# davxy/ark-vrf

Hardware: AMD Instinct MI355X
Metric: thin_vrf_batch_verifications_per_sec (higher is better)
Workload: dtype u32x8 (256-bit prime-field Montgomery, integer)

## Files before the change

### ark_vrf_amd/csrc/batch_terms_dev.h

```cpp
#pragma once
#include "proto_dev.h"

namespace avrf {

AVRF_DI fp fp_from_u128(const uint32_t *w) {
  fp a = fp_zero(); uint4 v = *reinterpret_cast<const uint4 *>(w);
  a.v[0] = v.x; a.v[1] = v.y; a.v[2] = v.z; a.v[3] = v.w; return a;
}
template <class S> AVRF_DI void emit_term(uint32_t *scalars, te_pre *pre, uint32_t t, const fp &scalar_plain, const uint8_t *xy) {
  using Fq = typename S::Fq;
  fp_store(scalars + 8 * (size_t)t, scalar_plain);
  fp x = fp_to_mont<Fq>(fp_load_le(xy)), y = fp_to_mont<Fq>(fp_load_le(xy + 32));
  store_pre(pre + t, te_make_pre<S>(x, y));
}

template <class F, int NT, bool ROLLED = false>
AVRF_DI fp block_sum(const fp &v, fp *red) {
  red[threadIdx.x] = v;
  __syncthreads();
#pragma unroll ROLLED ? 1 : NT
  for (int s2 = NT / 2; s2 >= 1; s2 >>= 1) {
    if ((int)threadIdx.x < s2) red[threadIdx.x] = fp_add<F>(red[threadIdx.x], red[threadIdx.x + s2]);
    __syncthreads();
  }
  return red[0];
}

template <class S, class Out>
AVRF_DI fp thin_item(const BatchDev &b, const Seed64 &seed, uint64_t j0, const uint32_t *__restrict__ c_in, const uint32_t *__restrict__ z_in,
                     uint32_t j, const Out &out) {
  using Fr = typename S::Fr;
  uint32_t io0 = b.io_off[j], m = b.io_off[j + 1] - io0;
  uint64_t gj = j0 + j;
  uint32_t ww[4];
  if (b.weights) { const uint4 v = *reinterpret_cast<const uint4 *>(b.weights + 16 * (size_t)j); ww[0] = v.x; ww[1] = v.y; ww[2] = v.z; ww[3] = v.w; }
  else { uint64_t blk[8]; sha512_xof_block(seed.w, gj >> 2, blk); digest_le128(blk, (int)(gj & 3), ww); }
  fp w_plain = fp_zero(); w_plain.v[0] = ww[0]; w_plain.v[1] = ww[1]; w_plain.v[2] = ww[2]; w_plain.v[3] = ww[3];
  fp w = fp_to_mont<Fr>(w_plain);
  fp c = fp_to_mont<Fr>(fp_from_u128(c_in + 4 * (size_t)j));
  const uint8_t *pr = b.proofs + 96 * (size_t)j;
  fp s = fp_to_mont<Fr>(fp_load_le(pr + 64));
  fp wc = fp_mul<Fr>(w, c);
  fp ws = fp_mul<Fr>(w, s);
  out.r(j, io0, w_plain, pr);
  out.key(j, io0, wc);
  for (uint32_t i = 0; i < m; i++) {
    fp z = fp_to_mont<Fr>(fp_from_u128(z_in + 4 * (size_t)(io0 + i)));
    const uint8_t *p = b.ios_xy + 128 * (size_t)(io0 + i);
    out.output(j, io0, i, fp_from_mont<Fr>(fp_mul<Fr>(wc, z)), p + 64);
    out.input(j, io0, i, fp_neg<Fr>(fp_mul<Fr>(ws, z)), p);
  }
  return ws;
}

template <class S, class Out>
AVRF_DI fp ped_item(const BatchDev &b, const Seed64 &seed, uint64_t j0, const uint32_t *__restrict__ c_in, const uint8_t *__restrict__ merged_xy,
                    uint32_t j, const Out &out, fp &usb) {
  using Fr = typename S::Fr;
  fp t_plain, u_plain;
  if (b.weights) { t_plain = fp_from_u128(reinterpret_cast<const uint32_t *>(b.weights + 32 * (size_t)j)); u_plain = fp_from_u128(reinterpret_cast<const uint32_t *>(b.weights + 32 * (size_t)j + 16)); }
  else {
    ShaReader rd; for (int i = 0; i < 8; i++) rd.seed[i] = seed.w[i]; rd.have = 0;
    t_plain = xof128(rd, (uint32_t)(2 * (j0 + j))); u_plain = xof128(rd, (uint32_t)(2 * (j0 + j) + 1));
  }
  fp tt = fp_to_mont<Fr>(t_plain), uu = fp_to_mont<Fr>(u_plain);
  fp c = fp_to_mont<Fr>(fp_from_u128(c_in + 4 * (size_t)j));
  const uint8_t *pr = b.proofs + 256 * (size_t)j, *mo = merged_xy + 128 * (size_t)j;
  fp s = fp_to_mont<Fr>(fp_load_le(pr + 192)), sb = fp_to_mont<Fr>(fp_load_le(pr + 224));
  out.term(j, 0, fp_from_mont<Fr>(fp_mul<Fr>(tt, c)), mo + 64);
  out.term(j, 1, t_plain, pr + 128);
  out.term(j, 2, fp_from_mont<Fr>(fp_neg<Fr>(fp_mul<Fr>(tt, s))), mo);
  out.term(j, 3, fp_from_mont<Fr>(fp_mul<Fr>(uu, c)), pr);
  out.term(j, 4, u_plain, pr + 64);
  const fp us = fp_mul<Fr>(uu, s); usb = fp_mul<Fr>(uu, sb);
  return us;
}

template <class S, bool ROLLED = false>
AVRF_DI void base_term(const uint32_t *__restrict__ gpart, uint32_t nparts, uint32_t *__restrict__ scalars, te_pre *__restrict__ pre,
                       uint32_t t_last, int which_base, fp *red) {
  using Fr = typename S::Fr; using Fq = typename S::Fq;
  fp acc = fp_zero();
  for (uint32_t i = threadIdx.x; i < nparts; i += 256) acc = fp_add<Fr>(acc, fp_load(gpart + 8 * (size_t)i));
  const fp sum = block_sum<Fr, 256, ROLLED>(acc, red);
  if (threadIdx.x == 0) {
    fp_store(scalars + 8 * (size_t)t_last, fp_from_mont<Fr>(fp_neg<Fr>(sum)));
    te_pre g;
    if (which_base == 0) { g.x = fp_const<Fq>(S::G_X); g.y = fp_const<Fq>(S::G_Y); g.k = fp_const<Fq>(S::G_K); }
    else { g.x = fp_const<Fq>(S::B_X); g.y = fp_const<Fq>(S::B_Y); g.k = fp_const<Fq>(S::B_K); }
    store_pre(pre + t_last, g);
  }
}

}
```

### ark_vrf_amd/csrc/consts_gen.h

```cpp
#pragma once
#include <stdint.h>

namespace avrf {

struct FqBandersnatch {
  static constexpr int N = 8;
  static constexpr uint32_t P[8] = {0x00000001u, 0xffffffffu, 0xfffe5bfeu, 0x53bda402u, 0x09a1d805u, 0x3339d808u, 0x299d7d48u, 0x73eda753u};
  static constexpr uint32_t ONE[8] = {0xfffffffeu, 0x00000001u, 0x00034802u, 0x5884b7fau, 0xecbc4ff5u, 0x998c4fefu, 0xacc5056fu, 0x1824b159u};
  static constexpr uint32_t R2[8] = {0xf3f29c6du, 0xc999e990u, 0x87925c23u, 0x2b6cedcbu, 0x7254398fu, 0x05d31496u, 0x9f59ff11u, 0x0748d9d9u};
  static constexpr uint32_t HALF[8] = {0x80000000u, 0x7fffffffu, 0x7fff2dffu, 0xa9ded201u, 0x04d0ec02u, 0x199cec04u, 0x94cebea4u, 0x39f6d3a9u};
  static constexpr uint32_t NINV = 0xffffffffu;
  static constexpr int BITS = 255;
  static constexpr bool FULL = false;
  static constexpr int TWO_ADICITY = 32;
  static constexpr uint32_t T_MINUS1_HALF[8] = {0x7fffffffu, 0x7fff2dffu, 0xa9ded201u, 0x04d0ec02u, 0x199cec04u, 0x94cebea4u, 0x39f6d3a9u, 0x00000000u};
  static constexpr uint32_t ROOT[8] = {0x0c17f47cu, 0x9cab6d5cu, 0xfd4b71e5u, 0x1ce1e93du, 0x471dd505u, 0x0d6db230u, 0x743a3b6au, 0x3f0ee990u};
  static constexpr uint32_t PM2[8] = {0xffffffffu, 0xfffffffeu, 0xfffe5bfeu, 0x53bda402u, 0x09a1d805u, 0x3339d808u, 0x299d7d48u, 0x73eda753u};
  static constexpr int SQRT_W = 8;
  static constexpr int SQRT_HW = 8;
  static constexpr int SQRT_STEPS = 4;
  static constexpr int SQRT_HBITS = 12;
  static constexpr uint32_t SQRT_HMUL = 0xa330d7b1u;
  static constexpr uint8_t SQRT_HIDX[4096] = {0, 0, 0, 139, 0, 0, 0, 0, 0, 0, 0, 167, 0, 0, 0, 0, 0, 0, 0, 0, 0, 133, 0, 0, 189, 0, 0, 0, 4, 0, 0, 0, 0, 0, 0, 0, 0, 0, 0, 226, 0, 0, 0, 0, 0, 248, 0, 0, 0, 0, 0, 0, 0, 0, 0, 0, 0, 0, 0, 0, 18, 0, 0, 0,
    0, 0, 0, 150, 0, 0, 0, 0, 0, 0, 0, 0, 0, 0, 0, 0, 0, 0, 0, 0, 0, 0, 0, 0, 0, 0, 0, 0, 0, 0, 0, 0, 0, 0, 0, 0, 0, 0, 0, 247, 0, 0, 0, 0, 0, 0, 0, 0, 0, 0, 0, 0, 0, 0, 0, 0, 0, 0, 0, 0, 0, 0, 0, 0,
    0, 0, 0, 0, 0, 0, 185, 0, 0, 0, 0, 0, 0, 0, 0, 0, 0, 148, 0, 0, 0, 0, 0, 0, 0, 0, 0, 0, 0, 0, 0, 0, 0, 0, 0, 0, 0, 0, 0, 0, 0, 0, 0, 0, 0, 0, 0, 0, 0, 17, 0, 0, 0, 0, 0, 0, 0, 0, 0, 0, 0, 0, 0, 0,
    0, 0, 0, 143, 0, 0, 0, 0, 0, 0, 0, 0, 0, 0, 0, 0, 0, 0, 0, 209, 0, 0, 0, 0, 0, 0, 0, 0, 0, 0, 0, 0, 0, 0, 0, 0, 0, 0, 0, 0, 0, 80, 0, 0, 0, 0, 0, 0, 0, 0, 0, 0, 0, 0, 23, 0, 0, 0, 0, 0, 0, 0, 0, 0,
    0, 0, 0, 0, 0, 0, 193, 0, 0, 0, 0, 0, 0, 0, 0, 0, 0, 0, 217, 0, 0, 0, 0, 0, 0, 0, 0, 0, 0, 210, 0, 0, 27, 0, 0, 0, 0, 0, 0, 0, 0, 0, 0, 0, 0, 0, 0, 0, 0, 0, 0, 0, 0, 0, 0, 230, 0, 77, 0, 161, 0, 0, 0, 0,
    0, 0, 0, 0, 0, 0, 0, 0, 0, 0, 0, 0, 121, 0, 0, 0, 0, 0, 0, 0, 0, 0, 173, 0, 0, 0, 0, 0, 0, 0, 0, 0, 0, 0, 0, 0, 0, 0, 188, 0, 0, 0, 0, 0, 0, 0, 0, 0, 0, 0, 0, 0, 0, 0, 0, 0, 0, 0, 0, 0, 0, 0, 0, 0,
    0, 0, 0, 0, 0, 0, 0, 0, 229, 0, 0, 0, 0, 0, 0, 0, 0, 0, 0, 99, 0, 0, 0, 0, 0, 0, 0, 0, 0, 0, 0, 0, 0, 0, 0, 0, 0, 0, 25, 0, 0, 0, 0, 0, 0, 0, 0, 0, 0, 0, 0, 0, 0, 0, 0, 0, 0, 0, 0, 0, 0, 0, 0, 0,
    0, 0, 218, 0, 0, 0, 0, 0, 0, 0, 0, 0, 0, 0, 0, 0, 0, 0, 0, 0, 0, 0, 0, 0, 0, 0, 0, 0, 0, 0, 0, 0, 0, 0, 0, 0, 156, 0, 0, 0, 0, 0, 0, 0, 0, 0, 0, 0, 0, 0, 0, 0, 0, 0, 0, 0, 0, 0, 0, 0, 0, 0, 0, 0,
    0, 0, 0, 0, 0, 0, 0, 0, 0, 0, 0, 0, 0, 0, 0, 0, 0, 0, 0, 0, 0, 0, 0, 0, 0, 0, 0, 0, 0, 0, 26, 0, 0, 0, 0, 0, 0, 0, 0, 0, 0, 236, 0, 0, 0, 0, 0, 0, 0, 55, 0, 0, 0, 0, 157, 0, 0, 0, 0, 0, 0, 0, 0, 0,
    0, 0, 0, 0, 0, 0, 0, 0, 0, 0, 0, 0, 0, 0, 0, 0, 0, 0, 0, 0, 109, 123, 0, 0, 0, 0, 0, 0, 0, 0, 0, 0, 0, 0, 0, 0, 0, 0, 0, 0, 0, 0, 0, 0, 0, 0, 0, 0, 0, 0, 0, 0, 0, 0, 0, 0, 0, 0, 0, 0, 0, 0, 0, 0,
    0, 0, 0, 225, 0, 0, 0, 0, 0, 0, 0, 0, 0, 0, 134, 0, 0, 159, 0, 0, 0, 0, 242, 0, 0, 0, 0, 244, 0, 0, 0, 0, 0, 0, 0, 0, 0, 0, 0, 0, 0, 0, 0, 0, 0, 0, 0, 0, 0, 0, 0, 0, 0, 0, 0, 0, 0, 0, 0, 76, 0, 0, 0, 152,
    0, 0, 0, 0, 0, 0, 0, 0, 0, 0, 0, 0, 0, 164, 0, 0, 0, 0, 0, 223, 0, 0, 21, 0, 0, 0, 0, 0, 0, 0, 40, 0, 0, 0, 0, 0, 0, 0, 0, 0, 0, 0, 0, 0, 0, 0, 0, 0, 0, 0, 0, 0, 0, 0, 0, 0, 0, 0, 0, 0, 0, 0, 0, 0,
    0, 0, 0, 0, 0, 0, 0, 0, 0, 0, 0, 0, 0, 141, 0, 0, 0, 0, 0, 0, 0, 0, 0, 0, 0, 0, 0, 0, 0, 0, 0, 0, 0, 0, 0, 0, 0, 0, 0, 0, 0, 0, 0, 0, 0, 0, 0, 0, 0, 0, 0, 0, 0, 0, 0, 0, 0, 0, 0, 0, 0, 0, 0, 0,
    0, 0, 0, 0, 0, 0, 0, 0, 0, 0, 0, 0, 0, 93, 0, 0, 0, 0, 171, 0, 0, 0, 0, 0, 0, 0, 0, 0, 0, 0, 0, 0, 0, 0, 0, 0, 0, 0, 0, 0, 0, 0, 0, 0, 0, 0, 0, 0, 0, 79, 0, 0, 0, 0, 0, 0, 0, 0, 0, 0, 0, 0, 0, 0,
    0, 0, 0, 0, 0, 0, 0, 0, 0, 0, 0, 0, 0, 0, 0, 0, 0, 0, 0, 0, 0, 0, 0, 0, 0, 0, 0, 0, 0, 0, 0, 0, 0, 0, 0, 0, 0, 0, 0, 0, 0, 0, 91, 0, 0, 158, 0, 0, 0, 0, 0, 0, 0, 0, 0, 0, 0, 0, 0, 0, 0, 0, 0, 0,
    0, 0, 0, 0, 0, 0, 0, 0, 0, 0, 0, 200, 0, 0, 0, 0, 0, 0, 0, 0, 0, 0, 0, 0, 0, 0, 0, 0, 0, 0, 0, 63, 0, 0, 0, 0, 0, 0, 0, 0, 0, 0, 0, 0, 0, 66, 0, 0, 0, 0, 0, 0, 0, 0, 0, 0, 0, 0, 0, 0, 0, 0, 0, 0,
    0, 0, 0, 0, 0, 0, 0, 0, 222, 0, 0, 0, 0, 0, 0, 0, 0, 0, 182, 0, 0, 0, 0, 0, 0, 0, 0, 0, 0, 0, 0, 0, 0, 0, 0, 0, 0, 0, 0, 0, 0, 0, 0, 0, 0, 0, 0, 0, 0, 0, 0, 0, 0, 0, 0, 0, 0, 0, 0, 0, 0, 0, 0, 0,
    0, 0, 0, 0, 0, 0, 0, 0, 0, 0, 0, 0, 0, 0, 0, 0, 0, 0, 0, 0, 113, 0, 0, 0, 0, 0, 0, 0, 0, 0, 0, 0, 0, 0, 0, 0, 0, 0, 0, 0, 124, 255, 0, 0, 0, 0, 0, 0, 0, 0, 0, 0, 0, 0, 59, 0, 0, 0, 0, 0, 0, 0, 0, 0,
    0, 0, 0, 0, 0, 0, 0, 0, 0, 0, 0, 0, 0, 170, 0, 0, 0, 184, 0, 0, 0, 0, 0, 87, 0, 0, 0, 83, 0, 0, 0, 0, 0, 0, 0, 0, 0, 0, 0, 44, 0, 0, 0, 0, 0, 0, 64, 0, 0, 0, 0, 0, 0, 0, 0, 0, 0, 0, 0, 0, 0, 0, 0, 0,
    0, 0, 0, 0, 0, 0, 0, 0, 0, 0, 0, 0, 0, 0, 0, 0, 0, 0, 0, 14, 0, 0, 0, 0, 0, 0, 0, 0, 0, 0, 0, 0, 213, 0, 0, 0, 0, 0, 0, 0, 0, 0, 0, 203, 0, 0, 0, 0, 0, 0, 0, 0, 199, 52, 0, 0, 0, 0, 0, 0, 0, 0, 0, 0,
    0, 0, 0, 0, 0, 86, 0, 0, 0, 0, 69, 0, 0, 126, 0, 0, 0, 0, 0, 0, 48, 0, 0, 0, 0, 0, 0, 0, 0, 0, 176, 0, 0, 0, 0, 0, 0, 254, 0, 0, 197, 0, 0, 0, 0, 214, 0, 0, 0, 0, 0, 0, 0, 0, 0, 0, 0, 0, 0, 0, 0, 180, 71, 0,
    0, 0, 0, 0, 0, 0, 0, 75, 0, 0, 0, 0, 0, 0, 0, 0, 0, 0, 85, 0, 0, 0, 0, 0, 0, 0, 0, 0, 0, 0, 0, 142, 0, 0, 0, 0, 0, 0, 0, 0, 0, 0, 0, 0, 0, 0, 0, 0, 0, 0, 0, 0, 0, 0, 0, 0, 0, 0, 0, 0, 0, 0, 0, 0,
    0, 0, 0, 0, 192, 0, 0, 0, 0, 0, 0, 172, 0, 0, 0, 0, 0, 0, 0, 0, 0, 0, 0, 211, 0, 0, 0, 215, 0, 0, 0, 0, 0, 0, 56, 0, 0, 42, 0, 0, 0, 0, 0, 0, 0, 0, 0, 0, 0, 0, 0, 0, 0, 0, 0, 0, 0, 0, 0, 0, 187, 0, 0, 0,
    0, 0, 0, 0, 0, 0, 0, 0, 0, 127, 252, 0, 0, 0, 0, 0, 0, 0, 0, 0, 0, 0, 0, 0, 0, 0, 0, 0, 0, 0, 241, 0, 0, 0, 0, 0, 0, 0, 0, 0, 0, 0, 0, 0, 0, 0, 0, 0, 0, 0, 0, 0, 0, 0, 0, 0, 0, 0, 0, 0, 0, 0, 0, 0,
    0, 0, 0, 0, 0, 0, 0, 0, 0, 0, 0, 0, 0, 0, 0, 0, 0, 0, 0, 0, 0, 0, 0, 0, 0, 0, 0, 0, 0, 0, 0, 0, 54, 0, 0, 0, 0, 0, 0, 0, 0, 0, 94, 0, 0, 0, 0, 0, 0, 0, 0, 0, 0, 0, 0, 0, 0, 0, 0, 0, 0, 0, 0, 0,
    0, 0, 0, 0, 0, 194, 0, 0, 0, 0, 0, 0, 0, 0, 0, 0, 0, 0, 0, 191, 0, 0, 0, 0, 0, 0, 0, 0, 0, 0, 0, 0, 0, 0, 0, 0, 0, 0, 0, 72, 0, 0, 0, 0, 0, 0, 0, 0, 0, 0, 0, 0, 0, 0, 0, 0, 0, 0, 0, 0, 0, 0, 0, 0,
    0, 0, 0, 0, 0, 30, 0, 0, 219, 0, 0, 0, 0, 0, 0, 0, 0, 0, 0, 0, 0, 0, 0, 0, 0, 0, 0, 0, 0, 0, 0, 0, 0, 0, 0, 0, 0, 0, 0, 0, 0, 0, 0, 0, 0, 0, 0, 0, 0, 0, 0, 0, 0, 0, 0, 0, 0, 0, 0, 0, 0, 0, 0, 0,
    0, 207, 0, 0, 0, 0, 0, 0, 0, 0, 0, 0, 0, 0, 0, 0, 0, 0, 0, 0, 0, 0, 0, 0, 0, 0, 0, 0, 0, 0, 0, 0, 0, 43, 0, 0, 0, 221, 0, 0, 0, 0, 0, 0, 0, 0, 0, 0, 0, 0, 0, 0, 0, 0, 0, 0, 0, 0, 0, 0, 0, 0, 0, 0,
    0, 0, 0, 0, 0, 0, 0, 0, 0, 0, 0, 0, 0, 0, 0, 0, 0, 0, 0, 0, 0, 0, 0, 0, 0, 0, 0, 0, 0, 0, 0, 0, 0, 0, 0, 0, 0, 13, 0, 0, 0, 0, 0, 0, 0, 0, 0, 0, 0, 0, 0, 0, 0, 0, 0, 0, 0, 0, 0, 0, 0, 0, 0, 0,
    0, 0, 0, 0, 0, 0, 0, 0, 0, 0, 0, 0, 0, 0, 0, 0, 0, 0, 0, 0, 168, 0, 0, 0, 0, 0, 0, 0, 149, 0, 0, 95, 0, 0, 0, 0, 0, 36, 0, 0, 0, 0, 0, 0, 0, 0, 0, 0, 0, 0, 0, 24, 0, 0, 0, 204, 0, 0, 0, 0, 0, 0, 0, 0,
    0, 0, 0, 0, 0, 0, 0, 0, 0, 0, 0, 0, 0, 0, 0, 0, 0, 0, 0, 0, 0, 0, 0, 116, 0, 0, 0, 0, 114, 0, 0, 0, 0, 31, 0, 0, 6, 0, 0, 0, 0, 0, 0, 0, 0, 0, 0, 97, 0, 0, 0, 0, 0, 0, 0, 0, 0, 0, 0, 0, 0, 0, 0, 0,
    0, 0, 0, 0, 0, 0, 0, 0, 0, 0, 0, 0, 0, 0, 0, 0, 0, 0, 0, 0, 0, 0, 0, 0, 0, 0, 0, 0, 0, 251, 237, 0, 0, 0, 0, 0, 0, 0, 0, 0, 0, 0, 0, 0, 0, 0, 0, 0, 0, 0, 0, 0, 0, 0, 0, 0, 0, 0, 0, 0, 29, 0, 0, 0,
    0, 183, 0, 0, 0, 0, 0, 0, 0, 108, 0, 0, 0, 0, 0, 0, 0, 0, 0, 0, 154, 0, 0, 0, 0, 0, 0, 0, 0, 0, 0, 0, 0, 0, 0, 0, 0, 0, 0, 0, 0, 0, 0, 0, 0, 0, 0, 0, 0, 0, 0, 0, 0, 0, 0, 0, 0, 0, 0, 0, 0, 0, 0, 0,
    0, 0, 0, 0, 0, 0, 0, 0, 0, 0, 0, 0, 0, 0, 0, 28, 0, 0, 0, 0, 0, 0, 0, 0, 0, 0, 0, 0, 0, 0, 0, 0, 0, 0, 0, 0, 0, 0, 0, 0, 0, 0, 0, 0, 0, 0, 0, 0, 90, 0, 0, 0, 0, 0, 0, 0, 0, 0, 0, 0, 0, 0, 0, 0,
    0, 0, 0, 0, 0, 0, 0, 0, 0, 0, 0, 0, 153, 0, 0, 0, 0, 0, 0, 0, 0, 0, 0, 0, 0, 0, 0, 0, 0, 0, 0, 227, 0, 0, 0, 0, 0, 0, 0, 0, 0, 0, 101, 0, 0, 0, 0, 0, 0, 0, 0, 0, 0, 0, 0, 0, 0, 0, 0, 0, 0, 0, 0, 0,
    0, 0, 0, 0, 0, 0, 0, 0, 0, 0, 0, 0, 60, 0, 0, 0, 0, 0, 0, 0, 0, 0, 0, 0, 0, 0, 0, 0, 45, 0, 0, 0, 0, 0, 0, 0, 0, 0, 249, 0, 0, 0, 0, 0, 0, 0, 0, 0, 0, 0, 0, 0, 0, 0, 0, 33, 0, 205, 0, 102, 0, 0, 0, 0,
    0, 0, 0, 0, 0, 0, 0, 0, 0, 0, 0, 0, 0, 0, 0, 0, 0, 0, 155, 0, 0, 82, 0, 0, 0, 0, 0, 0, 0, 0, 0, 0, 89, 0, 0, 0, 0, 0, 0, 0, 0, 0, 0, 0, 65, 0, 0, 0, 0, 0, 0, 0, 0, 0, 0, 0, 0, 0, 0, 0, 151, 0, 0, 0,
    0, 0, 0, 0, 0, 0, 0, 0, 0, 208, 0, 0, 0, 0, 0, 0, 0, 0, 0, 0, 0, 0, 0, 0, 0, 0, 0, 0, 0, 0, 0, 81, 0, 0, 0, 0, 0, 0, 0, 0, 0, 0, 0, 0, 0, 0, 0, 15, 0, 0, 0, 0, 0, 0, 0, 0, 0, 0, 0, 0, 0, 0, 0, 0,
    0, 145, 0, 0, 0, 0, 0, 0, 0, 0, 0, 0, 0, 0, 0, 0, 0, 0, 0, 0, 0, 0, 0, 0, 0, 0, 0, 0, 0, 0, 0, 0, 0, 20, 0, 0, 0, 0, 0, 0, 0, 0, 0, 0, 57, 0, 0, 0, 0, 0, 0, 0, 0, 0, 0, 0, 0, 0, 0, 0, 0, 0, 0, 0,
    0, 0, 0, 0, 0, 0, 0, 0, 0, 0, 0, 119, 0, 0, 0, 0, 0, 0, 0, 0, 0, 0, 0, 0, 0, 0, 0, 0, 0, 0, 0, 0, 0, 0, 0, 0, 0, 0, 0, 0, 0, 0, 0, 0, 0, 0, 0, 22, 0, 0, 0, 0, 0, 0, 146, 0, 0, 0, 0, 0, 0, 0, 0, 0,
    0, 0, 0, 0, 0, 120, 0, 0, 0, 0, 0, 98, 0, 0, 0, 0, 0, 0, 0, 0, 0, 0, 132, 0, 0, 0, 61, 0, 0, 5, 0, 0, 0, 0, 0, 0, 0, 0, 0, 39, 0, 0, 0, 0, 0, 0, 0, 11, 0, 0, 0, 0, 0, 0, 0, 0, 0, 0, 0, 0, 0, 0, 0, 0,
    0, 0, 0, 0, 0, 0, 0, 0, 0, 0, 0, 0, 0, 0, 0, 0, 234, 0, 0, 0, 0, 0, 0, 0, 0, 0, 0, 92, 0, 0, 0, 0, 0, 0, 0, 0, 0, 0, 0, 0, 0, 0, 0, 0, 0, 0, 0, 0, 0, 0, 0, 19, 0, 0, 0, 0, 0, 0, 0, 186, 0, 0, 0, 0,
    0, 0, 0, 0, 0, 0, 0, 0, 0, 0, 0, 0, 0, 0, 0, 0, 0, 0, 0, 0, 0, 0, 0, 0, 0, 0, 0, 0, 0, 0, 0, 0, 0, 0, 0, 0, 0, 0, 0, 0, 0, 0, 0, 195, 0, 0, 0, 0, 0, 0, 0, 0, 0, 0, 0, 0, 0, 0, 0, 0, 0, 0, 0, 0,
    0, 0, 0, 0, 0, 0, 0, 0, 12, 0, 0, 0, 73, 0, 0, 0, 100, 0, 0, 0, 0, 0, 0, 0, 0, 0, 0, 0, 0, 0, 0, 0, 0, 0, 239, 0, 0, 0, 0, 0, 0, 0, 0, 0, 0, 0, 0, 0, 62, 0, 0, 0, 50, 0, 0, 0, 0, 0, 0, 0, 0, 0, 0, 3,
    0, 0, 0, 0, 7, 0, 0, 0, 122, 0, 0, 0, 0, 0, 0, 0, 0, 0, 0, 0, 0, 130, 0, 0, 0, 9, 68, 0, 0, 0, 0, 0, 0, 0, 0, 0, 0, 0, 0, 0, 0, 0, 0, 0, 0, 0, 0, 0, 0, 0, 0, 0, 0, 0, 0, 0, 216, 0, 0, 0, 0, 105, 175, 0,
    0, 0, 0, 0, 0, 0, 0, 0, 0, 0, 0, 0, 0, 0, 0, 0, 0, 115, 0, 0, 0, 0, 0, 0, 0, 0, 0, 0, 0, 0, 0, 117, 0, 0, 0, 0, 0, 0, 238, 0, 0, 0, 0, 0, 118, 0, 0, 0, 0, 0, 0, 0, 0, 35, 129, 0, 0, 0, 169, 0, 0, 0, 0, 0,
    0, 0, 0, 0, 0, 160, 0, 0, 0, 0, 70, 0, 174, 0, 0, 0, 0, 0, 0, 0, 0, 0, 0, 0, 0, 0, 0, 0, 0, 0, 0, 0, 0, 34, 0, 0, 0, 0, 10, 0, 0, 0, 0, 0, 0, 0, 0, 0, 0, 0, 0, 0, 0, 0, 0, 0, 0, 0, 0, 0, 0, 0, 0, 0,
    0, 0, 0, 0, 0, 0, 0, 0, 0, 0, 0, 0, 0, 0, 0, 0, 0, 0, 0, 0, 0, 0, 0, 0, 0, 0, 0, 253, 0, 0, 0, 0, 0, 0, 0, 0, 0, 0, 0, 0, 0, 0, 0, 0, 165, 0, 0, 0, 0, 0, 0, 0, 0, 0, 0, 0, 181, 0, 0, 0, 0, 0, 0, 0,
    0, 0, 0, 0, 0, 0, 0, 0, 0, 0, 0, 0, 0, 0, 0, 0, 0, 0, 177, 0, 0, 0, 212, 0, 0, 0, 0, 0, 0, 0, 0, 0, 166, 0, 0, 0, 0, 0, 0, 0, 0, 0, 107, 0, 0, 0, 0, 0, 0, 0, 0, 0, 0, 0, 0, 0, 0, 0, 0, 0, 0, 0, 0, 0,
    0, 0, 0, 0, 0, 0, 0, 0, 0, 0, 0, 0, 0, 0, 0, 0, 0, 0, 0, 232, 0, 0, 0, 0, 0, 0, 0, 0, 224, 0, 0, 0, 0, 0, 0, 0, 0, 0, 0, 0, 0, 0, 0, 0, 0, 0, 0, 0, 0, 0, 0, 0, 0, 0, 240, 0, 0, 0, 0, 0, 0, 0, 0, 0,
    0, 0, 0, 0, 0, 0, 0, 0, 0, 0, 0, 0, 0, 0, 0, 0, 0, 0, 0, 0, 0, 0, 0, 0, 0, 0, 0, 0, 0, 0, 0, 0, 0, 0, 0, 0, 0, 0, 0, 0, 0, 0, 0, 0, 0, 0, 0, 0, 0, 0, 0, 0, 0, 0, 0, 0, 0, 0, 0, 0, 0, 0, 0, 0,
    0, 0, 0, 16, 0, 0, 0, 0, 0, 0, 0, 0, 0, 0, 0, 0, 0, 0, 0, 0, 0, 0, 0, 0, 0, 0, 0, 51, 0, 0, 0, 0, 0, 0, 0, 0, 0, 0, 0, 0, 0, 0, 0, 0, 0, 0, 0, 0, 0, 0, 0, 0, 74, 0, 0, 0, 0, 0, 0, 0, 0, 0, 103, 0,
    0, 0, 0, 0, 0, 8, 78, 0, 0, 0, 0, 0, 0, 0, 0, 0, 0, 0, 0, 0, 0, 0, 0, 0, 0, 0, 0, 0, 0, 0, 0, 0, 0, 0, 0, 0, 0, 0, 0, 0, 0, 0, 0, 0, 206, 136, 0, 0, 0, 0, 0, 0, 231, 0, 0, 0, 0, 0, 0, 0, 0, 0, 202, 0,
    0, 0, 0, 0, 0, 0, 0, 0, 0, 0, 0, 0, 0, 0, 0, 0, 0, 0, 0, 0, 0, 0, 0, 179, 0, 0, 0, 0, 0, 0, 0, 0, 0, 0, 0, 0, 0, 0, 0, 0, 0, 0, 0, 0, 0, 0, 0, 144, 0, 0, 0, 0, 0, 0, 0, 0, 0, 0, 0, 0, 0, 0, 0, 0,
    0, 0, 0, 0, 0, 0, 0, 0, 0, 0, 0, 0, 0, 0, 0, 0, 0, 0, 0, 0, 0, 0, 0, 0, 0, 0, 0, 0, 0, 0, 0, 0, 0, 0, 0, 0, 0, 0, 0, 0, 0, 0, 0, 0, 0, 0, 0, 0, 0, 0, 0, 0, 0, 0, 0, 0, 0, 0, 0, 0, 112, 0, 0, 0,
    0, 0, 0, 0, 0, 0, 0, 0, 0, 0, 0, 0, 0, 0, 0, 0, 0, 0, 0, 0, 0, 0, 96, 0, 0, 0, 0, 0, 0, 0, 0, 104, 0, 0, 0, 0, 0, 0, 0, 0, 0, 0, 0, 0, 0, 0, 0, 0, 0, 0, 0, 0, 0, 0, 0, 0, 0, 0, 0, 0, 0, 0, 0, 0,
    0, 0, 0, 0, 0, 0, 0, 0, 235, 0, 0, 0, 0, 0, 0, 0, 0, 0, 38, 0, 0, 0, 0, 0, 0, 0, 0, 0, 84, 0, 0, 0, 49, 0, 0, 0, 0, 0, 0, 0, 0, 0, 0, 0, 0, 0, 0, 0, 0, 0, 0, 0, 0, 0, 0, 0, 0, 0, 53, 0, 0, 0, 0, 0,
    0, 0, 0, 0, 0, 0, 37, 0, 0, 0, 0, 0, 0, 0, 0, 0, 0, 0, 0, 0, 0, 0, 0, 125, 0, 0, 0, 0, 0, 0, 0, 0, 0, 0, 0, 0, 0, 0, 0, 0, 0, 0, 0, 0, 0, 0, 0, 0, 0, 0, 0, 0, 0, 0, 0, 0, 0, 0, 0, 0, 0, 0, 0, 0,
    0, 0, 0, 0, 0, 0, 0, 0, 0, 0, 0, 0, 138, 0, 0, 0, 0, 162, 0, 0, 0, 0, 0, 0, 0, 128, 0, 0, 0, 0, 0, 0, 0, 0, 0, 0, 0, 0, 46, 0, 198, 0, 0, 0, 0, 32, 0, 0, 0, 0, 0, 0, 0, 0, 0, 0, 41, 0, 0, 0, 1, 163, 0, 0,
    0, 0, 0, 0, 0, 0, 246, 0, 0, 0, 0, 0, 110, 0, 0, 0, 0, 0, 0, 245, 0, 0, 0, 0, 0, 0, 0, 0, 0, 0, 0, 0, 0, 243, 0, 0, 0, 0, 0, 0, 0, 0, 0, 0, 0, 0, 0, 0, 0, 0, 0, 0, 47, 233, 0, 0, 0, 0, 88, 0, 0, 0, 0, 0,
    0, 0, 0, 0, 0, 0, 0, 0, 0, 0, 0, 0, 0, 0, 0, 0, 0, 0, 0, 0, 0, 0, 0, 0, 196, 137, 0, 0, 0, 2, 0, 0, 0, 0, 0, 0, 0, 0, 0, 0, 0, 0, 250, 0, 0, 0, 135, 0, 0, 0, 0, 131, 0, 0, 0, 0, 0, 0, 0, 0, 0, 0, 178, 0,
    0, 0, 190, 0, 0, 0, 0, 0, 0, 0, 0, 0, 0, 0, 0, 0, 111, 0, 0, 0, 0, 0, 0, 0, 0, 0, 0, 0, 0, 0, 0, 0, 0, 0, 228, 0, 0, 0, 0, 201, 0, 0, 140, 0, 0, 0, 0, 0, 0, 0, 0, 0, 0, 0, 0, 0, 0, 0, 0, 0, 0, 0, 0, 0,
    0, 0, 0, 0, 0, 0, 0, 67, 0, 0, 0, 0, 0, 0, 0, 0, 0, 0, 0, 0, 0, 0, 0, 0, 0, 0, 0, 0, 0, 0, 0, 0, 0, 0, 0, 0, 0, 0, 0, 0, 0, 0, 0, 0, 0, 0, 0, 0, 0, 0, 0, 0, 0, 0, 0, 58, 0, 0, 0, 0, 0, 0, 0, 147,
    0, 0, 0, 0, 0, 0, 0, 0, 0, 0, 0, 0, 0, 0, 0, 0, 0, 0, 0, 0, 0, 0, 0, 220, 0, 0, 0, 0, 0, 0, 0, 0, 0, 0, 106, 0, 0, 0, 0, 0, 0, 0, 0, 0, 0, 0, 0, 0, 0, 0, 0, 0, 0, 0, 0, 0, 0, 0, 0, 0, 0, 0, 0, 0};
  static constexpr uint32_t SQRT_G[4][256][8] = {{{0xfffffffeu, 0x00000001u, 0x00034802u, 0x5884b7fau, 0xecbc4ff5u, 0x998c4fefu, 0xacc5056fu, 0x1824b159u},
     {0xb3082d19u, 0x55a9e082u, 0xc7dc4a13u, 0x082f90b2u, 0xc76b052cu, 0x76ce3accu, 0x6e54185du, 0x15c39d95u},
     {0x05ddb4b8u, 0xb1bb81b1u, 0x4a762df0u, 0x98ffbb06u, 0xc5590209u, 0x726e959bu, 0x47a5e6aau, 0x0db2facbu},
     {0x4ba518a6u, 0x1cb397a0u, 0xe29bbae1u, 0xa6c4b1a6u, 0x446848f8u, 0x9c4d6f8cu, 0x4f599f0fu, 0x38590951u},
     {0x081b0db0u, 0x88291cf6u, 0x961782b0u, 0x8dea521au, 0x5485c90cu, 0xbf29568bu, 0x48e86a89u, 0x0abe1809u},
     {0xa619ac2au, 0x7a94fe9cu, 0xacd2cd1du, 0xa7d16f94u, 0x3f6d45e1u, 0xeb6432c7u, 0x69cba988u, 0x675bd361u},
// ... 1965 lines not shown
     {0x38a0b01eu, 0x71711555u, 0x4ad8bc83u, 0x7b62860au, 0x8782f80cu, 0xdae18326u, 0x8643d3c0u, 0x659d3378u},
     {0xe79619e8u, 0xbea57a0du, 0x30dfe95cu, 0xa307a773u, 0x757cc2b5u, 0xfa9bfbe4u, 0x7793ed48u, 0x1f278bdau},
     {0x5c85a48cu, 0xa5c78e6bu, 0x27dea76du, 0x3321a9d5u, 0x26f5f2ffu, 0x650e3bc6u, 0xf388ee57u, 0x05dc672au},
     {0x21df81e1u, 0xd49618f1u, 0x69e1efbdu, 0x629f100fu, 0x290a9c33u, 0xe5ec780au, 0x195bd29fu, 0x42342477u},
     {0x8f153822u, 0x190c7999u, 0x255bed10u, 0xff8667b7u, 0xfca3ce8au, 0xab9a30e6u, 0xcc563dc6u, 0x67d521b3u},
     {0x0c9a6196u, 0xe1ab252eu, 0x8c4639a8u, 0x99e01587u, 0x53ac4640u, 0xde1593d3u, 0x63fba955u, 0x545dee68u},
     {0x9d5bfae5u, 0x0eeebb8au, 0xac1efb3du, 0xff066916u, 0xddacd1a4u, 0x08c08e43u, 0x8948edf4u, 0x3f78143au},
     {0x2e7f1dc5u, 0x985c3cf6u, 0x9931a557u, 0x2ce65886u, 0xa5c89bbbu, 0xc783312eu, 0x6c4ec654u, 0x63692be2u},
     {0xc8a679b5u, 0x1575b970u, 0xe7d73a66u, 0xff7e3e9eu, 0x75be7c92u, 0x197077f6u, 0xd9afc7c1u, 0x4f67aeeau},
     {0x27640509u, 0xb0adef9au, 0x5f151c19u, 0x5959fdadu, 0x1d65c479u, 0x465e597bu, 0xd2631306u, 0x54db6e81u},
     {0xfb9b6cafu, 0xe4ea9f4du, 0xa2e53698u, 0xc5c2f8bfu, 0x32e15854u, 0x3656c273u, 0xf624afb5u, 0x14e2af6au},
     {0x5cc3402fu, 0x9df8c650u, 0x8eecfc0bu, 0x52161e02u, 0xc15e1bd4u, 0xd8363390u, 0xb209a781u, 0x58b8ae49u},
     {0x0edcce43u, 0xac2d119au, 0x0b5c9748u, 0x72e16391u, 0xb8958a06u, 0xa5715c3au, 0x57eeddd7u, 0x208a3b69u},
     {0x2c42eff8u, 0x6ecf4995u, 0x4d5dfa57u, 0x6ec1fa83u, 0x5656b15cu, 0x3ff5cf38u, 0x229e031bu, 0x54b80267u},
     {0xcc8444a5u, 0x90f6ca3bu, 0xb2348e04u, 0x14328249u, 0xee9ff368u, 0x9e1a4112u, 0x36badb91u, 0x49871dbdu},
     {0x295f01c5u, 0x2120e8a1u, 0x2bfa2fe5u, 0xcdebe1c7u, 0xdbbe9be6u, 0x2316952cu, 0xad2c723cu, 0x4b12a723u},
     {0x5b26f8b7u, 0x7ec4963du, 0xbaf08852u, 0xfc700595u, 0xe05523aau, 0xafc2f038u, 0x47197ed5u, 0x6b38b922u},
     {0x00ff35a2u, 0x2df3cffeu, 0xd8a54c35u, 0x8eaad385u, 0x73beda30u, 0x5a69ae1eu, 0x25cd8149u, 0x0ff2db8bu},
     {0x74dd5d7du, 0xbbb83148u, 0x8dafb8d6u, 0x39a9f661u, 0xe2db2568u, 0x0b08c472u, 0xee3af837u, 0x57598d2du},
     {0x87c54b83u, 0x693a8406u, 0xc68ebc74u, 0x1a480ddfu, 0x1ab40886u, 0xbf6277d1u, 0x79357d86u, 0x5f1a79ecu},
     {0xcd01e401u, 0x508f9afdu, 0xf449da9eu, 0xe348018cu, 0x4e84779du, 0xd552b7f9u, 0x37192982u, 0x41a2d19fu},
     {0xfa15c3aau, 0x3f250480u, 0xc047eb08u, 0xe07f6b96u, 0xe062508du, 0x3e4c19e1u, 0x72c2db07u, 0x071af18du},
     {0x1926ef0au, 0xd71a1016u, 0x14f1596bu, 0x1f063ac7u, 0xe929c6e2u, 0x0a9280b4u, 0xb8adeebcu, 0x37c836e3u},
     {0x1fd6ad56u, 0x6f765257u, 0xb0e5ddc4u, 0x5e09ca58u, 0xe6edaba3u, 0x452d4de9u, 0xa6d8a0a9u, 0x49cc3e60u},
     {0x2960af99u, 0xcb4b0e08u, 0x9f39e65cu, 0xaf57e981u, 0x51900ae1u, 0xc67b09b0u, 0xff21015eu, 0x085174abu},
     {0x0e92863cu, 0xb8390a3au, 0xc2863873u, 0x96044e6au, 0x8d6a0836u, 0x687322c8u, 0x8c1fa261u, 0x5c67f128u},
     {0x2cc8d086u, 0x97ae36d8u, 0x86ed9472u, 0x12c8360eu, 0x61e28bc2u, 0x8abd6721u, 0x520aa6bau, 0x6a96e461u},
     {0x11015834u, 0x7179e258u, 0x123ae337u, 0x00cc579fu, 0xcd24624bu, 0x34d5b008u, 0xe61da78au, 0x4e3c38aeu},
     {0x1ccd9350u, 0x38252215u, 0x513cd923u, 0xe2be613bu, 0x8613483eu, 0x952dd456u, 0xef52bfbeu, 0x2bdc7f5fu},
     {0x8e7396bdu, 0x9b248771u, 0x26512fcau, 0xf3b6754du, 0x1c539a97u, 0x34d5a86au, 0x758a30b2u, 0x188eeac5u},
     {0x11f2bec2u, 0x5f804b9bu, 0x974c34d5u, 0xb8795d14u, 0xf2df56e6u, 0xd88bc50au, 0x4ee3ffdcu, 0x6965d71cu},
     {0x3ed117d1u, 0x978cf7c8u, 0x8c5be1cbu, 0xfbea1715u, 0x3735000eu, 0xea44c4dbu, 0x4f6a138bu, 0x09f5c923u},
     {0x242103d5u, 0x0488c019u, 0x8a9255c6u, 0xda927718u, 0x2189c3f0u, 0xc1df9b00u, 0xd80c2aaau, 0x6a479f59u},
     {0x83be6793u, 0xa747e335u, 0x65f3469bu, 0x67e96b40u, 0x28053fe0u, 0xf27eec7cu, 0x5df2e598u, 0x3967452au},
     {0x06690b79u, 0x20871c43u, 0xc6cf4b80u, 0xf1994a48u, 0x91c8ecb4u, 0x8f821e00u, 0xaa89169au, 0x0bfb4c4eu},
     {0xd326577fu, 0x86b66109u, 0xc2e56c9bu, 0xf62e7165u, 0xa281ca4fu, 0x0f24d9cau, 0x5418de14u, 0x6827b849u},
     {0xea815d48u, 0x0b5a32d5u, 0x4a0239d4u, 0x6d1b4960u, 0x54de0512u, 0x5923129bu, 0x23174a1eu, 0x65a0400fu},
     {0x47dc3a8eu, 0x21419c6fu, 0x0e46c9e4u, 0x7317c3f5u, 0x3cd7e698u, 0x7c1e12ccu, 0x657c748bu, 0x72f09140u},
     {0x1248245au, 0x8870b9e3u, 0xd2cab986u, 0xb02ab3e2u, 0x4e204b01u, 0x6bc2be6du, 0xb4e2f21fu, 0x06f9fbb5u},
     {0x475f9917u, 0x4f8202a9u, 0x455e945bu, 0x55bf85ebu, 0xe32d7d9du, 0x6d4c8d1cu, 0x750bb29cu, 0x4d07a125u},
     {0xad0a14b7u, 0x7bd28a68u, 0x6693267fu, 0xf23d8db7u, 0xb520258cu, 0x54781be7u, 0x076cae45u, 0x319e968fu},
     {0x58371c58u, 0xe2723242u, 0x4596c7a7u, 0x953f710au, 0x05336c1au, 0xdd8e0667u, 0xba634814u, 0x44b2c153u},
     {0x0e3f6ca9u, 0x1280ba88u, 0x5ed2de1eu, 0x61b18d33u, 0x5cf486ceu, 0xb7f93933u, 0x9990f2ecu, 0x63369ddfu},
     {0x04de444bu, 0x1f5c0f6fu, 0xe3cfbaabu, 0x990b7d15u, 0x1a08d412u, 0xf8c2d5b9u, 0xc1fc894au, 0x31d70d61u},
     {0xab0be02bu, 0x53705adau, 0x98a62326u, 0x68512e19u, 0xd9f802e0u, 0x61571bdbu, 0x5c24e491u, 0x2fce8180u},
     {0xf4f5ed78u, 0xda3d5ffcu, 0x82f63a76u, 0xbca13283u, 0x3187122cu, 0xebfffb3du, 0x3aba3b86u, 0x248d2ba9u},
     {0x8e9fd984u, 0x7fce7d9bu, 0xd3b4713fu, 0x8af4e9ebu, 0x492b1d8eu, 0xa4f87dc0u, 0x8bb2d12du, 0x64b4b4e0u},
     {0xdd4f278cu, 0x75d572e8u, 0x13fc66ddu, 0x6d430159u, 0x92af252eu, 0xbaaa83d0u, 0xd31e8d84u, 0x394417c5u},
     {0x58da6aa4u, 0x82a20808u, 0x74829b5cu, 0x0228ee6au, 0xc9ad1160u, 0xb003ab1du, 0x34558665u, 0x41c5136bu},
     {0x7a99de9eu, 0x5a005690u, 0x277c49dbu, 0xcadb8951u, 0x829c620eu, 0x2379d76du, 0x244f4e65u, 0x1b378533u},
     {0xd4f64112u, 0xbf907bd1u, 0x77f47f45u, 0x0b168a22u, 0x08cc3a32u, 0x08c0e078u, 0xb0466d3au, 0x2c9cf211u},
     {0x78608249u, 0x05966d0bu, 0xb5386ac0u, 0x2f0458f2u, 0x264a0035u, 0x9b2e75ebu, 0x153a4cdfu, 0x3977f860u},
     {0x165d516eu, 0x963577f8u, 0x2ac0d3c5u, 0xaad9d00du, 0x64beed41u, 0x1afb7aaeu, 0x5051301du, 0x27006e59u},
     {0xcaca8313u, 0x0f1935d8u, 0x13b9bbe6u, 0x6bb619c1u, 0xe3f7a2d4u, 0x897d1e65u, 0x61ad525cu, 0x60ef201fu},
     {0x7c58e718u, 0xc11900b5u, 0x2c8cf843u, 0x7ddacaffu, 0xee2be61cu, 0xd9c13167u, 0x52050d46u, 0x0a9f3ae4u},
     {0xc9b1d3fcu, 0x6d79af89u, 0x7fb0345bu, 0x691fa9cau, 0x0ee1a74bu, 0xbac24d73u, 0x7e18a2aeu, 0x4865647eu},
     {0x14820d20u, 0x480d513cu, 0xdbea11dfu, 0xf3335d70u, 0x048359d7u, 0x2ba2fb41u, 0xf0f5e5d3u, 0x137198c5u},
     {0x916f7696u, 0x89bcccc5u, 0x88346f55u, 0x289bfc73u, 0x92e7d2d2u, 0xf36fb797u, 0xa7975ff5u, 0x4e97b638u},
     {0x3f739ac8u, 0xbfb0e683u, 0x2a5dfc83u, 0xe78fdad9u, 0xf8d6a763u, 0xf56f910eu, 0xf7e98b32u, 0x2fb9a958u},
     {0x709d69b0u, 0xd2b7d884u, 0xa111176cu, 0xbd13cd26u, 0x860eeebbu, 0x16f27755u, 0x5135a880u, 0x5ade1e7eu},
     {0x9853db04u, 0x81002b30u, 0xa5110b64u, 0x505d3ffdu, 0xe499541du, 0x43f3d603u, 0x1650b215u, 0x2883be66u},
     {0xdce32ecdu, 0x3a9b9f5bu, 0xb00bfc10u, 0xbdf98f59u, 0x894d3c96u, 0x961ca1b7u, 0x8a58766au, 0x579b3349u},
     {0x7d1f75b2u, 0x1b3c4feeu, 0x5af3fbc6u, 0x5265b158u, 0x1b468fe1u, 0x7e5c8c6au, 0xc3df928cu, 0x5ad7fe3au},
     {0x85190e97u, 0x3ff4cf36u, 0x76bf2e40u, 0x40c0d395u, 0x0bab14adu, 0xa5f3819du, 0x9390c01fu, 0x1ac4416bu},
     {0x3f26a9d1u, 0x25c3d512u, 0x083589c5u, 0x7d76d9e3u, 0x48c34a65u, 0xcfd61babu, 0x815554bcu, 0x3a10c229u},
     {0x71609b1au, 0xe8e8d1dfu, 0x0eb2f768u, 0x1cf1e962u, 0x9768a3c1u, 0x9fabe672u, 0xc6caae31u, 0x08ecbfa6u},
     {0x79bf4f1bu, 0xb5319907u, 0x983baadeu, 0xf317d445u, 0x6e269d85u, 0xfff73680u, 0xf4271f8du, 0x49c8dabcu},
     {0x83d014fau, 0x4606e968u, 0x7cd8ed52u, 0xc1f33b71u, 0xefba713au, 0x14e48227u, 0xc1c7efe4u, 0x54150adbu},
     {0x49eb7f23u, 0xa3b3f4dbu, 0x8caa9728u, 0x200f8a43u, 0x2652d494u, 0x7fc85d41u, 0x81885aefu, 0x1fee884cu},
     {0x8ad8bf35u, 0xe2646a4eu, 0xad159082u, 0x8b0d49dcu, 0xc608d4a7u, 0x2437f5abu, 0xc2606638u, 0x10270bf3u},
     {0x78f132efu, 0x8e7b2bddu, 0x7fd503e5u, 0x34528098u, 0x42d80083u, 0x0ea75e6eu, 0xfa0fd473u, 0x307f4f00u},
     {0x6494ce4bu, 0x5be50d8cu, 0x0e4a28fcu, 0x1f0038d4u, 0x5a6e8ca6u, 0x7bf4c2ceu, 0xb9f90fa8u, 0x5d5b87f2u},
     {0xb6e0b9e0u, 0x5b7a9877u, 0x6c064730u, 0x0932ac01u, 0x23023385u, 0x3f58c35au, 0xc343d22au, 0x42431340u},
     {0x0cd952aeu, 0x3c9c9e42u, 0x237cc1a0u, 0xbc23d412u, 0x5dc8bba1u, 0x9d7bd317u, 0x42ab5b37u, 0x29f78689u},
     {0xe0d8211cu, 0x816f371cu, 0xd22347ceu, 0x32bf4b89u, 0x4a501e19u, 0x9d272cfeu, 0x5f1ce5a8u, 0x0e3e41e3u},
     {0xeeacbd55u, 0x353e37b1u, 0xe98d368cu, 0x575b1e34u, 0xb25a5128u, 0xb9d5021bu, 0xe185e732u, 0x1caae6b8u},
     {0x88ac07cdu, 0x6b45cacbu, 0xe9500b87u, 0x09c4d7b2u, 0xf27cbdc9u, 0x2d5de551u, 0x49cd4467u, 0x07fa8c1cu}}};
};
struct FrBandersnatch {
  static constexpr int N = 8;
  static constexpr uint32_t P[8] = {0x2876e7e1u, 0x74fd06b5u, 0x74190471u, 0xff8f8700u, 0x02687600u, 0x0cce7602u, 0xca675f52u, 0x1cfb69d4u};
  static constexpr uint32_t ONE[8] = {0xbc48c0f8u, 0x5817ca56u, 0x5f37dc74u, 0x0383c7fcu, 0xecbc4ff8u, 0x998c4fefu, 0xacc5056fu, 0x1824b159u};
  static constexpr uint32_t R2[8] = {0x58db47cbu, 0xdbb4f5d6u, 0x7fecb938u, 0x40fa7ca2u, 0xc0055ceau, 0xaa9e6daeu, 0xb14aec7du, 0x0ae793ddu};
  static constexpr uint32_t HALF[8] = {0x943b73f0u, 0xba7e835au, 0x3a0c8238u, 0x7fc7c380u, 0x01343b00u, 0x06673b01u, 0x6533afa9u, 0x0e7db4eau};
  static constexpr uint32_t NINV = 0x5cc063dfu;
  static constexpr int BITS = 253;
  static constexpr bool FULL = false;
  static constexpr int TWO_ADICITY = 5;
  static constexpr uint32_t T_MINUS1_HALF[8] = {0xd4a1db9fu, 0xc5d3f41au, 0x01d06411u, 0x03fe3e1cu, 0x0809a1d8u, 0x483339d8u, 0x53299d7du, 0x0073eda7u};
  static constexpr uint32_t ROOT[8] = {0x8d79c573u, 0x4b263b9au, 0x007af1fdu, 0xeadb3d0au, 0x68832589u, 0xa54c8a46u, 0x4254fb9du, 0x0610860cu};
  static constexpr uint32_t PM2[8] = {0x2876e7dfu, 0x74fd06b5u, 0x74190471u, 0xff8f8700u, 0x02687600u, 0x0cce7602u, 0xca675f52u, 0x1cfb69d4u};
};
struct FqBabyJubJub {
  static constexpr int N = 8;
  static constexpr uint32_t P[8] = {0xf0000001u, 0x43e1f593u, 0x79b97091u, 0x2833e848u, 0x8181585du, 0xb85045b6u, 0xe131a029u, 0x30644e72u};
  static constexpr uint32_t ONE[8] = {0x4ffffffbu, 0xac96341cu, 0x9f60cd29u, 0x36fc7695u, 0x7879462eu, 0x666ea36fu, 0x9a07df2fu, 0x0e0a77c1u};
  static constexpr uint32_t R2[8] = {0xae216da7u, 0x1bb8e645u, 0xe35c59e3u, 0x53fe3ab1u, 0x53bb8085u, 0x8c49833du, 0x7f4e44a5u, 0x0216d0b1u};
  static constexpr uint32_t HALF[8] = {0xf8000000u, 0xa1f0fac9u, 0x3cdcb848u, 0x9419f424u, 0x40c0ac2eu, 0xdc2822dbu, 0x7098d014u, 0x18322739u};
  static constexpr uint32_t NINV = 0xefffffffu;
  static constexpr int BITS = 254;
  static constexpr bool FULL = false;
  static constexpr int TWO_ADICITY = 28;
  static constexpr uint32_t T_MINUS1_HALF[8] = {0x1f0fac9fu, 0xcdcb848au, 0x419f4243u, 0x0c0ac2e9u, 0xc2822db4u, 0x098d014du, 0x83227397u, 0x00000001u};
  static constexpr uint32_t ROOT[8] = {0x80d13d9cu, 0x636e7355u, 0x2445ffd6u, 0xa22bf374u, 0x1eb203d8u, 0x56452ac0u, 0x2963f9e7u, 0x1860ef94u};
  static constexpr uint32_t PM2[8] = {0xefffffffu, 0x43e1f593u, 0x79b97091u, 0x2833e848u, 0x8181585du, 0xb85045b6u, 0xe131a029u, 0x30644e72u};
  static constexpr int SQRT_W = 8;
  static constexpr int SQRT_HW = 8;
  static constexpr int SQRT_STEPS = 4;
  static constexpr int SQRT_HBITS = 12;
  static constexpr uint32_t SQRT_HMUL = 0x64ac5db9u;
  static constexpr uint8_t SQRT_HIDX[4096] = {170, 0, 0, 0, 0, 0, 0, 0, 0, 0, 0, 0, 0, 0, 0, 0, 0, 0, 0, 0, 0, 0, 0, 0, 0, 0, 0, 0, 0, 196, 0, 0, 0, 0, 0, 0, 0, 0, 0, 0, 0, 0, 0, 0, 0, 0, 0, 0, 0, 0, 0, 0, 0, 0, 0, 0, 0, 0, 0, 0, 0, 0, 0, 0,
    0, 0, 0, 0, 0, 0, 0, 0, 0, 0, 0, 0, 0, 0, 0, 0, 0, 0, 0, 0, 0, 0, 0, 0, 0, 0, 0, 198, 0, 0, 0, 0, 0, 0, 0, 103, 0, 165, 0, 0, 1, 0, 0, 0, 0, 0, 0, 0, 0, 0, 0, 0, 0, 0, 0, 0, 0, 0, 0, 0, 0, 0, 0, 0,
    0, 0, 0, 0, 0, 0, 0, 0, 0, 0, 0, 0, 0, 0, 0, 0, 166, 0, 0, 0, 0, 0, 0, 0, 0, 0, 0, 0, 0, 0, 0, 0, 0, 0, 0, 0, 0, 0, 195, 0, 0, 0, 0, 0, 0, 0, 0, 0, 0, 0, 0, 0, 26, 0, 0, 0, 0, 0, 0, 105, 0, 0, 0, 0,
    0, 0, 0, 0, 0, 0, 0, 0, 0, 0, 0, 0, 0, 0, 0, 0, 0, 0, 0, 0, 163, 0, 0, 0, 0, 0, 0, 0, 0, 0, 0, 0, 0, 0, 0, 0, 0, 0, 0, 0, 0, 0, 228, 0, 187, 0, 0, 0, 0, 0, 0, 0, 0, 0, 117, 0, 0, 0, 0, 0, 0, 0, 98, 0,
    0, 0, 191, 0, 0, 0, 0, 0, 0, 0, 0, 0, 0, 0, 0, 0, 0, 0, 0, 0, 0, 0, 0, 0, 52, 0, 0, 0, 0, 0, 0, 0, 0, 0, 0, 0, 0, 0, 0, 0, 0, 0, 0, 0, 0, 0, 0, 0, 0, 0, 0, 0, 0, 0, 0, 0, 0, 0, 0, 0, 0, 0, 0, 0,
    0, 0, 0, 0, 115, 0, 0, 0, 0, 0, 0, 0, 0, 0, 0, 0, 0, 0, 0, 0, 0, 0, 0, 0, 0, 234, 0, 0, 0, 0, 0, 0, 0, 123, 0, 0, 0, 0, 0, 0, 0, 0, 0, 0, 0, 0, 0, 0, 0, 0, 0, 0, 0, 0, 0, 0, 0, 0, 0, 19, 0, 0, 0, 0,
    0, 0, 0, 0, 0, 0, 0, 0, 0, 0, 0, 0, 0, 0, 0, 0, 0, 0, 0, 0, 0, 0, 0, 0, 0, 0, 0, 0, 0, 0, 0, 0, 0, 0, 0, 0, 0, 0, 0, 0, 0, 0, 0, 0, 0, 0, 0, 0, 0, 0, 0, 0, 0, 0, 0, 0, 0, 0, 0, 0, 0, 0, 0, 0,
    0, 125, 0, 0, 0, 0, 2, 0, 0, 0, 0, 0, 0, 0, 0, 0, 0, 0, 40, 0, 0, 0, 0, 0, 0, 0, 0, 0, 0, 0, 0, 0, 183, 0, 0, 0, 0, 0, 0, 0, 0, 0, 0, 0, 0, 0, 27, 0, 0, 0, 0, 0, 0, 0, 0, 0, 0, 0, 0, 0, 0, 0, 0, 0,
    0, 0, 0, 0, 0, 0, 0, 0, 0, 0, 0, 0, 0, 0, 0, 0, 0, 0, 0, 0, 0, 104, 0, 0, 0, 0, 0, 0, 0, 0, 0, 0, 0, 0, 0, 0, 0, 0, 0, 0, 13, 0, 0, 0, 0, 0, 0, 0, 0, 0, 0, 0, 0, 0, 33, 0, 0, 0, 0, 0, 0, 0, 0, 0,
    0, 0, 0, 0, 0, 0, 0, 0, 0, 0, 0, 0, 0, 0, 90, 0, 0, 0, 0, 205, 0, 0, 0, 0, 0, 0, 0, 0, 0, 0, 0, 0, 0, 0, 0, 47, 0, 0, 0, 0, 172, 0, 0, 0, 0, 0, 0, 41, 0, 0, 0, 0, 0, 0, 0, 0, 0, 0, 0, 0, 0, 0, 0, 0,
    255, 0, 0, 0, 0, 0, 0, 0, 0, 0, 0, 0, 0, 0, 0, 188, 0, 241, 0, 0, 0, 0, 0, 0, 0, 0, 0, 0, 5, 0, 0, 0, 0, 0, 0, 0, 0, 0, 0, 0, 0, 0, 0, 0, 0, 240, 0, 0, 0, 0, 0, 0, 0, 74, 0, 0, 22, 0, 0, 0, 0, 0, 0, 0,
    0, 0, 0, 0, 0, 0, 0, 0, 0, 0, 0, 0, 0, 0, 0, 0, 0, 206, 0, 0, 0, 0, 0, 0, 0, 0, 0, 0, 194, 0, 0, 0, 0, 0, 0, 0, 0, 0, 0, 0, 0, 0, 0, 0, 0, 0, 0, 0, 0, 0, 0, 0, 0, 0, 0, 0, 0, 0, 0, 0, 0, 0, 0, 0,
    0, 0, 0, 0, 0, 0, 0, 0, 56, 0, 0, 0, 0, 0, 0, 0, 84, 0, 0, 0, 0, 0, 0, 0, 0, 0, 0, 0, 0, 0, 0, 0, 0, 0, 0, 0, 0, 0, 0, 0, 0, 0, 0, 0, 0, 0, 0, 0, 0, 0, 0, 0, 0, 0, 0, 0, 0, 0, 0, 0, 0, 0, 219, 0,
    0, 0, 0, 30, 0, 0, 0, 0, 73, 0, 0, 0, 0, 0, 0, 0, 0, 0, 0, 0, 0, 0, 3, 0, 0, 0, 143, 0, 0, 0, 0, 0, 0, 11, 0, 189, 0, 0, 0, 0, 0, 0, 0, 0, 0, 0, 0, 0, 0, 0, 23, 0, 0, 49, 0, 0, 0, 0, 0, 0, 0, 0, 89, 0,
    0, 0, 39, 0, 0, 0, 0, 0, 0, 0, 0, 0, 0, 0, 102, 0, 0, 0, 107, 0, 0, 0, 0, 76, 0, 0, 0, 0, 0, 0, 0, 0, 0, 0, 0, 0, 0, 0, 0, 0, 0, 0, 0, 0, 0, 0, 0, 0, 0, 0, 0, 0, 0, 0, 0, 0, 0, 0, 0, 0, 0, 0, 0, 0,
    0, 0, 0, 0, 0, 0, 0, 0, 0, 0, 0, 0, 0, 0, 0, 0, 0, 0, 0, 0, 0, 0, 0, 0, 0, 0, 0, 83, 0, 0, 0, 0, 0, 0, 0, 0, 0, 0, 0, 0, 0, 0, 0, 0, 0, 0, 0, 0, 0, 0, 186, 0, 0, 0, 227, 0, 0, 7, 0, 0, 92, 0, 247, 0,
    0, 181, 0, 0, 0, 0, 0, 0, 0, 0, 0, 0, 0, 0, 0, 0, 199, 0, 0, 0, 0, 0, 0, 0, 0, 0, 0, 0, 0, 0, 0, 0, 0, 0, 0, 0, 0, 0, 0, 0, 0, 0, 0, 0, 0, 0, 0, 50, 0, 0, 0, 0, 0, 0, 0, 0, 0, 0, 0, 0, 0, 0, 0, 0,
    0, 0, 0, 0, 0, 0, 0, 0, 0, 0, 0, 0, 0, 0, 0, 0, 0, 0, 0, 0, 0, 0, 0, 0, 0, 0, 0, 0, 95, 0, 0, 0, 0, 0, 0, 0, 0, 0, 0, 0, 0, 0, 0, 0, 0, 0, 0, 0, 0, 0, 0, 0, 0, 0, 0, 0, 0, 36, 0, 0, 0, 0, 0, 0,
    0, 0, 0, 0, 0, 0, 0, 0, 0, 0, 0, 0, 0, 0, 0, 0, 0, 0, 0, 0, 237, 0, 0, 0, 0, 0, 0, 0, 0, 149, 0, 0, 0, 0, 0, 0, 229, 0, 0, 0, 159, 0, 0, 0, 0, 0, 88, 0, 0, 0, 0, 0, 110, 0, 0, 0, 0, 0, 0, 0, 0, 0, 0, 0,
    0, 156, 0, 0, 0, 0, 0, 0, 0, 0, 0, 0, 0, 0, 0, 0, 0, 145, 0, 0, 0, 0, 0, 0, 0, 0, 0, 0, 0, 0, 0, 0, 0, 64, 0, 0, 0, 0, 0, 0, 0, 0, 0, 0, 0, 0, 0, 0, 0, 0, 0, 0, 0, 0, 0, 0, 0, 0, 0, 0, 0, 0, 0, 0,
    0, 0, 0, 0, 0, 0, 0, 0, 0, 79, 0, 0, 0, 0, 0, 0, 0, 0, 0, 0, 0, 193, 0, 69, 0, 62, 0, 0, 0, 0, 0, 0, 0, 0, 0, 0, 120, 0, 0, 0, 0, 0, 0, 0, 0, 0, 0, 0, 0, 0, 0, 0, 0, 0, 0, 0, 0, 0, 0, 0, 0, 0, 0, 214,
    0, 0, 0, 0, 0, 0, 0, 0, 0, 0, 0, 0, 0, 0, 0, 0, 122, 0, 48, 0, 0, 144, 0, 0, 0, 0, 0, 0, 0, 0, 0, 0, 0, 0, 0, 54, 0, 0, 0, 0, 0, 0, 0, 200, 0, 0, 0, 0, 0, 0, 0, 0, 0, 0, 0, 0, 0, 0, 0, 0, 0, 0, 0, 0,
    0, 0, 0, 0, 0, 0, 0, 0, 0, 0, 0, 0, 0, 0, 0, 0, 0, 0, 0, 0, 0, 0, 0, 0, 0, 0, 0, 0, 0, 0, 0, 0, 0, 244, 0, 0, 224, 0, 0, 0, 6, 0, 0, 0, 0, 0, 0, 0, 246, 0, 0, 0, 0, 209, 0, 0, 0, 0, 0, 0, 0, 0, 0, 0,
    0, 0, 142, 0, 0, 0, 0, 0, 0, 0, 0, 0, 0, 0, 75, 0, 0, 0, 0, 0, 222, 0, 0, 0, 0, 0, 0, 0, 0, 0, 0, 0, 0, 0, 0, 0, 0, 0, 0, 0, 0, 0, 0, 0, 0, 0, 0, 0, 0, 0, 0, 0, 0, 0, 0, 0, 0, 0, 0, 0, 0, 0, 0, 0,
    8, 0, 0, 0, 0, 0, 0, 0, 0, 0, 0, 0, 0, 0, 0, 0, 0, 0, 0, 0, 0, 0, 18, 0, 0, 0, 0, 0, 0, 0, 0, 0, 0, 0, 0, 0, 0, 0, 0, 0, 0, 0, 0, 114, 0, 0, 0, 0, 0, 0, 0, 0, 0, 0, 0, 0, 0, 45, 0, 0, 0, 0, 0, 85,
    0, 0, 0, 0, 0, 0, 0, 0, 0, 0, 0, 0, 0, 0, 0, 0, 0, 0, 0, 0, 0, 0, 0, 0, 0, 0, 0, 0, 0, 0, 0, 0, 0, 0, 0, 0, 0, 0, 0, 0, 0, 0, 0, 0, 0, 32, 0, 0, 0, 0, 46, 0, 0, 0, 0, 0, 0, 0, 0, 0, 0, 0, 0, 0,
    0, 0, 0, 0, 0, 0, 0, 0, 0, 0, 137, 0, 0, 87, 0, 0, 0, 0, 0, 0, 0, 0, 0, 0, 0, 0, 29, 0, 0, 0, 0, 0, 0, 0, 0, 0, 0, 0, 0, 0, 0, 0, 0, 0, 0, 0, 0, 157, 0, 0, 0, 0, 0, 0, 0, 0, 0, 0, 0, 0, 0, 215, 0, 0,
    9, 0, 0, 0, 0, 0, 0, 0, 0, 0, 0, 0, 0, 0, 0, 0, 0, 0, 0, 0, 0, 0, 0, 0, 174, 0, 0, 0, 0, 160, 0, 0, 0, 0, 0, 0, 0, 0, 0, 0, 0, 0, 0, 0, 0, 0, 0, 0, 0, 0, 0, 0, 0, 0, 0, 0, 0, 0, 0, 0, 0, 0, 0, 0,
    0, 0, 0, 0, 0, 0, 0, 0, 0, 0, 0, 213, 0, 0, 0, 0, 173, 0, 0, 0, 0, 0, 0, 0, 0, 0, 0, 0, 0, 0, 0, 242, 0, 0, 0, 0, 0, 0, 0, 0, 0, 0, 0, 0, 0, 0, 0, 0, 0, 0, 0, 0, 146, 0, 0, 0, 0, 0, 0, 0, 0, 0, 0, 0,
    0, 0, 0, 0, 0, 0, 0, 0, 0, 0, 136, 0, 0, 0, 0, 0, 0, 0, 0, 0, 0, 0, 0, 0, 0, 0, 0, 0, 0, 0, 0, 0, 0, 0, 0, 0, 0, 0, 0, 0, 0, 0, 0, 0, 0, 0, 0, 0, 0, 0, 0, 0, 0, 0, 94, 0, 0, 0, 0, 203, 0, 0, 0, 0,
    0, 0, 0, 0, 0, 0, 0, 0, 14, 0, 0, 0, 0, 0, 0, 0, 0, 0, 0, 0, 0, 81, 0, 0, 0, 118, 0, 0, 0, 0, 0, 0, 0, 0, 134, 0, 0, 0, 96, 0, 0, 116, 0, 0, 0, 0, 0, 0, 0, 0, 0, 0, 0, 0, 0, 0, 0, 0, 0, 0, 0, 0, 0, 0,
    0, 0, 0, 0, 0, 0, 0, 0, 0, 0, 0, 0, 0, 0, 0, 0, 0, 0, 0, 0, 0, 0, 0, 0, 0, 0, 0, 0, 0, 0, 0, 72, 0, 0, 0, 0, 0, 0, 0, 182, 0, 0, 0, 0, 0, 0, 0, 0, 0, 0, 0, 0, 0, 16, 0, 0, 176, 0, 250, 0, 0, 0, 0, 0,
    0, 0, 0, 0, 0, 0, 0, 0, 0, 0, 0, 86, 0, 0, 0, 0, 0, 0, 0, 0, 0, 0, 0, 0, 0, 0, 0, 0, 0, 0, 0, 0, 0, 0, 0, 0, 0, 0, 248, 0, 0, 0, 0, 0, 0, 0, 0, 0, 0, 190, 0, 197, 0, 65, 0, 0, 0, 0, 0, 0, 0, 0, 0, 0,
    0, 207, 0, 0, 0, 0, 0, 0, 0, 0, 0, 0, 0, 0, 0, 0, 0, 0, 0, 0, 0, 0, 0, 0, 0, 0, 0, 0, 0, 0, 0, 0, 0, 0, 0, 0, 0, 0, 0, 0, 0, 192, 0, 0, 0, 0, 0, 0, 0, 0, 0, 0, 0, 0, 0, 0, 0, 17, 0, 0, 0, 0, 0, 0,
    0, 0, 0, 0, 0, 0, 0, 0, 0, 28, 0, 0, 0, 0, 0, 0, 0, 0, 0, 0, 0, 0, 238, 0, 0, 0, 0, 0, 216, 0, 0, 0, 0, 31, 0, 0, 0, 0, 101, 0, 0, 0, 0, 0, 0, 21, 0, 0, 0, 0, 0, 0, 0, 0, 109, 0, 0, 0, 0, 0, 0, 0, 0, 0,
    0, 0, 0, 0, 0, 0, 0, 0, 0, 0, 0, 0, 0, 0, 0, 0, 0, 164, 0, 0, 0, 0, 0, 0, 0, 0, 0, 0, 0, 0, 0, 0, 0, 0, 0, 0, 0, 0, 0, 0, 0, 0, 0, 0, 0, 223, 0, 0, 0, 0, 0, 0, 0, 0, 0, 0, 0, 0, 0, 0, 0, 0, 0, 0,
    0, 0, 0, 0, 0, 0, 0, 0, 0, 0, 0, 0, 0, 0, 0, 0, 0, 0, 0, 0, 0, 0, 0, 0, 0, 0, 0, 178, 0, 0, 0, 0, 0, 0, 0, 0, 0, 0, 0, 0, 0, 0, 0, 0, 0, 0, 0, 0, 0, 0, 0, 0, 0, 0, 0, 0, 0, 71, 0, 0, 0, 0, 0, 0,
    0, 0, 0, 0, 0, 0, 0, 0, 0, 53, 0, 119, 0, 0, 220, 0, 0, 135, 0, 0, 99, 0, 0, 0, 58, 0, 0, 0, 0, 0, 0, 0, 0, 0, 0, 0, 0, 0, 0, 0, 0, 0, 0, 0, 0, 0, 0, 211, 0, 0, 0, 0, 0, 0, 0, 0, 0, 0, 0, 0, 0, 0, 0, 0,
    0, 0, 0, 0, 0, 0, 0, 0, 0, 0, 0, 0, 0, 0, 0, 0, 0, 0, 0, 0, 0, 0, 0, 0, 0, 0, 0, 0, 0, 0, 0, 0, 0, 0, 0, 0, 0, 0, 0, 0, 0, 0, 0, 0, 0, 0, 0, 0, 0, 0, 0, 204, 0, 0, 0, 0, 235, 0, 0, 230, 0, 0, 0, 0,
    0, 0, 0, 0, 0, 0, 0, 167, 0, 0, 0, 217, 0, 0, 0, 0, 0, 0, 0, 0, 0, 177, 0, 0, 151, 0, 0, 0, 0, 0, 0, 0, 0, 0, 0, 0, 0, 0, 0, 61, 0, 139, 0, 0, 0, 0, 0, 0, 15, 0, 0, 0, 131, 0, 0, 0, 0, 0, 0, 0, 0, 0, 0, 0,
    0, 0, 201, 0, 0, 0, 0, 158, 0, 0, 0, 0, 91, 0, 0, 0, 0, 0, 0, 0, 0, 0, 0, 0, 0, 0, 0, 0, 0, 0, 0, 0, 0, 0, 0, 0, 0, 0, 0, 0, 0, 0, 0, 0, 0, 0, 0, 0, 0, 0, 0, 0, 0, 0, 0, 0, 0, 0, 212, 0, 0, 0, 0, 0,
    0, 0, 184, 0, 0, 0, 0, 0, 0, 0, 0, 0, 0, 0, 0, 0, 0, 0, 0, 0, 0, 0, 0, 0, 0, 0, 0, 0, 0, 0, 0, 0, 0, 0, 0, 0, 0, 0, 0, 0, 0, 0, 0, 0, 0, 0, 66, 0, 0, 0, 0, 0, 0, 0, 0, 0, 0, 78, 0, 0, 0, 0, 0, 0,
    0, 0, 0, 0, 0, 0, 0, 0, 0, 0, 0, 0, 0, 0, 0, 0, 0, 0, 150, 0, 0, 202, 0, 0, 0, 0, 0, 0, 0, 112, 0, 0, 0, 0, 0, 0, 0, 0, 0, 0, 0, 0, 0, 0, 0, 0, 133, 0, 0, 0, 0, 0, 0, 0, 0, 0, 0, 113, 0, 60, 0, 0, 0, 0,
    0, 0, 0, 0, 0, 0, 0, 0, 0, 0, 127, 0, 0, 0, 0, 0, 0, 0, 0, 0, 0, 0, 0, 0, 0, 0, 169, 0, 0, 0, 0, 0, 0, 0, 44, 0, 0, 0, 175, 0, 0, 0, 0, 0, 0, 0, 0, 0, 0, 0, 0, 0, 0, 0, 0, 77, 0, 0, 0, 218, 0, 0, 0, 0,
    0, 0, 0, 0, 0, 0, 0, 0, 0, 0, 0, 0, 0, 0, 0, 0, 0, 0, 0, 0, 161, 0, 0, 0, 0, 0, 0, 0, 0, 0, 0, 0, 0, 0, 141, 0, 0, 0, 0, 0, 0, 0, 0, 0, 0, 0, 0, 0, 0, 0, 0, 0, 0, 232, 0, 0, 0, 0, 0, 0, 0, 0, 0, 0,
    0, 0, 0, 0, 0, 0, 0, 0, 0, 0, 0, 0, 0, 0, 0, 0, 0, 0, 0, 0, 0, 0, 0, 0, 0, 0, 0, 0, 155, 0, 0, 0, 0, 0, 0, 0, 0, 0, 0, 0, 0, 0, 55, 0, 0, 0, 0, 0, 0, 0, 0, 0, 0, 0, 0, 168, 0, 0, 0, 0, 0, 0, 0, 0,
    0, 0, 0, 130, 0, 0, 0, 0, 0, 253, 0, 0, 0, 0, 0, 0, 0, 0, 0, 0, 0, 0, 0, 0, 0, 0, 0, 0, 0, 0, 0, 0, 0, 0, 0, 0, 0, 0, 0, 0, 0, 0, 0, 0, 0, 0, 0, 0, 0, 0, 0, 0, 0, 0, 0, 0, 0, 0, 0, 0, 0, 0, 0, 0,
    0, 0, 0, 0, 0, 0, 0, 0, 0, 0, 0, 0, 0, 0, 0, 147, 0, 0, 0, 0, 0, 0, 0, 0, 0, 0, 0, 0, 0, 0, 0, 0, 0, 0, 0, 0, 0, 0, 0, 0, 0, 251, 0, 0, 0, 0, 0, 0, 0, 106, 0, 0, 0, 0, 0, 0, 0, 0, 0, 0, 0, 0, 0, 0,
    0, 0, 0, 0, 0, 243, 0, 0, 0, 0, 0, 0, 0, 0, 0, 0, 0, 0, 0, 0, 0, 0, 0, 0, 0, 0, 0, 0, 0, 0, 0, 0, 0, 0, 0, 0, 0, 0, 0, 0, 0, 0, 0, 0, 0, 0, 0, 0, 0, 0, 180, 0, 0, 0, 0, 0, 0, 0, 0, 0, 0, 0, 0, 0,
    0, 0, 0, 0, 0, 0, 0, 0, 63, 0, 0, 0, 226, 0, 0, 0, 0, 0, 0, 0, 245, 0, 0, 0, 0, 0, 0, 0, 0, 0, 59, 0, 100, 0, 0, 0, 0, 0, 0, 0, 0, 0, 0, 0, 0, 0, 0, 0, 0, 0, 0, 0, 0, 0, 35, 0, 0, 0, 0, 0, 0, 0, 0, 0,
    0, 0, 0, 0, 0, 0, 0, 0, 0, 0, 0, 0, 0, 0, 0, 233, 0, 0, 0, 0, 0, 0, 154, 0, 0, 0, 0, 0, 0, 0, 0, 0, 0, 0, 0, 0, 67, 0, 0, 0, 0, 0, 0, 0, 0, 0, 0, 0, 0, 0, 0, 0, 0, 0, 0, 0, 0, 0, 38, 0, 0, 0, 0, 0,
    0, 0, 0, 0, 0, 0, 0, 0, 0, 0, 0, 0, 0, 0, 0, 0, 0, 0, 0, 0, 0, 0, 0, 0, 0, 0, 0, 0, 0, 0, 0, 0, 0, 0, 129, 0, 0, 37, 0, 231, 0, 0, 0, 0, 0, 0, 70, 0, 0, 0, 0, 0, 0, 0, 0, 0, 0, 0, 0, 0, 0, 0, 0, 0,
    0, 0, 0, 0, 0, 0, 0, 0, 0, 0, 0, 0, 0, 0, 0, 0, 0, 0, 0, 0, 0, 0, 0, 0, 0, 0, 0, 0, 0, 0, 0, 0, 0, 0, 0, 0, 0, 0, 0, 0, 0, 0, 0, 0, 0, 68, 0, 0, 0, 0, 0, 0, 0, 0, 0, 0, 0, 0, 0, 0, 0, 0, 0, 0,
    0, 0, 0, 0, 0, 0, 0, 0, 0, 0, 42, 0, 0, 0, 0, 0, 0, 0, 0, 132, 0, 0, 0, 0, 0, 0, 0, 0, 0, 20, 0, 0, 0, 0, 0, 0, 0, 0, 0, 0, 0, 0, 0, 0, 0, 0, 0, 0, 0, 0, 0, 0, 0, 0, 0, 0, 0, 0, 0, 0, 0, 0, 0, 0,
    121, 0, 0, 0, 0, 0, 0, 0, 0, 0, 0, 0, 0, 0, 0, 0, 0, 0, 0, 0, 108, 0, 0, 0, 0, 0, 0, 0, 0, 0, 0, 0, 0, 0, 0, 0, 0, 0, 0, 0, 0, 0, 0, 239, 0, 0, 0, 43, 0, 0, 0, 0, 0, 0, 0, 0, 0, 140, 0, 0, 0, 0, 0, 0,
    0, 0, 0, 0, 0, 0, 0, 0, 0, 0, 0, 0, 0, 0, 0, 0, 0, 0, 0, 0, 0, 0, 0, 0, 0, 0, 0, 0, 0, 0, 0, 0, 0, 0, 57, 0, 0, 0, 0, 0, 0, 0, 0, 0, 0, 0, 0, 0, 0, 0, 0, 0, 0, 0, 0, 0, 0, 0, 0, 0, 0, 153, 0, 0,
    0, 0, 0, 0, 0, 0, 0, 0, 0, 0, 0, 0, 0, 0, 0, 0, 0, 0, 0, 0, 0, 0, 0, 0, 0, 0, 0, 0, 0, 0, 0, 0, 0, 0, 0, 138, 0, 0, 0, 0, 0, 0, 0, 0, 0, 210, 0, 0, 0, 0, 0, 0, 0, 0, 0, 0, 0, 0, 0, 0, 0, 0, 225, 0,
    0, 0, 0, 0, 0, 0, 0, 0, 0, 0, 0, 0, 0, 0, 0, 0, 0, 0, 0, 179, 0, 0, 0, 0, 0, 0, 0, 0, 0, 0, 0, 0, 0, 0, 0, 0, 0, 0, 162, 0, 208, 0, 0, 221, 0, 0, 0, 0, 0, 0, 0, 0, 0, 252, 0, 0, 0, 0, 0, 0, 0, 0, 0, 0,
    0, 0, 0, 0, 0, 0, 0, 0, 0, 0, 0, 126, 0, 0, 0, 0, 0, 0, 152, 0, 0, 0, 0, 0, 0, 0, 0, 0, 0, 0, 0, 0, 0, 0, 0, 0, 0, 0, 0, 0, 0, 0, 0, 0, 0, 0, 0, 0, 0, 0, 0, 0, 0, 0, 0, 0, 24, 0, 0, 0, 0, 0, 0, 254,
    0, 0, 0, 0, 0, 0, 0, 0, 0, 0, 0, 0, 0, 0, 0, 0, 0, 0, 0, 0, 0, 124, 0, 0, 0, 0, 0, 0, 0, 0, 93, 0, 0, 0, 80, 0, 34, 0, 0, 0, 0, 0, 0, 0, 0, 0, 0, 0, 0, 0, 0, 0, 0, 0, 0, 51, 0, 0, 0, 0, 0, 0, 0, 0,
    0, 0, 0, 0, 0, 0, 0, 0, 0, 0, 0, 0, 97, 0, 0, 0, 0, 0, 0, 0, 0, 0, 0, 0, 0, 0, 0, 0, 0, 82, 0, 0, 0, 0, 0, 0, 0, 0, 0, 10, 0, 0, 0, 0, 0, 0, 0, 0, 0, 0, 0, 0, 0, 0, 0, 0, 0, 0, 0, 0, 0, 0, 0, 0,
    0, 0, 0, 0, 0, 0, 0, 0, 0, 0, 0, 0, 0, 25, 0, 0, 0, 0, 0, 0, 0, 0, 0, 0, 0, 0, 0, 0, 0, 0, 0, 0, 0, 0, 0, 0, 0, 0, 0, 185, 0, 0, 0, 0, 0, 0, 0, 0, 0, 0, 0, 0, 0, 0, 0, 0, 0, 0, 0, 0, 0, 0, 0, 0,
    0, 0, 0, 0, 0, 0, 0, 0, 0, 0, 0, 0, 0, 0, 0, 0, 12, 0, 0, 0, 0, 0, 0, 0, 0, 0, 171, 0, 0, 0, 0, 111, 0, 0, 0, 0, 0, 0, 0, 0, 0, 0, 0, 0, 0, 0, 0, 0, 0, 0, 0, 0, 0, 0, 236, 0, 0, 0, 0, 0, 0, 0, 0, 0,
    128, 0, 0, 0, 0, 0, 0, 0, 0, 0, 249, 0, 0, 0, 0, 0, 0, 0, 0, 0, 0, 0, 0, 0, 0, 0, 0, 0, 0, 0, 0, 0, 0, 0, 0, 0, 0, 0, 0, 0, 0, 0, 0, 0, 0, 148, 0, 0, 0, 0, 0, 0, 0, 0, 0, 4, 0, 0, 0, 0, 0, 0, 0, 0};
  static constexpr uint32_t SQRT_G[4][256][8] = {{{0x4ffffffbu, 0xac96341cu, 0x9f60cd29u, 0x36fc7695u, 0x7879462eu, 0x666ea36fu, 0x9a07df2fu, 0x0e0a77c1u},
     {0x584bb683u, 0x89bcc016u, 0x0164a50cu, 0xe8d9887fu, 0x795eda3du, 0x755e95cbu, 0x1323b130u, 0x0f572b87u},
     {0x2c80552bu, 0x9b457955u, 0xe04e7089u, 0x5821ebc4u, 0x2f55cc8du, 0x052c529fu, 0x8e3fa253u, 0x2d2ec870u},
     {0x40f181c0u, 0x88831878u, 0x20a88556u, 0x5b566b92u, 0x094ed9f3u, 0x22be6aa8u, 0xcb99841cu, 0x2418aa1du},
     {0x70784d69u, 0xf90ad83du, 0x90089c33u, 0xc98f3964u, 0x6a63be44u, 0x538bf7a4u, 0xcf5c3c58u, 0x1f2fab5cu},
     {0xa4999d8cu, 0xf8d5b996u, 0xaf24872au, 0xe648af41u, 0x68b86ec6u, 0xad89d877u, 0xddfd330bu, 0x123fde36u},
// ... 1965 lines not shown
     {0x88a17b2eu, 0x55a5c605u, 0x6f0c3c44u, 0x89bee2edu, 0xc3bf6d14u, 0x9a86d958u, 0xd6e52a01u, 0x147e8408u},
     {0x125d6166u, 0x11da29b6u, 0x5389b195u, 0xb069b2a2u, 0xd1277a24u, 0x7ad23dd6u, 0xae748ed2u, 0x1dbb3113u},
     {0xf18fe85du, 0x2afb6941u, 0x7d30c7a9u, 0xa232d596u, 0xb85d1d74u, 0x8f5037e6u, 0x327dcc45u, 0x1ad7d437u},
     {0x3d3d77b3u, 0xc3220f74u, 0x9d27e646u, 0x79381f8bu, 0x5605077fu, 0x22826e20u, 0xa6c5fc20u, 0x0485ca17u},
     {0x7e6f742du, 0xff139de2u, 0xfbe9b5edu, 0x53082d40u, 0x5b8040a0u, 0xcc68c6a0u, 0x01504a4du, 0x2686a41du},
     {0x9edcef8bu, 0x7f753d97u, 0xb1479120u, 0x5f3f172cu, 0x74096c6eu, 0x8db16279u, 0x39c108cfu, 0x2b377b35u},
     {0xec34858cu, 0x32a90d93u, 0x2752e561u, 0xda7ff528u, 0x34e8faa9u, 0x4e60e34bu, 0xd50f7643u, 0x1e6b62e0u},
     {0xe9165b90u, 0x8042a523u, 0x7a4fa0a3u, 0x8b264098u, 0xdeea9bf9u, 0x49c6df3cu, 0x3c2ea1a5u, 0x2c39d29eu},
     {0x77787d38u, 0xc3b18587u, 0xfc35e7f3u, 0xa3fa2ac3u, 0x1706fed7u, 0x9f18932du, 0x2a30c91bu, 0x1e6b47bfu},
     {0xb5ad7c3fu, 0xf8ad4ae2u, 0x83cb85beu, 0x2d60c6ffu, 0x5d9429f7u, 0xd976fd2bu, 0x3f9ad9a9u, 0x24407ce7u},
     {0xd15f7f3cu, 0xda48ceb3u, 0x7a115a15u, 0xdc339055u, 0x70faaa61u, 0xb8581e48u, 0xe1f911b7u, 0x15c2087eu},
     {0x742f8f03u, 0xf4b67d7cu, 0x63d068ccu, 0x681b2ddcu, 0x1bfb576au, 0x8ce5bcefu, 0xd2b63cfeu, 0x167c2951u},
     {0xbf574c64u, 0x2214f7b1u, 0xf7317df2u, 0x28f9232fu, 0xb0ad75cdu, 0xe57584a8u, 0xdc176d03u, 0x2b81fb59u},
     {0x4ffffffbu, 0xac96341cu, 0x9f60cd29u, 0x36fc7695u, 0x7879462eu, 0x666ea36fu, 0x9a07df2fu, 0x0e0a77c1u},
     {0x001fcfb4u, 0x283ae711u, 0xfeb4f32au, 0x05ead253u, 0xfa1144cau, 0xcbc338abu, 0xdb78fc8eu, 0x300e4c10u},
     {0xa5d2b60eu, 0x302fa787u, 0xb54036b7u, 0x80cc914fu, 0xd235eb3bu, 0x4f65c0b3u, 0x5108a15eu, 0x0adb1208u},
     {0x675e84d3u, 0xee3c2f8eu, 0x0aad344cu, 0x9e75055bu, 0xbdc1eb48u, 0x1dc96c5du, 0x0a4c7628u, 0x1be5ca6au},
     {0xdda29e9bu, 0x3207cbddu, 0x262fbefcu, 0x77ca35a6u, 0xb059de38u, 0x3d7e07dfu, 0x32bd1157u, 0x12a91d5fu},
     {0xfe7017a4u, 0x18e68c51u, 0xfc88a8e8u, 0x860112b1u, 0xc9243ae8u, 0x29000dcfu, 0xaeb3d3e4u, 0x158c7a3bu},
     {0xb2c2884eu, 0x80bfe61fu, 0xdc918a4au, 0xaefbc8bcu, 0x2b7c50ddu, 0x95cdd796u, 0x3a6ba409u, 0x2bde845bu},
     {0x71908bd4u, 0x44ce57b1u, 0x7dcfbaa3u, 0xd52bbb07u, 0x260117bcu, 0xebe77f16u, 0xdfe155dbu, 0x09ddaa55u},
     {0x51231076u, 0xc46cb7fcu, 0xc871df70u, 0xc8f4d11bu, 0x0d77ebeeu, 0x2a9ee33du, 0xa770975au, 0x052cd33du},
     {0x03cb7a75u, 0x1138e800u, 0x52668b30u, 0x4db3f320u, 0x4c985db3u, 0x69ef626bu, 0x0c2229e6u, 0x11f8eb92u},
     {0x06e9a471u, 0xc39f5070u, 0xff69cfedu, 0x9d0da7afu, 0xa296bc63u, 0x6e896679u, 0xa502fe84u, 0x042a7bd4u},
     {0x788782c9u, 0x8030700cu, 0x7d83889du, 0x8439bd84u, 0x6a7a5985u, 0x1937b289u, 0xb700d70eu, 0x11f906b3u},
     {0x3a5283c2u, 0x4b34aab1u, 0xf5edead2u, 0xfad32148u, 0x23ed2e65u, 0xded9488bu, 0xa196c67fu, 0x0c23d18bu},
     {0x1ea080c5u, 0x699926e0u, 0xffa8167bu, 0x4c0057f2u, 0x1086adfbu, 0xfff8276eu, 0xff388e71u, 0x1aa245f3u},
     {0x7bd070feu, 0x4f2b7817u, 0x15e907c4u, 0xc018ba6cu, 0x658600f2u, 0x2b6a88c7u, 0x0e7b632bu, 0x19e82521u},
     {0x30a8b39du, 0x21ccfde2u, 0x8287f29fu, 0xff3ac518u, 0xd0d3e28fu, 0xd2dac10du, 0x051a3325u, 0x04e25319u},
     {0xa0000006u, 0x974bc177u, 0xda58a367u, 0xf13771b2u, 0x0908122eu, 0x51e1a247u, 0x4729c0fau, 0x2259d6b1u},
     {0xefe0304du, 0x1ba70e82u, 0x7b047d67u, 0x224915f4u, 0x87701393u, 0xec8d0d0au, 0x05b8a39au, 0x00560262u},
     {0x4a2d49f3u, 0x13b24e0cu, 0xc47939dau, 0xa76756f8u, 0xaf4b6d21u, 0x68ea8502u, 0x9028fecbu, 0x25893c6au},
     {0x88a17b2eu, 0x55a5c605u, 0x6f0c3c44u, 0x89bee2edu, 0xc3bf6d14u, 0x9a86d958u, 0xd6e52a01u, 0x147e8408u},
     {0x125d6166u, 0x11da29b6u, 0x5389b195u, 0xb069b2a2u, 0xd1277a24u, 0x7ad23dd6u, 0xae748ed2u, 0x1dbb3113u},
     {0xf18fe85du, 0x2afb6941u, 0x7d30c7a9u, 0xa232d596u, 0xb85d1d74u, 0x8f5037e6u, 0x327dcc45u, 0x1ad7d437u},
     {0x3d3d77b3u, 0xc3220f74u, 0x9d27e646u, 0x79381f8bu, 0x5605077fu, 0x22826e20u, 0xa6c5fc20u, 0x0485ca17u},
     {0x7e6f742du, 0xff139de2u, 0xfbe9b5edu, 0x53082d40u, 0x5b8040a0u, 0xcc68c6a0u, 0x01504a4du, 0x2686a41du},
     {0x9edcef8bu, 0x7f753d97u, 0xb1479120u, 0x5f3f172cu, 0x74096c6eu, 0x8db16279u, 0x39c108cfu, 0x2b377b35u},
     {0xec34858cu, 0x32a90d93u, 0x2752e561u, 0xda7ff528u, 0x34e8faa9u, 0x4e60e34bu, 0xd50f7643u, 0x1e6b62e0u},
     {0xe9165b90u, 0x8042a523u, 0x7a4fa0a3u, 0x8b264098u, 0xdeea9bf9u, 0x49c6df3cu, 0x3c2ea1a5u, 0x2c39d29eu},
     {0x77787d38u, 0xc3b18587u, 0xfc35e7f3u, 0xa3fa2ac3u, 0x1706fed7u, 0x9f18932du, 0x2a30c91bu, 0x1e6b47bfu},
     {0xb5ad7c3fu, 0xf8ad4ae2u, 0x83cb85beu, 0x2d60c6ffu, 0x5d9429f7u, 0xd976fd2bu, 0x3f9ad9a9u, 0x24407ce7u},
     {0xd15f7f3cu, 0xda48ceb3u, 0x7a115a15u, 0xdc339055u, 0x70faaa61u, 0xb8581e48u, 0xe1f911b7u, 0x15c2087eu},
     {0x742f8f03u, 0xf4b67d7cu, 0x63d068ccu, 0x681b2ddcu, 0x1bfb576au, 0x8ce5bcefu, 0xd2b63cfeu, 0x167c2951u},
     {0xbf574c64u, 0x2214f7b1u, 0xf7317df2u, 0x28f9232fu, 0xb0ad75cdu, 0xe57584a8u, 0xdc176d03u, 0x2b81fb59u},
     {0x4ffffffbu, 0xac96341cu, 0x9f60cd29u, 0x36fc7695u, 0x7879462eu, 0x666ea36fu, 0x9a07df2fu, 0x0e0a77c1u},
     {0x001fcfb4u, 0x283ae711u, 0xfeb4f32au, 0x05ead253u, 0xfa1144cau, 0xcbc338abu, 0xdb78fc8eu, 0x300e4c10u},
     {0xa5d2b60eu, 0x302fa787u, 0xb54036b7u, 0x80cc914fu, 0xd235eb3bu, 0x4f65c0b3u, 0x5108a15eu, 0x0adb1208u},
     {0x675e84d3u, 0xee3c2f8eu, 0x0aad344cu, 0x9e75055bu, 0xbdc1eb48u, 0x1dc96c5du, 0x0a4c7628u, 0x1be5ca6au},
     {0xdda29e9bu, 0x3207cbddu, 0x262fbefcu, 0x77ca35a6u, 0xb059de38u, 0x3d7e07dfu, 0x32bd1157u, 0x12a91d5fu},
     {0xfe7017a4u, 0x18e68c51u, 0xfc88a8e8u, 0x860112b1u, 0xc9243ae8u, 0x29000dcfu, 0xaeb3d3e4u, 0x158c7a3bu},
     {0xb2c2884eu, 0x80bfe61fu, 0xdc918a4au, 0xaefbc8bcu, 0x2b7c50ddu, 0x95cdd796u, 0x3a6ba409u, 0x2bde845bu},
     {0x71908bd4u, 0x44ce57b1u, 0x7dcfbaa3u, 0xd52bbb07u, 0x260117bcu, 0xebe77f16u, 0xdfe155dbu, 0x09ddaa55u},
     {0x51231076u, 0xc46cb7fcu, 0xc871df70u, 0xc8f4d11bu, 0x0d77ebeeu, 0x2a9ee33du, 0xa770975au, 0x052cd33du},
     {0x03cb7a75u, 0x1138e800u, 0x52668b30u, 0x4db3f320u, 0x4c985db3u, 0x69ef626bu, 0x0c2229e6u, 0x11f8eb92u},
     {0x06e9a471u, 0xc39f5070u, 0xff69cfedu, 0x9d0da7afu, 0xa296bc63u, 0x6e896679u, 0xa502fe84u, 0x042a7bd4u},
     {0x788782c9u, 0x8030700cu, 0x7d83889du, 0x8439bd84u, 0x6a7a5985u, 0x1937b289u, 0xb700d70eu, 0x11f906b3u},
     {0x3a5283c2u, 0x4b34aab1u, 0xf5edead2u, 0xfad32148u, 0x23ed2e65u, 0xded9488bu, 0xa196c67fu, 0x0c23d18bu},
     {0x1ea080c5u, 0x699926e0u, 0xffa8167bu, 0x4c0057f2u, 0x1086adfbu, 0xfff8276eu, 0xff388e71u, 0x1aa245f3u},
     {0x7bd070feu, 0x4f2b7817u, 0x15e907c4u, 0xc018ba6cu, 0x658600f2u, 0x2b6a88c7u, 0x0e7b632bu, 0x19e82521u},
     {0x30a8b39du, 0x21ccfde2u, 0x8287f29fu, 0xff3ac518u, 0xd0d3e28fu, 0xd2dac10du, 0x051a3325u, 0x04e25319u},
     {0xa0000006u, 0x974bc177u, 0xda58a367u, 0xf13771b2u, 0x0908122eu, 0x51e1a247u, 0x4729c0fau, 0x2259d6b1u},
     {0xefe0304du, 0x1ba70e82u, 0x7b047d67u, 0x224915f4u, 0x87701393u, 0xec8d0d0au, 0x05b8a39au, 0x00560262u},
     {0x4a2d49f3u, 0x13b24e0cu, 0xc47939dau, 0xa76756f8u, 0xaf4b6d21u, 0x68ea8502u, 0x9028fecbu, 0x25893c6au},
     {0x88a17b2eu, 0x55a5c605u, 0x6f0c3c44u, 0x89bee2edu, 0xc3bf6d14u, 0x9a86d958u, 0xd6e52a01u, 0x147e8408u},
     {0x125d6166u, 0x11da29b6u, 0x5389b195u, 0xb069b2a2u, 0xd1277a24u, 0x7ad23dd6u, 0xae748ed2u, 0x1dbb3113u},
     {0xf18fe85du, 0x2afb6941u, 0x7d30c7a9u, 0xa232d596u, 0xb85d1d74u, 0x8f5037e6u, 0x327dcc45u, 0x1ad7d437u},
     {0x3d3d77b3u, 0xc3220f74u, 0x9d27e646u, 0x79381f8bu, 0x5605077fu, 0x22826e20u, 0xa6c5fc20u, 0x0485ca17u},
     {0x7e6f742du, 0xff139de2u, 0xfbe9b5edu, 0x53082d40u, 0x5b8040a0u, 0xcc68c6a0u, 0x01504a4du, 0x2686a41du},
     {0x9edcef8bu, 0x7f753d97u, 0xb1479120u, 0x5f3f172cu, 0x74096c6eu, 0x8db16279u, 0x39c108cfu, 0x2b377b35u},
     {0xec34858cu, 0x32a90d93u, 0x2752e561u, 0xda7ff528u, 0x34e8faa9u, 0x4e60e34bu, 0xd50f7643u, 0x1e6b62e0u},
     {0xe9165b90u, 0x8042a523u, 0x7a4fa0a3u, 0x8b264098u, 0xdeea9bf9u, 0x49c6df3cu, 0x3c2ea1a5u, 0x2c39d29eu},
     {0x77787d38u, 0xc3b18587u, 0xfc35e7f3u, 0xa3fa2ac3u, 0x1706fed7u, 0x9f18932du, 0x2a30c91bu, 0x1e6b47bfu},
     {0xb5ad7c3fu, 0xf8ad4ae2u, 0x83cb85beu, 0x2d60c6ffu, 0x5d9429f7u, 0xd976fd2bu, 0x3f9ad9a9u, 0x24407ce7u},
     {0xd15f7f3cu, 0xda48ceb3u, 0x7a115a15u, 0xdc339055u, 0x70faaa61u, 0xb8581e48u, 0xe1f911b7u, 0x15c2087eu},
     {0x742f8f03u, 0xf4b67d7cu, 0x63d068ccu, 0x681b2ddcu, 0x1bfb576au, 0x8ce5bcefu, 0xd2b63cfeu, 0x167c2951u},
     {0xbf574c64u, 0x2214f7b1u, 0xf7317df2u, 0x28f9232fu, 0xb0ad75cdu, 0xe57584a8u, 0xdc176d03u, 0x2b81fb59u}}};
};
struct FrBabyJubJub {
  static constexpr int N = 8;
  static constexpr uint32_t P[8] = {0x392126f1u, 0x677297dcu, 0x3920ee0au, 0xab3eedb8u, 0xd0302b0bu, 0x370a08b6u, 0x5c263405u, 0x060c89ceu};
  static constexpr uint32_t ONE[8] = {0xa08f9c76u, 0x073315deu, 0xa098f24bu, 0xe7acffc6u, 0xd818f015u, 0xf85a9201u, 0xe1bb7724u, 0x01f16424u};
  static constexpr uint32_t R2[8] = {0xe7ecb21eu, 0x35e44abeu, 0xf5f84ec4u, 0x74646cacu, 0x3faa158fu, 0xe472df20u, 0xf1ba50a8u, 0x0445b524u};
  static constexpr uint32_t HALF[8] = {0x1c909378u, 0x33b94beeu, 0x1c907705u, 0xd59f76dcu, 0x68181585u, 0x9b85045bu, 0x2e131a02u, 0x030644e7u};
  static constexpr uint32_t NINV = 0xbc48f5efu;
  static constexpr int BITS = 251;
  static constexpr bool FULL = false;
  static constexpr int TWO_ADICITY = 4;
  static constexpr uint32_t T_MINUS1_HALF[8] = {0xe1c90937u, 0x533b94beu, 0xc1c90770u, 0x5d59f76du, 0xb6818158u, 0x29b85045u, 0x72e131a0u, 0x0030644eu};
  static constexpr uint32_t ROOT[8] = {0x9b1974efu, 0x2fb01b00u, 0x5eb3e91au, 0x723c0b73u, 0xf0533decu, 0x341f16b7u, 0x09cf7bc1u, 0x04edaec3u};
  static constexpr uint32_t PM2[8] = {0x392126efu, 0x677297dcu, 0x3920ee0au, 0xab3eedb8u, 0xd0302b0bu, 0x370a08b6u, 0x5c263405u, 0x060c89ceu};
};
struct FrJubJub {
  static constexpr int N = 8;
  static constexpr uint32_t P[8] = {0xd6f72cb7u, 0xd0970e5eu, 0xccc81082u, 0xa6682093u, 0x01343b00u, 0x06673b01u, 0x6533afa9u, 0x0e7db4eau};
  static constexpr uint32_t ONE[8] = {0xb99607d9u, 0x25f80bb3u, 0x66b6e750u, 0xf315d62fu, 0xeb8814f4u, 0x932514eeu, 0x479155c6u, 0x09a6fc6fu};
  static constexpr uint32_t R2[8] = {0x95e57731u, 0x67719aa4u, 0x9ce3fc26u, 0x51b0cef0u, 0xc026e9a5u, 0x69dab7fau, 0x8d127688u, 0x04f6547bu};
  static constexpr uint32_t HALF[8] = {0x6b7b965bu, 0x684b872fu, 0xe6640841u, 0x53341049u, 0x809a1d80u, 0x83339d80u, 0x3299d7d4u, 0x073eda75u};
  static constexpr uint32_t NINV = 0xef788ef9u;
  static constexpr int BITS = 252;
  static constexpr bool FULL = false;
  static constexpr int TWO_ADICITY = 1;
  static constexpr uint32_t T_MINUS1_HALF[8] = {0xb5bdcb2du, 0xb425c397u, 0xf3320420u, 0x299a0824u, 0x404d0ec0u, 0x4199cec0u, 0x994cebeau, 0x039f6d3au};
  static constexpr uint32_t ROOT[8] = {0x1d6124deu, 0xaa9f02abu, 0x66112932u, 0xb3524a64u, 0x15ac260bu, 0x73422612u, 0x1da259e2u, 0x04d6b87bu};
  static constexpr uint32_t PM2[8] = {0xd6f72cb5u, 0xd0970e5eu, 0xccc81082u, 0xa6682093u, 0x01343b00u, 0x06673b01u, 0x6533afa9u, 0x0e7db4eau};
};
struct FqEd25519 {
  static constexpr int N = 8;
  static constexpr uint32_t P[8] = {0xffffffedu, 0xffffffffu, 0xffffffffu, 0xffffffffu, 0xffffffffu, 0xffffffffu, 0xffffffffu, 0x7fffffffu};
  static constexpr uint32_t ONE[8] = {0x00000026u, 0x00000000u, 0x00000000u, 0x00000000u, 0x00000000u, 0x00000000u, 0x00000000u, 0x00000000u};
  static constexpr uint32_t R2[8] = {0x000005a4u, 0x00000000u, 0x00000000u, 0x00000000u, 0x00000000u, 0x00000000u, 0x00000000u, 0x00000000u};
  static constexpr uint32_t HALF[8] = {0xfffffff6u, 0xffffffffu, 0xffffffffu, 0xffffffffu, 0xffffffffu, 0xffffffffu, 0xffffffffu, 0x3fffffffu};
  static constexpr uint32_t NINV = 0x286bca1bu;
  static constexpr int BITS = 255;
  static constexpr bool FULL = false;
  static constexpr int TWO_ADICITY = 2;
  static constexpr uint32_t T_MINUS1_HALF[8] = {0xfffffffdu, 0xffffffffu, 0xffffffffu, 0xffffffffu, 0xffffffffu, 0xffffffffu, 0xffffffffu, 0x0fffffffu};
  static constexpr uint32_t ROOT[8] = {0xfe2bdb04u, 0x3b5807d4u, 0xb51be9edu, 0x03f590fdu, 0x336202d1u, 0x6d6e16bfu, 0xd6c71ba8u, 0x75776b0bu};
  static constexpr uint32_t PM2[8] = {0xffffffebu, 0xffffffffu, 0xffffffffu, 0xffffffffu, 0xffffffffu, 0xffffffffu, 0xffffffffu, 0x7fffffffu};
  static constexpr int SQRT_W = 8;
  static constexpr int SQRT_HW = 2;
  static constexpr int SQRT_STEPS = 1;
  static constexpr int SQRT_HBITS = 6;
  static constexpr uint32_t SQRT_HMUL = 0x73b5e9f7u;
  static constexpr uint8_t SQRT_HIDX[64] = {0, 0, 0, 0, 0, 0, 0, 0, 0, 0, 0, 0, 0, 0, 0, 2, 0, 0, 0, 0, 0, 0, 0, 0, 0, 0, 0, 0, 0, 0, 0, 0, 0, 0, 0, 0, 0, 0, 0, 3, 0, 0, 0, 0, 0, 0, 0, 0, 0, 0, 0, 1, 0, 0, 0, 0, 0, 0, 0, 0, 0, 0, 0, 0};
  static constexpr uint32_t SQRT_G[1][4][8] = {{{0x00000026u, 0x00000000u, 0x00000000u, 0x00000000u, 0x00000000u, 0x00000000u, 0x00000000u, 0x00000000u},
     {0x01d424e9u, 0xc4a7f82bu, 0x4ae41612u, 0xfc0a6f02u, 0xcc9dfd2eu, 0x9291e940u, 0x2938e457u, 0x0a8894f4u},
     {0xffffffc7u, 0xffffffffu, 0xffffffffu, 0xffffffffu, 0xffffffffu, 0xffffffffu, 0xffffffffu, 0x7fffffffu},
     {0xfe2bdb04u, 0x3b5807d4u, 0xb51be9edu, 0x03f590fdu, 0x336202d1u, 0x6d6e16bfu, 0xd6c71ba8u, 0x75776b0bu}}};
  static constexpr uint32_t SQRT_GH[1][4][8] = {{{0x00000026u, 0x00000000u, 0x00000000u, 0x00000000u, 0x00000000u, 0x00000000u, 0x00000000u, 0x00000000u},
     {0x00000000u, 0x00000000u, 0x00000000u, 0x00000000u, 0x00000000u, 0x00000000u, 0x00000000u, 0x00000000u},
     {0x01d424e9u, 0xc4a7f82bu, 0x4ae41612u, 0xfc0a6f02u, 0xcc9dfd2eu, 0x9291e940u, 0x2938e457u, 0x0a8894f4u},
     {0x00000000u, 0x00000000u, 0x00000000u, 0x00000000u, 0x00000000u, 0x00000000u, 0x00000000u, 0x00000000u}}};
};
struct FrEd25519 {
  static constexpr int N = 8;
  static constexpr uint32_t P[8] = {0x5cf5d3edu, 0x5812631au, 0xa2f79cd6u, 0x14def9deu, 0x00000000u, 0x00000000u, 0x00000000u, 0x10000000u};
  static constexpr uint32_t ONE[8] = {0x8d98951du, 0xd6ec3174u, 0x737dcf70u, 0xc6ef5bf4u, 0xfffffffeu, 0xffffffffu, 0xffffffffu, 0x0fffffffu};
  static constexpr uint32_t R2[8] = {0x449c0f01u, 0xa40611e3u, 0x68859347u, 0xd00e1ba7u, 0x17f5be65u, 0xceec73d2u, 0x7c309a3du, 0x0399411bu};
  static constexpr uint32_t HALF[8] = {0x2e7ae9f6u, 0x2c09318du, 0x517bce6bu, 0x0a6f7cefu, 0x00000000u, 0x00000000u, 0x00000000u, 0x08000000u};
  static constexpr uint32_t NINV = 0x12547e1bu;
  static constexpr int BITS = 253;
  static constexpr bool FULL = false;
  static constexpr int TWO_ADICITY = 2;
  static constexpr uint32_t T_MINUS1_HALF[8] = {0x4b9eba7du, 0xcb024c63u, 0xd45ef39au, 0x029bdf3bu, 0x00000000u, 0x00000000u, 0x00000000u, 0x02000000u};
  static constexpr uint32_t ROOT[8] = {0xb42f0e7du, 0x7c790e32u, 0xa7ae2cc8u, 0x4c8ce706u, 0x921779adu, 0xd73823ccu, 0x893f562au, 0x05599959u};
  static constexpr uint32_t PM2[8] = {0x5cf5d3ebu, 0x5812631au, 0xa2f79cd6u, 0x14def9deu, 0x00000000u, 0x00000000u, 0x00000000u, 0x10000000u};
};
struct FqSecp256r1 {
  static constexpr int N = 8;
  static constexpr uint32_t P[8] = {0xffffffffu, 0xffffffffu, 0xffffffffu, 0x00000000u, 0x00000000u, 0x00000000u, 0x00000001u, 0xffffffffu};
  static constexpr uint32_t ONE[8] = {0x00000001u, 0x00000000u, 0x00000000u, 0xffffffffu, 0xffffffffu, 0xffffffffu, 0xfffffffeu, 0x00000000u};
  static constexpr uint32_t R2[8] = {0x00000003u, 0x00000000u, 0xffffffffu, 0xfffffffbu, 0xfffffffeu, 0xffffffffu, 0xfffffffdu, 0x00000004u};
  static constexpr uint32_t HALF[8] = {0xffffffffu, 0xffffffffu, 0x7fffffffu, 0x00000000u, 0x00000000u, 0x80000000u, 0x80000000u, 0x7fffffffu};
  static constexpr uint32_t NINV = 0x00000001u;
  static constexpr int BITS = 256;
  static constexpr bool FULL = true;
  static constexpr int TWO_ADICITY = 1;
  static constexpr uint32_t T_MINUS1_HALF[8] = {0xffffffffu, 0xffffffffu, 0x3fffffffu, 0x00000000u, 0x00000000u, 0x40000000u, 0xc0000000u, 0x3fffffffu};
  static constexpr uint32_t ROOT[8] = {0xfffffffeu, 0xffffffffu, 0xffffffffu, 0x00000001u, 0x00000000u, 0x00000000u, 0x00000002u, 0xfffffffeu};
  static constexpr uint32_t PM2[8] = {0xfffffffdu, 0xffffffffu, 0xffffffffu, 0x00000000u, 0x00000000u, 0x00000000u, 0x00000001u, 0xffffffffu};
  static constexpr int SQRT_W = 8;
  static constexpr int SQRT_HW = 1;
  static constexpr int SQRT_STEPS = 1;
  static constexpr int SQRT_HBITS = 5;
  static constexpr uint32_t SQRT_HMUL = 0xd8266debu;
  static constexpr uint8_t SQRT_HIDX[32] = {0, 0, 0, 0, 0, 0, 0, 0, 0, 1, 0, 0, 0, 0, 0, 0, 0, 0, 0, 0, 0, 0, 0, 0, 0, 0, 0, 0, 0, 0, 0, 0};
  static constexpr uint32_t SQRT_G[1][2][8] = {{{0x00000001u, 0x00000000u, 0x00000000u, 0xffffffffu, 0xffffffffu, 0xffffffffu, 0xfffffffeu, 0x00000000u},
     {0xfffffffeu, 0xffffffffu, 0xffffffffu, 0x00000001u, 0x00000000u, 0x00000000u, 0x00000002u, 0xfffffffeu}}};
  static constexpr uint32_t SQRT_GH[1][2][8] = {{{0x00000001u, 0x00000000u, 0x00000000u, 0xffffffffu, 0xffffffffu, 0xffffffffu, 0xfffffffeu, 0x00000000u},
     {0x00000000u, 0x00000000u, 0x00000000u, 0x00000000u, 0x00000000u, 0x00000000u, 0x00000000u, 0x00000000u}}};
};
struct FrSecp256r1 {
  static constexpr int N = 8;
  static constexpr uint32_t P[8] = {0xfc632551u, 0xf3b9cac2u, 0xa7179e84u, 0xbce6faadu, 0xffffffffu, 0xffffffffu, 0x00000000u, 0xffffffffu};
  static constexpr uint32_t ONE[8] = {0x039cdaafu, 0x0c46353du, 0x58e8617bu, 0x43190552u, 0x00000000u, 0x00000000u, 0xffffffffu, 0x00000000u};
  static constexpr uint32_t R2[8] = {0xbe79eea2u, 0x83244c95u, 0x49bd6fa6u, 0x4699799cu, 0x2b6bec59u, 0x2845b239u, 0xf3d95620u, 0x66e12d94u};
  static constexpr uint32_t HALF[8] = {0x7e3192a8u, 0x79dce561u, 0xd38bcf42u, 0xde737d56u, 0xffffffffu, 0x7fffffffu, 0x80000000u, 0x7fffffffu};
  static constexpr uint32_t NINV = 0xee00bc4fu;
  static constexpr int BITS = 256;
  static constexpr bool FULL = true;
  static constexpr int TWO_ADICITY = 4;
  static constexpr uint32_t T_MINUS1_HALF[8] = {0x17e3192au, 0x279dce56u, 0x6d38bcf4u, 0xfde737d5u, 0xffffffffu, 0x07ffffffu, 0xf8000000u, 0x07ffffffu};
  static constexpr uint32_t ROOT[8] = {0x7e368fe1u, 0x1015708fu, 0x6ecc4511u, 0x31c6c545u, 0x98a19ea1u, 0x5281fe89u, 0x10c63fe8u, 0x0279089eu};
  static constexpr uint32_t PM2[8] = {0xfc63254fu, 0xf3b9cac2u, 0xa7179e84u, 0xbce6faadu, 0xffffffffu, 0xffffffffu, 0x00000000u, 0xffffffffu};
};
struct FqBls12381 {
  static constexpr int N = 12;
  static constexpr uint32_t P[12] = {0xffffaaabu, 0xb9feffffu, 0xb153ffffu, 0x1eabfffeu, 0xf6b0f624u, 0x6730d2a0u, 0xf38512bfu, 0x64774b84u, 0x434bacd7u, 0x4b1ba7b6u, 0x397fe69au, 0x1a0111eau};
  static constexpr uint32_t ONE[12] = {0x0002fffdu, 0x76090000u, 0xc40c0002u, 0xebf4000bu, 0x53c758bau, 0x5f489857u, 0x70525745u, 0x77ce5853u, 0xa256ec6du, 0x5c071a97u, 0xfa80e493u, 0x15f65ec3u};
  static constexpr uint32_t R2[12] = {0x1c341746u, 0xf4df1f34u, 0x09d104f1u, 0x0a76e6a6u, 0x4c95b6d5u, 0x8de5476cu, 0x939d83c0u, 0x67eb88a9u, 0xb519952du, 0x9a793e85u, 0x92cae3aau, 0x11988fe5u};
  static constexpr uint32_t HALF[12] = {0xffffd555u, 0xdcff7fffu, 0x58a9ffffu, 0x0f55ffffu, 0x7b587b12u, 0xb3986950u, 0x79c2895fu, 0xb23ba5c2u, 0x21a5d66bu, 0x258dd3dbu, 0x1cbff34du, 0x0d0088f5u};
  static constexpr uint32_t PM2[12] = {0xffffaaa9u, 0xb9feffffu, 0xb153ffffu, 0x1eabfffeu, 0xf6b0f624u, 0x6730d2a0u, 0xf38512bfu, 0x64774b84u, 0x434bacd7u, 0x4b1ba7b6u, 0x397fe69au, 0x1a0111eau};
  static constexpr uint32_t NINV = 0xfffcfffdu;
  static constexpr int BITS = 381;
  static constexpr bool FULL = false;
};
struct FqBn254 {
  static constexpr int N = 8;
  static constexpr uint32_t P[8] = {0xd87cfd47u, 0x3c208c16u, 0x6871ca8du, 0x97816a91u, 0x8181585du, 0xb85045b6u, 0xe131a029u, 0x30644e72u};
  static constexpr uint32_t ONE[8] = {0xc58f0d9du, 0xd35d438du, 0xf5c70b3du, 0x0a78eb28u, 0x7879462cu, 0x666ea36fu, 0x9a07df2fu, 0x0e0a77c1u};
  static constexpr uint32_t R2[8] = {0x538afa89u, 0xf32cfc5bu, 0xd44501fbu, 0xb5e71911u, 0x0a417ff6u, 0x47ab1effu, 0xcab8351fu, 0x06d89f71u};
  static constexpr uint32_t HALF[8] = {0x6c3e7ea3u, 0x9e10460bu, 0xb438e546u, 0xcbc0b548u, 0x40c0ac2eu, 0xdc2822dbu, 0x7098d014u, 0x18322739u};
  static constexpr uint32_t PM2[8] = {0xd87cfd45u, 0x3c208c16u, 0x6871ca8du, 0x97816a91u, 0x8181585du, 0xb85045b6u, 0xe131a029u, 0x30644e72u};
  static constexpr uint32_t NINV = 0xe4866389u;
  static constexpr int BITS = 254;
  static constexpr bool FULL = false;
};
struct G1Bls12381 { using Fq = FqBls12381; using Fr = FqBandersnatch;
  static constexpr uint32_t B[12] = {0x000cfff3u, 0xaa270000u, 0xfc34000au, 0x53cc0032u, 0x6b0a807fu, 0x478fe97au, 0xe6ba24d7u, 0xb1d37ebeu, 0xbf78ab2fu, 0x8ec9733bu, 0x3d83de7eu, 0x09d64551u};
  static constexpr int TWO_ADICITY = 32;
  static constexpr uint32_t ROOT_OF_UNITY[8] = {0x5f0e466au, 0xb9b58d8cu, 0x1819d7ecu, 0x5b1b4c80u, 0x52a31e64u, 0x0af53ae3u, 0x19e9b27bu, 0x5bf3addau};
  static constexpr int XI0 = 1;  static constexpr bool MTWIST = true;
  static constexpr int ATE_LOOP_BITS = 64;
  static constexpr uint64_t ATE_LOOP[1] = {0xd201000000010000ULL};
  static constexpr int FINAL_EXP_BITS = 4314;
  static constexpr uint64_t FINAL_EXP[68] = {0xc0bcb9b55df57510ULL, 0x25f98630e68bfb24ULL, 0x4406fbc8fbd5f489ULL, 0x8e2f8491d12191a0ULL, 0x3e9d71650a6f8069ULL, 0x226c2f011d4cab80ULL, 0x67f67c4717489119ULL, 0xaf3f881bd88592d7ULL, 0x1a67e49eeed2161dULL, 0xe5b78c7869aeb218ULL, 0xf6539314043f7bbcULL, 0x73f62537f2701aaeULL, 0xaff1c910e9622d2aULL, 0x6283313492caa9d4ULL, 0x2e2f3ec2bea83d19ULL, 0xa4c7e79fb02faa73ULL, 0x6c49637fd7961be1ULL, 0x08e88adce8817745ULL, 0x35de3f7a36399917ULL, 0x9c1d9f7c31759c36ULL, 0xfa9e13c24ea820b0ULL, 0x3fc56947a403577dULL, 0xa4c1b6dcfc5cceb7ULL, 0x1bbd81367066bca6ULL, 0x0418a3ef0bc62775ULL, 0x49bf9b71a9f9e010ULL, 0x511291097db60b17ULL, 0x498345c6e5308f1cULL, 0x6d8823b19dadd7c2ULL, 0x92004cedd556952cULL, 0x4c6bec3ec03ef195ULL, 0x0a1fad20044ce6adULL, 0xc55d3109cd15948dULL, 0x334f46c02c3f0bd0ULL, 0x3b5a62eb34c05739ULL, 0x724538411d1676a5ULL, 0x127a1b5ad0463434ULL, 0x61a474c5c85b0129ULL, 0x8dfc8e2886ef965eULL, 0x96532fef459f1243ULL, 0x40ee7169cdc10412ULL, 0x9c40a68eb74bb22aULL, 0x25118790f4684d0bULL, 0x596bc293c8d4c01fULL, 0x1064837f27611212ULL, 0x077ffb10bf24dde4ULL, 0xc49f570bcd2b01f3ULL, 0x1a0c5bf24c374693ULL, 0x350da5359bc73ab6ULL, 0xd2670d93e4d7acddULL, 0xd39099b86e1ab656ULL, 0x19328148978e2b0dULL, 0xb113f414386b0e88ULL, 0x07a0dce2630d9aa4ULL, 0xa927e7bb93753318ULL, 0xe347aa68ad49466fULL, 0x1c0ad0d6106feaf4ULL, 0xc872ee83ff3a0f0fULL, 0x074e43b9a660835cULL, 0xc0aadff5e9cfee9aULL, 0x30698e8cc7deada9ULL, 0xd1073776ab353f2cULL, 0x17848517badc3a43ULL, 0x7363baa13f8d14a9ULL, 0xd4977b3f7d4507d0ULL, 0x496a1c0a89ee0193ULL, 0xdcc825b7e1bda9c0ULL, 0x0000000002ee1db5ULL};
  static constexpr int HARD_EXP_BITS = 1268;
  static constexpr uint64_t HARD_EXP[20] = {0xe516c3f438e3ba79ULL, 0xfa9912aae208ccf1ULL, 0x905ce937335d5b68ULL, 0xc71a2629b0dea236ULL, 0x83774940996754c8ULL, 0x21d160aeb6a1e799ULL, 0x2ed0b283ed237db4ULL, 0x915c97f36c6f1821ULL, 0x67f17fcbde783765ULL, 0x2378b9039096d1b7ULL, 0x7988f8761bdc51dcULL, 0x2076995003fc77a1ULL, 0x827eca0ba621315bULL, 0xe5a72bce8d63cb9fULL, 0xf68f7764c28b6f8aULL, 0x2f230063cf081517ULL, 0x94506632528d6a9aULL, 0xd3cde88eeb996ca3ULL, 0xc0bd38c3195c899eULL, 0x000f686b3d807d01ULL};
  static constexpr uint32_t FROB2_GAMMA[12] = {0x798dba3au, 0xecfb361bu, 0x91865a2cu, 0xc100ddb8u, 0x232bda8eu, 0x0ec08ff1u, 0xf1ca4721u, 0xd5c13cc6u, 0xbf7b5c04u, 0x47222a47u, 0xe51c5f59u, 0x0110f184u};
  static constexpr uint32_t FROB1_GAMMA[5][2][12] = {{{0xb319d465u, 0x07089552u, 0xb50a8313u, 0xc6695f92u, 0xd117228fu, 0x97e83cccu, 0xb2dc29eeu, 0xa35baecau, 0x5daace4du, 0x1ce393eau, 0xb0fb66ebu, 0x08f2220fu}, {0x4ce5d646u, 0xb2f66aadu, 0xfc497cecu, 0x5842a06bu, 0x2599d394u, 0xcf4895d4u, 0x40a8e8d0u, 0xc11b9cbau, 0xe5a0de89u, 0x2e3813cbu, 0x88847fafu, 0x110eefdau}}, {{0x00000000u, 0x00000000u, 0x00000000u, 0x00000000u, 0x00000000u, 0x00000000u, 0x00000000u, 0x00000000u, 0x00000000u, 0x00000000u, 0x00000000u, 0x00000000u}, {0x8671f071u, 0xcd03c9e4u, 0x1fcda5d2u, 0x5dab2246u, 0xd3851b95u, 0x587042afu, 0x01bacb9eu, 0x8eb60ebeu, 0x83d050d2u, 0x03f97d6eu, 0x54638741u, 0x18f02065u}}, {{0x5aa30fdau, 0x7bcfa7a2u, 0x2a927e7cu, 0xdc17dec1u, 0x6b4ebef1u, 0x2f088dd8u, 0xda74d4a7u, 0xd1ca2087u, 0x96cebc1du, 0x2da25966u, 0xbbfd87d2u, 0x0e2b7eedu}, {0x5aa30fdau, 0x7bcfa7a2u, 0x2a927e7cu, 0xdc17dec1u, 0x6b4ebef1u, 0x2f088dd8u, 0xda74d4a7u, 0xd1ca2087u, 0x96cebc1du, 0x2da25966u, 0xbbfd87d2u, 0x0e2b7eedu}}, {{0x867545c3u, 0x890dc9e4u, 0x3285a5d5u, 0x2af32253u, 0x309b7e2cu, 0x50880866u, 0x7e881024u, 0xa20d1b8cu, 0xe2db9068u, 0x14e4f04fu, 0x1564853au, 0x14e56d3fu}, {0x00000000u, 0x00000000u, 0x00000000u, 0x00000000u, 0x00000000u, 0x00000000u, 0x00000000u, 0x00000000u, 0x00000000u, 0x00000000u, 0x00000000u, 0x00000000u}}, {{0x0dbce43fu, 0x82d83cf5u, 0xdf9d018fu, 0xa2813e53u, 0x3c65e181u, 0xc6f0caa5u, 0x8d50fe95u, 0x7525cf52u, 0xf4798a6bu, 0x4a85ed50u, 0x6cf8eebdu, 0x171da0fdu}, {0xf242c66cu, 0x3726c30au, 0xd1b6fe70u, 0x7c2ac1aau, 0xba4b14a2u, 0xa04007fbu, 0x66341429u, 0xef517c32u, 0x4ed2226bu, 0x0095ba65u, 0xcc86f7ddu, 0x02e370ecu}}};
  static constexpr bool X_CHAIN = true;
  static constexpr uint64_t X_ABS = 0xd201000000010000ULL;  static constexpr bool X_NEG = true;
};
struct G1Bn254 { using Fq = FqBn254; using Fr = FqBabyJubJub;
  static constexpr uint32_t B[8] = {0x50ad28d7u, 0x7a17caa9u, 0xe15521b9u, 0x1f6ac17au, 0x696bd284u, 0x334bea4eu, 0xce179d8eu, 0x2a1f6744u};
  static constexpr int TWO_ADICITY = 28;
  static constexpr uint32_t ROOT_OF_UNITY[8] = {0x80d13d9cu, 0x636e7355u, 0x2445ffd6u, 0xa22bf374u, 0x1eb203d8u, 0x56452ac0u, 0x2963f9e7u, 0x1860ef94u};
  static constexpr int XI0 = 9;  static constexpr bool MTWIST = false;
  static constexpr int ATE_LOOP_BITS = 127;
  static constexpr uint64_t ATE_LOOP[2] = {0xf83e9682e87cfd46ULL, 0x6f4d8248eeb859fbULL};
  static constexpr int FINAL_EXP_BITS = 2790;
  static constexpr uint64_t FINAL_EXP[44] = {0x86964b64ca86f120ULL, 0x40a4efb7e54523a4ULL, 0x837fa97896e84abbULL, 0x361102b6b9b2b918ULL, 0xc0de81def35692daULL, 0xbe04c7e8a6c3c760ULL, 0xd766f9c9d570bb7fULL, 0xc230974d83561841ULL, 0x5bba1668c3be69a3ULL, 0x7f3811c410526294ULL, 0x29baee7ddadda71cULL, 0xbf813b8d145da900ULL, 0x641bbadf423f9a2cULL, 0xa80bb4ea44eacc5eULL, 0xcd65664814fde37cULL, 0x4a0364b9580291d2ULL, 0xee93dfb10826f0ddULL, 0x6b42db8dc5514724ULL, 0xbb10cf430b0f3785ULL, 0x40494e406f804216ULL, 0x55cfe107acf3aafbULL, 0x2088ec80e0ebae87ULL, 0x846a3ed011a337a0ULL, 0x48a45a4a1e3a5195ULL, 0xe5664568dfc50e16ULL, 0xab6a41294c0cc4ebULL, 0x82d0d602d268c7daULL, 0x6668449aed3cc48aULL, 0x5062cd0fb2015dfcULL, 0x7f2940a8b1ddb3d1ULL, 0x77f5b63a2a226448ULL, 0xfef0781361e443aeULL, 0xf977870e88d5c6c8ULL, 0x790364a61f676baaULL, 0x5887e72eceaddea3ULL, 0x1377e563a09a1b70ULL, 0x0c54efee1bd8c3b2ULL, 0x3ec3d15ad524d8f7ULL, 0xdaf15466b2383a5dULL, 0xe1e30a73bb94fec0ULL, 0x6a1c71015f3f7be2ULL, 0x842d43bf6369b1ffULL, 0x20fddadf107d20bcULL, 0x0000002f4b6dc970ULL};
  static constexpr int HARD_EXP_BITS = 761;
  static constexpr uint64_t HARD_EXP[12] = {0xe81bb482ccdf42b1ULL, 0x5abf5cc4f49c36d4ULL, 0xf1154e7e1da014fdULL, 0xdcc7b44c87cdbacfULL, 0xaaa441e3954bcf8aULL, 0x6b887d56d5095f23ULL, 0x79581e16f3fd90c6ULL, 0x3b1b1355d189227dULL, 0x4e529a5861876f6bULL, 0x6c0eb522d5b12278ULL, 0x331ec15183177fafULL, 0x01baaa710b0759adULL};
  static constexpr uint32_t FROB2_GAMMA[8] = {0x00fa1bf2u, 0xca8d8005u, 0x68b39769u, 0xf0c5d614u, 0xad0d4418u, 0x0e201271u, 0xbad856e6u, 0x04290f65u};
  static constexpr uint32_t FROB1_GAMMA[5][2][8] = {{{0x33144907u, 0xaf9ba696u, 0x87afb78au, 0xca6b1d73u, 0xf08a2087u, 0x11bded5eu, 0x1a1f3a7cu, 0x02f34d75u}, {0x4c492d72u, 0xa222ae23u, 0x565de15bu, 0xd00f02a4u, 0x53dfc926u, 0xdc2ff3a2u, 0xb3899551u, 0x10a75716u}}, {{0x4563ab30u, 0xb5773b10u, 0xa9aa6454u, 0x347f91c8u, 0x242e0991u, 0x7a007127u, 0x118214ecu, 0x1956bcd8u}, {0xa0aa4757u, 0x6e849f1eu, 0x89f89141u, 0xaa1c7b6du, 0xfae0ca3au, 0xb6e713cdu, 0x4e82ebc3u, 0x26694fbbu}}, {{0x2936b629u, 0xe4bbdd0cu, 0xe133bacbu, 0xbb30f162u, 0xf9645366u, 0x31a9d1b6u, 0xa500f8ddu, 0x253570beu}, {0x5ffe77c7u, 0xa1d77ce4u, 0x7826d1dbu, 0x07affd11u, 0xbb7edc6bu, 0x6d16bd27u, 0x85defeccu, 0x2c872002u}}, {{0x843abe92u, 0x7361d77fu, 0x273411fbu, 0xa5bb2bd3u, 0x4b3e2399u, 0x9c941f31u, 0xbb9fd3ecu, 0x15df9cddu}, {0x4bd8c949u, 0x5dddfd15u, 0xa4445b60u, 0x62cb29a5u, 0x0c7dd2b9u, 0x37bc870au, 0x3171f0fdu, 0x24830a9du}}, {{0x41690fe7u, 0xc970692fu, 0x27694b0bu, 0xe2403421u, 0x83c459e8u, 0x32bee66bu, 0x0ab08841u, 0x12aabcedu}, {0x40aebfa9u, 0x0d485d23u, 0xab2fcc57u, 0x05193418u, 0x8a4910f5u, 0xd3b0a40bu, 0x35d2925au, 0x2f21ebb5u}}};
  static constexpr bool X_CHAIN = false;
  static constexpr uint64_t X_ABS = 0x44e992b44a6909f1ULL;  static constexpr bool X_NEG = false;
};

struct SuiteBandersnatch {
  using Fq = FqBandersnatch; using Fr = FrBandersnatch;
  static constexpr int SUITE_ID_LEN = 27;
  static constexpr uint8_t SUITE_ID[27] = {66, 97, 110, 100, 101, 114, 115, 110, 97, 116, 99, 104, 45, 83, 72, 65, 53, 49, 50, 45, 69, 76, 76, 50, 45, 118, 49};
  static constexpr int ID = 0;
  static constexpr int A_KIND = 1;
  static constexpr int COFACTOR = 4;
  static constexpr uint32_t D[8] = {0x47a2c730u, 0xa8dced1bu, 0xad3cccc7u, 0x381c065au, 0x188351f8u, 0x53ff52e1u, 0x990fe940u, 0x362e8d63u};
  static constexpr uint32_t G_X[8] = {0xe7ab47f5u, 0xec2627e1u, 0x4f01aa9cu, 0x3e63de48u, 0x53946dc4u, 0xfe0f5c3bu, 0xaeb2cfcdu, 0x2d71920bu};
  static constexpr uint32_t G_Y[8] = {0x1895bd34u, 0x4e30593eu, 0x32afbe4bu, 0x156d738fu, 0xcdeb75f4u, 0x45ef0b1cu, 0x37d2e71fu, 0x6a7cca00u};
  static constexpr uint32_t G_K[8] = {0xf12d8aa9u, 0x5584000au, 0x322f4e62u, 0x677dfd79u, 0x1827d548u, 0x938b881cu, 0xd6a47261u, 0x70e1e5b8u};
  static constexpr uint32_t G_C[8] = {0xcc974166u, 0x5e3167b6u, 0xeee46460u, 0x358cad81u, 0xbadcd586u, 0x157d8b50u, 0xda123e0fu, 0x2a6c669eu};
  static constexpr uint32_t B_X[8] = {0x20054b92u, 0x27a0004du, 0x0d409892u, 0x56329e1cu, 0x3f1c21ccu, 0x3177b2ffu, 0x68009400u, 0x6f3653aeu};
  static constexpr uint32_t B_Y[8] = {0x050fb6c3u, 0x541cf21cu, 0x3aec196du, 0xf3149537u, 0x91577d02u, 0x5f39f2a0u, 0x521cc3fau, 0x437d00b6u};
  static constexpr uint32_t B_K[8] = {0xcb686fd8u, 0xefc75d35u, 0xb774cfc3u, 0x5be10999u, 0x8a24d14bu, 0xcf9d892cu, 0x6a095cc4u, 0x5176b204u};
  static constexpr uint32_t B_C[8] = {0x820a2debu, 0x0e79c759u, 0x39ab0950u, 0x700c6797u, 0xed65088cu, 0x305fec14u, 0xb6f24d5fu, 0x0c46712cu};
  static constexpr uint32_t ACC_X[8] = {0xbb60f130u, 0xec45dcd4u, 0x99232bc0u, 0x56d2b42eu, 0x14aa00cau, 0x588c5d8fu, 0x9dceb6b4u, 0x3d8ef509u};
  static constexpr uint32_t ACC_Y[8] = {0x9ba8386eu, 0xab8740a2u, 0x0cafb70du, 0xee1df029u, 0xff82d9bau, 0x99cba184u, 0x5bd5562bu, 0x49e1ac24u};
  static constexpr uint32_t ACC_K[8] = {0xe00865c6u, 0x336712dau, 0xb512b9f2u, 0x8e7937bcu, 0x10e6a730u, 0x99038e54u, 0x0031ff1bu, 0x4e862715u};
// ... 327 lines not shown
```

### ark_vrf_amd/csrc/proto_dev.h

```cpp
#pragma once
#include "sha512_dev.h"
#include "shake_dev.h"
#include "sha256_dev.h"
#include "te.h"
#include <type_traits>

#define fp_mul fp_mul_nf
#define fp_sqr fp_sqr_nf
#define fp_inv fp_inv_nf
#define fp_to_mont fp_to_mont_nf
#define fp_from_mont fp_from_mont_nf
#define fp_is_negative_mont fp_is_negative_mont_nf
#define fp_from_wide_mont fp_from_wide_mont_nf
#define te_to_aff te_to_aff_nf
#define te_make_pre te_make_pre_nf
#include "sw_map.h"
#include "fpu_te.h"

namespace avrf {

enum : uint8_t {
  DS_TINY = 0x00, DS_THIN = 0x01, DS_PEDERSEN = 0x02, DS_NONCE_EXPAND = 0x10, DS_NONCE = 0x11, DS_PEDERSEN_BLINDING = 0x12,
  DS_POINT_TO_HASH = 0x20, DS_DELINEARIZE = 0x30, DS_CHALLENGE = 0x40, DS_BATCH_VERIFY = 0x50
};
// ... 11 lines not shown
  const te_pre *fixed;
  uint8_t *records;
  const uint8_t *weights;
  te_ext *tabs;
  uint32_t first;
};
struct Seed64 { uint64_t w[8]; };
template <class S> using suite_tr = std::conditional_t<S::XOF_SHAKE, Shake128, std::conditional_t<S::TR_SHA256, Sha256, Sha512>>;

template <class S, class T> AVRF_DI void absorb_point_xy(T &h, const fp &x, const fp &y) {
  using Fq = typename S::Fq;
  if constexpr (S::SW_CODEC) {
    absorb_sw_enc(h, sw_encode_te<S>(fp_to_mont<Fq>(x), fp_to_mont<Fq>(y)));
    return;
  }
  uint32_t sign = fp_is_negative_plain<Fq>(x) ? 0x80000000u : 0u;
#pragma unroll
  for (int i = 0; i < 8; i++) tr_u32le(h, y.v[i] | (i == 7 ? sign : 0u));
}
template <class T> AVRF_DI void absorb_sw_enc(T &h, const sw_enc &e) {
#pragma unroll
  for (int i = 0; i < 8; i++) tr_u32le(h, e.x.v[i]);
  tr_byte(h, e.flag);
}
template <class S, class T> AVRF_DI void absorb_generator(T &h) {
  for (int i = 0; i < S::POINT_LEN; i++) tr_byte(h, S::G_ENC[i]);
}
template <class T> AVRF_DI void absorb_fp_le(T &h, const fp &a) {
#pragma unroll
  for (int i = 0; i < 8; i++) tr_u32le(h, a.v[i]);
}
template <class S> AVRF_DI uint32_t point_flags(const fp &x, const fp &y) {
  using Fq = typename S::Fq;
  uint32_t f = 0;
  if (ge_p<Fq>(x) || ge_p<Fq>(y)) f |= FLAG_RANGE;
  fp one = fp_zero(); one.v[0] = 1;
  if constexpr (S::SW_NATIVE) { if (fp_is_zero(x) && fp_is_zero(y)) f |= FLAG_IDENTITY; }
  else if (fp_is_zero(x) && fp_eq(y, one)) f |= FLAG_IDENTITY;
  return f;
}

template <class S, class T> AVRF_DI void tr_base(T &h, uint8_t scheme, bool schnorr, const fp &pkx, const fp &pky,
                                        const uint8_t *ios_xy, uint32_t m, const uint8_t *ad, uint32_t adl, uint32_t *flags) {
  tr_init(h);
  for (int i = 0; i < S::SUITE_ID_LEN; i++) tr_byte(h, S::SUITE_ID[i]);
  tr_byte(h, scheme);
  tr_u64le(h, (uint64_t)m + (schnorr ? 1 : 0));
  uint32_t f = 0;
  if constexpr (S::SW_CODEC) if (m == 1) {
    fp xs[3], ys[3]; sw_enc enc[3];
    xs[0] = fp_load_le(ios_xy); ys[0] = fp_load_le(ios_xy + 32); xs[1] = fp_load_le(ios_xy + 64); ys[1] = fp_load_le(ios_xy + 96);
    if (schnorr) { xs[2] = pkx; ys[2] = pky; } else { xs[2] = xs[0]; ys[2] = ys[0]; }
    sw_encode_te_many<S, 3>(xs, ys, enc);
    if (schnorr) { absorb_generator<S>(h); f |= point_flags<S>(xs[2], ys[2]); absorb_sw_enc(h, enc[2]); }
    f |= point_flags<S>(xs[0], ys[0]) | point_flags<S>(xs[1], ys[1]);
    absorb_sw_enc(h, enc[0]); absorb_sw_enc(h, enc[1]);
    tr_u64le(h, (uint64_t)adl);
    tr_bytes(h, ad, adl);
    *flags |= f;
    return;
  }
  if (schnorr) {
    absorb_generator<S>(h);
    f |= point_flags<S>(pkx, pky);
    absorb_point_xy<S>(h, pkx, pky);
  }
  for (uint32_t i = 0; i < m; i++) {
    const uint8_t *p = ios_xy + 128 * (size_t)i;
    fp x = fp_load_le(p), y = fp_load_le(p + 32);
    f |= point_flags<S>(x, y); absorb_point_xy<S>(h, x, y);
    x = fp_load_le(p + 64); y = fp_load_le(p + 96);
    f |= point_flags<S>(x, y); absorb_point_xy<S>(h, x, y);
  }
  tr_u64le(h, (uint64_t)adl);
  tr_bytes(h, ad, adl);
  *flags |= f;
}
template <class S, class T> AVRF_DI void tr_base(T &h, uint8_t scheme, bool schnorr, const uint8_t *pk_xy,
                                        const uint8_t *ios_xy, uint32_t m, const uint8_t *ad, uint32_t adl, uint32_t *flags) {
  fp x = fp_zero(), y = fp_zero();
  if (schnorr) { x = fp_load_le(pk_xy); y = fp_load_le(pk_xy + 32); }
  tr_base<S>(h, scheme, schnorr, x, y, ios_xy, m, ad, adl, flags);
}
template <class T> AVRF_DI auto delin_seed(const T &h) {
  T hd = h; tr_byte(hd, DS_DELINEARIZE); return tr_reader(hd);
}
template <class R> AVRF_DI fp xof128(R &rd, uint32_t i) {
  uint32_t w[4]; rd_chunk16(rd, i, w);
  fp a = fp_zero(); a.v[0] = w[0]; a.v[1] = w[1]; a.v[2] = w[2]; a.v[3] = w[3]; return a;
}
template <class T> AVRF_DI fp challenge_finish(const T &h) {
  auto rd = tr_reader(h); return xof128(rd, 0);
}
template <class T> AVRF_DI void squeeze64(const T &h, fp &lo, fp &hi) {
  auto rd = tr_reader(h);
#pragma unroll
  for (int k = 0; k < 4; k++) {
    uint32_t w[4]; rd_chunk16(rd, (uint32_t)k, w);
    fp &dst = k < 2 ? lo : hi;
#pragma unroll
    for (int i = 0; i < 4; i++) dst.v[4 * (k & 1) + i] = w[i];
  }
}
template <class S, class T> AVRF_DN fp nonce(fp sk_plain, T t) {
  using Fr = typename S::Fr;
  T te = t; tr_byte(te, DS_NONCE_EXPAND); absorb_fp_le(te, sk_plain);
  fp lo, hi;
  squeeze64(te, lo, hi);
  T tn = t; tr_byte(tn, DS_NONCE);
  absorb_fp_le(tn, lo); absorb_fp_le(tn, hi);
  squeeze64(tn, lo, hi);
  static_assert((Fr::BITS + 128 + 7) / 8 == 48, "nonce length");
#pragma unroll
  for (int i = 4; i < 8; i++) hi.v[i] = 0;
  return fp_from_wide_mont<Fr>(lo, hi);
}


template <class S> AVRF_DI te_pre pre_from_xy(const uint8_t *xy) {
  using Fq = typename S::Fq;
  return te_make_pre<S>(fp_to_mont<Fq>(fp_load_le(xy)), fp_to_mont<Fq>(fp_load_le(xy + 32)));
}
template <class S> struct Chain {
#ifndef AVRF_NO_UNSAT_CHAINS
  static constexpr bool U = !S::SW_NATIVE && FuAsm<typename S::Fq>::value;
#else
  static constexpr bool U = false;
#endif
  struct sat_t { te_ext p; };
  using acc_t = std::conditional_t<U, teu4<S>, te_ext>;
  static AVRF_DI acc_t identity() { if constexpr (U) return teu4_identity<S>(); else return te_identity<S>(); }
  static AVRF_DI acc_t dbl(const acc_t &a) { if constexpr (U) return teu4_dbl<S>(a); else return te_dbl<S>(a); }
  template <int N> static AVRF_DI acc_t dbln(acc_t a) {
#pragma unroll 1
    for (int t = 0; t < N; t++) a = dbl(a);
    return a;
  }
  static AVRF_DI acc_t add(const acc_t &a, const te_ext &e) { if constexpr (U) return teu4_add_sat<S>(a, e); else return te_add<S>(a, e); }
  static AVRF_DI acc_t madd(const acc_t &a, const te_pre &q) { if constexpr (U) return teu4_madd_pre<S>(a, q); else return te_madd<S>(a, q); }
  static AVRF_DI te_ext finish(const acc_t &a) { if constexpr (U) return teu4_to_ext<S>(a); else return a; }
};
template <class S> AVRF_DN te_ext te_smul(te_pre p, fp k, int nbits) {
  te_ext tab[16];
  tab[0] = te_identity<S>(); tab[1] = te_from_pre<S>(p);
  for (int i = 2; i < 16; i++) tab[i] = te_madd<S>(tab[i - 1], p);
  using CH = Chain<S>;
  typename CH::acc_t acc = CH::identity();
  for (int w = (nbits + 3) / 4 - 1; w >= 0; w--) {
    acc = CH::template dbln<4>(acc);
    uint32_t d = (k.v[w >> 3] >> (4 * (w & 7))) & 15u;
    if (d) acc = CH::add(acc, tab[d]);
  }
  return CH::finish(acc);
}
enum { ITEM_TAB_SLOTS = 40 };
template <class S> AVRF_DN te_ext te_smul_ws(te_ext *tab, te_pre p, fp k, int nbits) {
  te_ext cur = te_from_pre<S>(p);
  store_ext(tab + 1, cur);
  for (int i = 2; i < 16; i++) { cur = te_madd<S>(cur, p); store_ext(tab + i, cur); }
  using CH = Chain<S>;
  typename CH::acc_t acc = CH::identity();
  for (int w = (nbits + 3) / 4 - 1; w >= 0; w--) {
    const uint32_t d = (k.v[w >> 3] >> (4 * (w & 7))) & 15u;
    te_ext e; if (d) e = load_ext(tab + d);
    acc = CH::template dbln<4>(acc);
    if (d) acc = CH::add(acc, e);
// ... 66 lines not shown
```

### ark_vrf_amd/csrc/sha512_dev.h

```cpp
#pragma once
#include <hip/hip_runtime.h>
#include <stdint.h>

namespace avrf {

#ifndef AVRF_DI
#define AVRF_DI __device__ __forceinline__
#endif

static __device__ __constant__ uint64_t SHA512_K[80] = {
    0x428a2f98d728ae22ULL, 0x7137449123ef65cdULL, 0xb5c0fbcfec4d3b2fULL, 0xe9b5dba58189dbbcULL,
    0x3956c25bf348b538ULL, 0x59f111f1b605d019ULL, 0x923f82a4af194f9bULL, 0xab1c5ed5da6d8118ULL,
    0xd807aa98a3030242ULL, 0x12835b0145706fbeULL, 0x243185be4ee4b28cULL, 0x550c7dc3d5ffb4e2ULL,
    0x72be5d74f27b896fULL, 0x80deb1fe3b1696b1ULL, 0x9bdc06a725c71235ULL, 0xc19bf174cf692694ULL,
    0xe49b69c19ef14ad2ULL, 0xefbe4786384f25e3ULL, 0x0fc19dc68b8cd5b5ULL, 0x240ca1cc77ac9c65ULL,
    0x2de92c6f592b0275ULL, 0x4a7484aa6ea6e483ULL, 0x5cb0a9dcbd41fbd4ULL, 0x76f988da831153b5ULL,
    0x983e5152ee66dfabULL, 0xa831c66d2db43210ULL, 0xb00327c898fb213fULL, 0xbf597fc7beef0ee4ULL,
    0xc6e00bf33da88fc2ULL, 0xd5a79147930aa725ULL, 0x06ca6351e003826fULL, 0x142929670a0e6e70ULL,
    0x27b70a8546d22ffcULL, 0x2e1b21385c26c926ULL, 0x4d2c6dfc5ac42aedULL, 0x53380d139d95b3dfULL,
    0x650a73548baf63deULL, 0x766a0abb3c77b2a8ULL, 0x81c2c92e47edaee6ULL, 0x92722c851482353bULL,
    0xa2bfe8a14cf10364ULL, 0xa81a664bbc423001ULL, 0xc24b8b70d0f89791ULL, 0xc76c51a30654be30ULL,
    0xd192e819d6ef5218ULL, 0xd69906245565a910ULL, 0xf40e35855771202aULL, 0x106aa07032bbd1b8ULL,
    0x19a4c116b8d2d0c8ULL, 0x1e376c085141ab53ULL, 0x2748774cdf8eeb99ULL, 0x34b0bcb5e19b48a8ULL,
    0x391c0cb3c5c95a63ULL, 0x4ed8aa4ae3418acbULL, 0x5b9cca4f7763e373ULL, 0x682e6ff3d6b2b8a3ULL,
// ... 52 lines not shown
        uint64_t s1 = bitop3_64(ror64(w2, 19), ror64(w2, 61), shr64(w2, 6), 0x96);
        w[i] = w[i] + s0 + w[(i + 9) & 15] + s1;
      }
      uint64_t S1 = bitop3_64(ror64(e, 14), ror64(e, 18), ror64(e, 41), 0x96);
      uint64_t ch = bitop3_64(e, f, g, 0xCA);
      uint64_t t1 = hh + S1 + ch + SHA512_K[r + i] + w[i];
      uint64_t S0 = bitop3_64(ror64(a, 28), ror64(a, 34), ror64(a, 39), 0x96);
      uint64_t mj = bitop3_64(a, b, c, 0xE8);
      uint64_t t2 = S0 + mj;
      hh = g; g = f; f = e; e = d + t1; d = c; c = b; b = a; a = t1 + t2;
    }
  }
  ShaH o;
  o.v[0] = hin.v[0] + a; o.v[1] = hin.v[1] + b; o.v[2] = hin.v[2] + c; o.v[3] = hin.v[3] + d;
  o.v[4] = hin.v[4] + e; o.v[5] = hin.v[5] + f; o.v[6] = hin.v[6] + g; o.v[7] = hin.v[7] + hh;
  return o;
}
AVRF_DI void sha512_compress(uint64_t (&h)[8], uint64_t (&w)[16]) {
  ShaH hi; ShaW wi;
#pragma unroll
  for (int i = 0; i < 8; i++) hi.v[i] = h[i];
#pragma unroll
  for (int i = 0; i < 16; i++) wi.v[i] = w[i];
  ShaH o = sha512_compress_nf(hi, wi);
#pragma unroll
  for (int i = 0; i < 8; i++) h[i] = o.v[i];
}

AVRF_DI void sha512_init(Sha512 &s) {
  s.h[0] = 0x6a09e667f3bcc908ULL; s.h[1] = 0xbb67ae8584caa73bULL; s.h[2] = 0x3c6ef372fe94f82bULL; s.h[3] = 0xa54ff53a5f1d36f1ULL;
  s.h[4] = 0x510e527fade682d1ULL; s.h[5] = 0x9b05688c2b3e6c1fULL; s.h[6] = 0x1f83d9abfb41bd6bULL; s.h[7] = 0x5be0cd19137e2179ULL;
#pragma unroll
  for (int i = 0; i < 16; i++) s.w[i] = 0;
  s.fill = 0; s.total = 0;
}

AVRF_DI void sha512_put(Sha512 &s, uint32_t pos, uint8_t b) {
  uint32_t wi = pos >> 3;
  uint64_t v = (uint64_t)b << (56 - 8 * (pos & 7));
#pragma unroll
  for (int i = 0; i < 16; i++) s.w[i] |= (wi == (uint32_t)i) ? v : 0ULL;
}
AVRF_DI void sha512_flush(Sha512 &s) {
  sha512_compress(s.h, s.w);
#pragma unroll
  for (int i = 0; i < 16; i++) s.w[i] = 0;
  s.fill = 0;
}
AVRF_DI void sha512_byte(Sha512 &s, uint8_t b) {
  sha512_put(s, s.fill, b);
  s.fill++; s.total++;
  if (s.fill == 128) sha512_flush(s);
}
AVRF_DI void sha512_bytes(Sha512 &s, const uint8_t *p, uint32_t n) {
  for (uint32_t i = 0; i < n; i++) sha512_byte(s, p[i]);
}
AVRF_DI void sha512_u32le(Sha512 &s, uint32_t v) {
#pragma unroll
  for (int i = 0; i < 4; i++) sha512_byte(s, (uint8_t)(v >> (8 * i)));
}
AVRF_DI void sha512_u64le(Sha512 &s, uint64_t v) { sha512_u32le(s, (uint32_t)v); sha512_u32le(s, (uint32_t)(v >> 32)); }

AVRF_DI void sha512_final(Sha512 s, uint64_t (&out)[8]) {
  uint64_t bits = (uint64_t)s.total * 8;
  sha512_put(s, s.fill, 0x80);
  if (s.fill >= 112) { sha512_flush(s); }
  s.w[15] = bits;
  sha512_compress(s.h, s.w);
#pragma unroll
  for (int i = 0; i < 8; i++) out[i] = s.h[i];
}

AVRF_DI void sha512_xof_block(const uint64_t (&seed)[8], uint64_t counter, uint64_t (&out)[8]) {
  Sha512 s; sha512_init(s);
#pragma unroll
  for (int i = 0; i < 8; i++) s.w[i] = seed[i];
  s.w[8] = __builtin_bswap64(counter);
  s.w[9] = 0x8000000000000000ULL;
  s.w[15] = 72 * 8;
  sha512_compress(s.h, s.w);
#pragma unroll
  for (int i = 0; i < 8; i++) out[i] = s.h[i];
}
AVRF_DI void digest_le128(const uint64_t (&dg)[8], int off16, uint32_t (&w)[4]) {
  uint64_t hi = 0, lo = 0;
#pragma unroll
  for (int i = 0; i < 4; i++) { if (off16 == i) { hi = dg[2 * i]; lo = dg[2 * i + 1]; } }
  uint64_t b0 = __builtin_bswap64(hi), b1 = __builtin_bswap64(lo);
  w[0] = (uint32_t)b0; w[1] = (uint32_t)(b0 >> 32); w[2] = (uint32_t)b1; w[3] = (uint32_t)(b1 >> 32);
}

AVRF_DI void tr_init(Sha512 &s) { sha512_init(s); }
AVRF_DI void tr_byte(Sha512 &s, uint8_t b) { sha512_byte(s, b); }
struct ShaReader { uint64_t seed[8]; uint64_t blk[8]; uint32_t have; };
AVRF_DI ShaReader tr_reader(const Sha512 &s) { ShaReader r; sha512_final(s, r.seed); r.have = 0; return r; }
AVRF_DI void rd_chunk16(ShaReader &r, uint32_t i, uint32_t (&w)[4]) {
  if (r.have != (i >> 2) + 1) { sha512_xof_block(r.seed, i >> 2, r.blk); r.have = (i >> 2) + 1; }
  digest_le128(r.blk, (int)(i & 3), w);
}
AVRF_DI void tr_u32le(Sha512 &s, uint32_t v) {
  if ((s.fill & 3) == 0) {
    const uint64_t x = (uint64_t)__builtin_bswap32(v) << ((s.fill & 4) ? 0 : 32);
    const uint32_t wi = s.fill >> 3;
#pragma unroll
    for (int i = 0; i < 16; i++) s.w[i] |= (wi == (uint32_t)i) ? x : 0ULL;
    s.fill += 4; s.total += 4;
    if (s.fill == 128) sha512_flush(s);
  } else {
#pragma unroll
    for (int i = 0; i < 4; i++) sha512_byte(s, (uint8_t)(v >> (8 * i)));
  }
}
template <class T> AVRF_DI void tr_bytes(T &s, const uint8_t *p, uint32_t n) { for (uint32_t i = 0; i < n; i++) tr_byte(s, p[i]); }
template <class T> AVRF_DI void tr_u32le(T &s, uint32_t v) {
#pragma unroll
  for (int i = 0; i < 4; i++) tr_byte(s, (uint8_t)(v >> (8 * i)));
}
template <class T> AVRF_DI void tr_u64le(T &s, uint64_t v) { tr_u32le(s, (uint32_t)v); tr_u32le(s, (uint32_t)(v >> 32)); }

}
```

### ark_vrf_amd/csrc/vrf_batch.hip

```cpp
#include "vrf_batch.h"
#include "proto_dev.h"
#include "batch_terms_dev.h"
#include "suite_dispatch.h"

#ifndef AVRF_TU_SUITE
#error "vrf_batch.hip is built once per suite: -DAVRF_TU_SUITE=<id> (csrc/Makefile)"
#endif
namespace avrf {

template <class S>
__global__ void __launch_bounds__(128)
k_thin_prepare(BatchDev b, uint32_t *__restrict__ c_out, uint32_t *__restrict__ z_out, uint32_t *__restrict__ flags) {
  using Fr = typename S::Fr;
  uint32_t j = blockIdx.x * blockDim.x + threadIdx.x;
  if (j >= b.n) return;
  uint32_t io0 = b.io_off[j], io1 = b.io_off[j + 1], m = io1 - io0;
  uint32_t ad0 = b.ad_off[j], adl = b.ad_off[j + 1] - ad0;
  uint32_t f = 0;
  suite_tr<S> h; tr_init(h);
  for (int i = 0; i < S::SUITE_ID_LEN; i++) tr_byte(h, S::SUITE_ID[i]);
  tr_byte(h, DS_THIN);
  tr_u64le(h, (uint64_t)m + 1);
  absorb_generator<S>(h);
  sw_enc enc[4]; bool have_enc = false;
  if constexpr (S::SW_CODEC) if (m == 1) {
    const uint8_t *p = b.ios_xy + 128 * (size_t)io0, *pr = b.proofs + 96 * (size_t)j, *pk = b.pks_xy + 64 * (size_t)j;
    const fp xs[4] = {fp_load_le(pk), fp_load_le(p), fp_load_le(p + 64), fp_load_le(pr)};
    const fp ys[4] = {fp_load_le(pk + 32), fp_load_le(p + 32), fp_load_le(p + 96), fp_load_le(pr + 32)};
    sw_encode_te_many<S, 4>(xs, ys, enc); have_enc = true;
  }
  {
    fp x = fp_load_le(b.pks_xy + 64 * (size_t)j), y = fp_load_le(b.pks_xy + 64 * (size_t)j + 32);
    f |= point_flags<S>(x, y);
    if (have_enc) absorb_sw_enc(h, enc[0]); else absorb_point_xy<S>(h, x, y);
  }
  for (uint32_t i = 0; i < m; i++) {
    const uint8_t *p = b.ios_xy + 128 * (size_t)(io0 + i);
    fp x = fp_load_le(p), y = fp_load_le(p + 32);
    f |= point_flags<S>(x, y); if (have_enc) absorb_sw_enc(h, enc[1]); else absorb_point_xy<S>(h, x, y);
    x = fp_load_le(p + 64); y = fp_load_le(p + 96);
    f |= point_flags<S>(x, y); if (have_enc) absorb_sw_enc(h, enc[2]); else absorb_point_xy<S>(h, x, y);
  }
  tr_u64le(h, (uint64_t)adl);
  tr_bytes(h, b.ads + ad0, adl);
  if (m) {
    auto rd = delin_seed(h);
    for (uint32_t i = 0; i < m; i++) {
      uint32_t w[4]; rd_chunk16(rd, i, w);
      uint4 *o = reinterpret_cast<uint4 *>(z_out + 4 * (size_t)(io0 + i));
      *o = make_uint4(w[0], w[1], w[2], w[3]);
    }
  }
  {
    const uint8_t *pr = b.proofs + 96 * (size_t)j;
    fp x = fp_load_le(pr), y = fp_load_le(pr + 32), s = fp_load_le(pr + 64);
    if (point_flags<S>(x, y) & FLAG_RANGE) f |= FLAG_RANGE;
    if (ge_p<Fr>(s)) f |= FLAG_SCALAR;
    tr_byte(h, DS_CHALLENGE);
    if (have_enc) absorb_sw_enc(h, enc[3]); else absorb_point_xy<S>(h, x, y);
    auto rd = tr_reader(h);
    uint32_t w[4]; rd_chunk16(rd, 0, w);
    uint4 *o = reinterpret_cast<uint4 *>(c_out + 4 * (size_t)j);
    *o = make_uint4(w[0], w[1], w[2], w[3]);
    if (b.records) {
      uint4 *r = reinterpret_cast<uint4 *>(b.records + 64 * (size_t)j);
      const uint4 *sp = reinterpret_cast<const uint4 *>(pr + 64);
      r[0] = make_uint4(w[0], w[1], w[2], w[3]); r[1] = make_uint4(0, 0, 0, 0); r[2] = sp[0]; r[3] = sp[1];
    }
  }
  if (f) atomicOr(flags, f);
}

template <class S> struct PlainTerms {
  uint32_t *__restrict__ scalars; te_pre *__restrict__ pre; const uint8_t *__restrict__ pks_xy;
  using Fr = typename S::Fr;
  AVRF_DI void r(uint32_t j, uint32_t io0, const fp &w_plain, const uint8_t *xy) const { emit_term<S>(scalars, pre, 2 * j + 2 * io0, w_plain, xy); }
  AVRF_DI void key(uint32_t j, uint32_t io0, const fp &wc) const { emit_term<S>(scalars, pre, 2 * j + 2 * io0 + 1, fp_from_mont<Fr>(wc), pks_xy + 64 * (size_t)j); }
  AVRF_DI void output(uint32_t j, uint32_t io0, uint32_t i, const fp &sc_plain, const uint8_t *xy) const { emit_term<S>(scalars, pre, 2 * j + 2 * io0 + 2 + 2 * i, sc_plain, xy); }
  AVRF_DI void input(uint32_t j, uint32_t io0, uint32_t i, const fp &sc_mont, const uint8_t *xy) const { emit_term<S>(scalars, pre, 2 * j + 2 * io0 + 3 + 2 * i, fp_from_mont<Fr>(sc_mont), xy); }
};

template <class S>
__global__ void __launch_bounds__(128)
k_thin_terms(BatchDev b, Seed64 seed, uint64_t j0, const uint32_t *__restrict__ c_in, const uint32_t *__restrict__ z_in,
             uint32_t *__restrict__ scalars, te_pre *__restrict__ pre, uint32_t *__restrict__ gpart) {
  using Fr = typename S::Fr;
  __shared__ fp red[128];
  uint32_t j = blockIdx.x * blockDim.x + threadIdx.x;
  fp ws = fp_zero();
  if (j < b.n) ws = thin_item<S>(b, seed, j0, c_in, z_in, j, PlainTerms<S>{scalars, pre, b.pks_xy});
  const fp sum = block_sum<Fr, 128>(ws, red);
  if (threadIdx.x == 0) fp_store(gpart + 8 * (size_t)blockIdx.x, sum);
}

template <class S>
__global__ void __launch_bounds__(256)
k_g_final(const uint32_t *__restrict__ gpart, uint32_t nparts, uint32_t *__restrict__ scalars, te_pre *__restrict__ pre,
          uint32_t t_last, int which_base) {
  __shared__ fp red[256];
  base_term<S>(gpart, nparts, scalars, pre, t_last, which_base, red);
}



template <class S, bool SHARED>
__global__ void __launch_bounds__(128)
k_ped_prepare(BatchDev b, uint32_t *__restrict__ c_out, uint8_t *__restrict__ merged_xy, uint32_t *__restrict__ flags) {
  using Fr = typename S::Fr;
  uint32_t j = blockIdx.x * blockDim.x + threadIdx.x;
  if (j >= b.n) return;
  uint32_t io0 = b.io_off[j], m = b.io_off[j + 1] - io0, ad0 = b.ad_off[j], adl = b.ad_off[j + 1] - ad0;
  const uint8_t *ios = b.ios_xy + 128 * (size_t)io0, *pr = b.proofs + 256 * (size_t)j;
  suite_tr<S> t; uint32_t f = 0;
  tr_base<S>(t, DS_PEDERSEN, false, nullptr, ios, m, b.ads + ad0, adl, &f);
  uint8_t *mo = merged_xy + 128 * (size_t)j;
  if constexpr (SHARED) {
    if (m == 1) {
      const uint4 *src = reinterpret_cast<const uint4 *>(ios + 64); uint4 *dst = reinterpret_cast<uint4 *>(mo + 64);
#pragma unroll
      for (int i = 0; i < 4; i++) dst[i] = src[i];
    } else if (m == 0) {
      fp zero = fp_zero(), one = fp_zero(); one.v[0] = S::SW_NATIVE ? 0 : 1;
      fp_store_le(mo + 64, zero); fp_store_le(mo + 96, one);
    } else {
      auto dseed = delin_seed(t);
      uint32_t *z_out = reinterpret_cast<uint32_t *>(merged_xy + 128 * (size_t)b.n);
      te_ext om = te_identity<S>();
      for (uint32_t i = 0; i < m; i++) {
        te_pre po = pre_from_xy<S>(ios + 128 * (size_t)i + 64);
        if (i == 0) om = te_madd<S>(om, po);
        else {
          fp z = xof128(dseed, i - 1);
          *reinterpret_cast<uint4 *>(z_out + 4 * (size_t)(io0 + i)) = make_uint4(z.v[0], z.v[1], z.v[2], z.v[3]);
          om = te_add<S>(om, te_smul<S>(po, z, 128));
        }
      }
      store_xy<S>(mo + 64, te_to_aff<S>(om));
    }
  } else if (m == 1) {
    const uint4 *src = reinterpret_cast<const uint4 *>(ios); uint4 *dst = reinterpret_cast<uint4 *>(mo);
#pragma unroll
    for (int i = 0; i < 8; i++) dst[i] = src[i];
  } else if (m == 0) {
    fp zero = fp_zero(), one = fp_zero(); one.v[0] = S::SW_NATIVE ? 0 : 1;
    fp_store_le(mo, zero); fp_store_le(mo + 32, one); fp_store_le(mo + 64, zero); fp_store_le(mo + 96, one);
  } else {
    auto dseed = delin_seed(t);
    te_ext im = te_identity<S>(), om = te_identity<S>();
    for (uint32_t i = 0; i < m; i++) {
      te_pre pi = pre_from_xy<S>(ios + 128 * (size_t)i), po = pre_from_xy<S>(ios + 128 * (size_t)i + 64);
      if (i == 0) { im = te_madd<S>(im, pi); om = te_madd<S>(om, po); }
      else { fp z = xof128(dseed, i - 1); im = te_add<S>(im, te_smul<S>(pi, z, 128)); om = te_add<S>(om, te_smul<S>(po, z, 128)); }
    }
    te_aff ia = te_to_aff<S>(im), oa = te_to_aff<S>(om);
    store_xy<S>(mo, ia); store_xy<S>(mo + 64, oa);
  }
  fp ybx = fp_load_le(pr), yby = fp_load_le(pr + 32), rx = fp_load_le(pr + 64), ry = fp_load_le(pr + 96);
  fp okx = fp_load_le(pr + 128), oky = fp_load_le(pr + 160);
  f |= point_flags<S>(ybx, yby);
  f |= (point_flags<S>(rx, ry) | point_flags<S>(okx, oky)) & FLAG_RANGE;
  if (ge_p<Fr>(fp_load_le(pr + 192)) || ge_p<Fr>(fp_load_le(pr + 224))) f |= FLAG_SCALAR;
  if constexpr (S::SW_CODEC) {
    const fp xs[3] = {ybx, rx, okx}, ys[3] = {yby, ry, oky};
    sw_enc enc[3]; sw_encode_te_many<S, 3>(xs, ys, enc);
    absorb_sw_enc(t, enc[0]); tr_byte(t, DS_CHALLENGE); absorb_sw_enc(t, enc[1]); absorb_sw_enc(t, enc[2]);
  } else {
    absorb_point_xy<S>(t, ybx, yby);
    tr_byte(t, DS_CHALLENGE); absorb_point_xy<S>(t, rx, ry); absorb_point_xy<S>(t, okx, oky);
  }
  fp c = challenge_finish(t);
  *reinterpret_cast<uint4 *>(c_out + 4 * (size_t)j) = make_uint4(c.v[0], c.v[1], c.v[2], c.v[3]);
  if (b.records) {
    uint4 *r = reinterpret_cast<uint4 *>(b.records + 96 * (size_t)j);
    const uint4 *sp = reinterpret_cast<const uint4 *>(pr + 192);
    r[0] = make_uint4(c.v[0], c.v[1], c.v[2], c.v[3]); r[1] = make_uint4(0, 0, 0, 0); r[2] = sp[0]; r[3] = sp[1]; r[4] = sp[2]; r[5] = sp[3];
  }
  if (f) atomicOr(flags, f);
}

template <class S> struct PlainPedTerms {
  uint32_t *__restrict__ scalars; te_pre *__restrict__ pre;
  AVRF_DI void term(uint32_t j, uint32_t k, const fp &sc_plain, const uint8_t *xy) const { emit_term<S>(scalars, pre, 5 * j + k, sc_plain, xy); }
};

template <class S>
__global__ void __launch_bounds__(128)
k_ped_terms(BatchDev b, Seed64 seed, uint64_t j0, const uint32_t *__restrict__ c_in, const uint8_t *__restrict__ merged_xy,
            uint32_t *__restrict__ scalars, te_pre *__restrict__ pre, uint32_t *__restrict__ gpart, uint32_t *__restrict__ bpart) {
  using Fr = typename S::Fr;
  __shared__ fp red[128];
  uint32_t j = blockIdx.x * blockDim.x + threadIdx.x;
  fp us = fp_zero(), usb = fp_zero();
  if (j < b.n) us = ped_item<S>(b, seed, j0, c_in, merged_xy, j, PlainPedTerms<S>{scalars, pre}, usb);
  const fp gsum = block_sum<Fr, 128>(us, red);
  if (threadIdx.x == 0) fp_store(gpart + 8 * (size_t)blockIdx.x, gsum);
  __syncthreads();
  const fp bsum = block_sum<Fr, 128>(usb, red);
  if (threadIdx.x == 0) fp_store(bpart + 8 * (size_t)blockIdx.x, bsum);
}

template <class S> void BatchOps<S>::ped_prepare(const BatchDev &b, uint32_t *d_c, uint8_t *d_merged, uint32_t *d_flags, bool shared, hipStream_t st) {
  if (!b.n) return;
  dim3 g((b.n + 127) / 128), blk(128);
  if (shared) hipLaunchKernelGGL((k_ped_prepare<S, true>), g, blk, 0, st, b, d_c, d_merged, d_flags);
  else hipLaunchKernelGGL((k_ped_prepare<S, false>), g, blk, 0, st, b, d_c, d_merged, d_flags);
}
template <class S> void BatchOps<S>::ped_terms(const BatchDev &b, const Seed64 &seed, uint64_t j0, const uint32_t *d_c, const uint8_t *d_merged,
                                               uint32_t *d_scalars, te_pre_raw *d_pre, uint32_t *d_gpart, uint32_t n_terms, hipStream_t st) {
  if (!b.n) return;
  dim3 g((b.n + 127) / 128), blk(128);
  uint32_t *bp = d_gpart + 8 * (size_t)g.x;
  hipLaunchKernelGGL(k_ped_terms<S>, g, blk, 0, st, b, seed, j0, d_c, d_merged, d_scalars, (te_pre *)d_pre, d_gpart, bp);
  hipLaunchKernelGGL(k_g_final<S>, dim3(1), dim3(256), 0, st, d_gpart, g.x, d_scalars, (te_pre *)d_pre, n_terms - 2, 0);
  hipLaunchKernelGGL(k_g_final<S>, dim3(1), dim3(256), 0, st, bp, g.x, d_scalars, (te_pre *)d_pre, n_terms - 1, 1);
}
template <class S> void BatchOps<S>::thin_prepare(const BatchDev &b, uint32_t *d_c, uint32_t *d_z, uint32_t *d_flags, hipStream_t st) {
  if (!b.n) return;
  dim3 g((b.n + 127) / 128), blk(128);
  hipLaunchKernelGGL(k_thin_prepare<S>, g, blk, 0, st, b, d_c, d_z, d_flags);
}
template <class S> void BatchOps<S>::thin_terms(const BatchDev &b, const Seed64 &seed, uint64_t j0, const uint32_t *d_c, const uint32_t *d_z,
                                                uint32_t *d_scalars, te_pre_raw *d_pre, uint32_t *d_gpart, uint32_t n_terms, hipStream_t st) {
  if (!b.n) return;
  dim3 g((b.n + 127) / 128), blk(128);
  hipLaunchKernelGGL(k_thin_terms<S>, g, blk, 0, st, b, seed, j0, d_c, d_z, d_scalars, (te_pre *)d_pre, d_gpart);
  hipLaunchKernelGGL(k_g_final<S>, dim3(1), dim3(256), 0, st, d_gpart, g.x, d_scalars, (te_pre *)d_pre, n_terms - 1, 0);
}
template struct BatchOps<suite_by_id<AVRF_TU_SUITE>::type>;

}
```

Before: 132.0 million.

## Specialize single-IO thin transcript hashing, share weight XOF blocks, drop Montgomery conversions

Adds a single-IO fast path for thin challenge preparation. It pre-bakes the constant transcript prefix into the SHA-512 block and writes point words at compile-time offsets, so there is no byte-by-byte absorption. The terms kernels now compute each SHA-512 XOF weight block once per thread block into LDS and slice per-item weights from it, instead of each thread hashing a full block. Scalar products skip the to-Montgomery and from-Montgomery conversions by multiplying plain values and correcting with R2/R3 constants. The block size grows to 256 threads, which raises LDS use and the width of the reduction.

```diff
diff --git a/ark_vrf_amd/csrc/batch_terms_dev.h b/ark_vrf_amd/csrc/batch_terms_dev.h
--- a/ark_vrf_amd/csrc/batch_terms_dev.h
+++ b/ark_vrf_amd/csrc/batch_terms_dev.h
@@ -25,6 +25,28 @@
   }
   return red[0];
 }
+
+template <int NT, int BYTES> struct WeightBlocks {
+  static_assert(BYTES == 16 || BYTES == 32, "16 bytes per item (thin) or 32 (Pedersen)");
+  static constexpr int MAXB = NT * BYTES / 64 + 1;
+  static constexpr int WORDS = 8 * MAXB;
+  static AVRF_DI void fill(const Seed64 &seed, uint64_t g_first, uint32_t count, uint64_t *lds) {
+    const uint64_t fb = g_first * BYTES / 64, lb = ((g_first + count) * BYTES - 1) / 64;
+    uint32_t nb = count ? (uint32_t)(lb - fb) + 1 : 0;
+    nb = nb < (uint32_t)MAXB ? nb : (uint32_t)MAXB;
+    for (uint32_t k = threadIdx.x; k < nb; k += NT) {
+      uint64_t blk[8]; sha512_xof_block(seed.w, fb + k, blk);
+#pragma unroll
+      for (int i = 0; i < 8; i++) lds[i * MAXB + k] = blk[i];
+    }
+    __syncthreads();
+  }
+  static AVRF_DI void chunk16(const uint64_t *lds, uint64_t g_first, uint64_t g, int c, uint32_t (&w)[4]) {
+    const uint64_t byte = g * BYTES + 16 * (uint64_t)c;
+    const uint32_t k = (uint32_t)(byte / 64 - g_first * BYTES / 64), q = (uint32_t)(byte % 64) / 16;
+    be128_le(lds[(2 * q) * MAXB + k], lds[(2 * q + 1) * MAXB + k], w);
+  }
+};
 
 template <class S, class Out>
 AVRF_DI fp thin_item(const BatchDev &b, const Seed64 &seed, uint64_t j0, const uint32_t *__restrict__ c_in, const uint32_t *__restrict__ z_in,
@@ -54,26 +76,56 @@
 }
 
 template <class S, class Out>
+AVRF_DI fp thin_item_plain(const BatchDev &b, const uint32_t (&ww)[4], const uint32_t *__restrict__ c_in, const uint32_t *__restrict__ z_in,
+                           uint32_t j, const Out &out) {
+  using Fr = typename S::Fr;
+  uint32_t io0 = b.io_off[j], m = b.io_off[j + 1] - io0;
+  fp w_plain = fp_zero(); w_plain.v[0] = ww[0]; w_plain.v[1] = ww[1]; w_plain.v[2] = ww[2]; w_plain.v[3] = ww[3];
+  const fp r2 = fp_const<Fr>(Fr::R2), r3 = fp_const<Fr>(Fr::R3);
+  const uint8_t *pr = b.proofs + 96 * (size_t)j;
+  const fp wc = fp_mul<Fr>(fp_from_u128(c_in + 4 * (size_t)j), w_plain);
+  const fp ws = fp_mul<Fr>(fp_load_le(pr + 64), w_plain);
+  out.r(j, io0, w_plain, pr);
+  out.key(j, io0, fp_mul<Fr>(wc, r2));
+  for (uint32_t i = 0; i < m; i++) {
+    const fp z = fp_from_u128(z_in + 4 * (size_t)(io0 + i));
+    const uint8_t *p = b.ios_xy + 128 * (size_t)(io0 + i);
+    out.output(j, io0, i, fp_mul<Fr>(fp_mul<Fr>(wc, z), r3), p + 64);
+    out.input(j, io0, i, fp_neg<Fr>(fp_mul<Fr>(fp_mul<Fr>(ws, z), r3)), p);
+  }
+  return fp_mul<Fr>(ws, r3);
+}
+
+template <class S, class Out>
+AVRF_DI fp ped_item_w(const BatchDev &b, const fp &t_plain, const fp &u_plain, const uint32_t *__restrict__ c_in,
+                      const uint8_t *__restrict__ merged_xy, uint32_t j, const Out &out, fp &usb);
+
+template <class S, class Out>
 AVRF_DI fp ped_item(const BatchDev &b, const Seed64 &seed, uint64_t j0, const uint32_t *__restrict__ c_in, const uint8_t *__restrict__ merged_xy,
                     uint32_t j, const Out &out, fp &usb) {
-  using Fr = typename S::Fr;
   fp t_plain, u_plain;
   if (b.weights) { t_plain = fp_from_u128(reinterpret_cast<const uint32_t *>(b.weights + 32 * (size_t)j)); u_plain = fp_from_u128(reinterpret_cast<const uint32_t *>(b.weights + 32 * (size_t)j + 16)); }
   else {
     ShaReader rd; for (int i = 0; i < 8; i++) rd.seed[i] = seed.w[i]; rd.have = 0;
     t_plain = xof128(rd, (uint32_t)(2 * (j0 + j))); u_plain = xof128(rd, (uint32_t)(2 * (j0 + j) + 1));
   }
-  fp tt = fp_to_mont<Fr>(t_plain), uu = fp_to_mont<Fr>(u_plain);
-  fp c = fp_to_mont<Fr>(fp_from_u128(c_in + 4 * (size_t)j));
+  return ped_item_w<S>(b, t_plain, u_plain, c_in, merged_xy, j, out, usb);
+}
+template <class S, class Out>
+AVRF_DI fp ped_item_w(const BatchDev &b, const fp &t_plain, const fp &u_plain, const uint32_t *__restrict__ c_in,
+                      const uint8_t *__restrict__ merged_xy, uint32_t j, const Out &out, fp &usb) {
+  using Fr = typename S::Fr;
+  const fp r2 = fp_const<Fr>(Fr::R2), r3 = fp_const<Fr>(Fr::R3);
+  const fp c = fp_from_u128(c_in + 4 * (size_t)j);
   const uint8_t *pr = b.proofs + 256 * (size_t)j, *mo = merged_xy + 128 * (size_t)j;
-  fp s = fp_to_mont<Fr>(fp_load_le(pr + 192)), sb = fp_to_mont<Fr>(fp_load_le(pr + 224));
-  out.term(j, 0, fp_from_mont<Fr>(fp_mul<Fr>(tt, c)), mo + 64);
+  const fp s = fp_load_le(pr + 192), sb = fp_load_le(pr + 224);
+  out.term(j, 0, fp_mul<Fr>(fp_mul<Fr>(c, t_plain), r2), mo + 64);
   out.term(j, 1, t_plain, pr + 128);
-  out.term(j, 2, fp_from_mont<Fr>(fp_neg<Fr>(fp_mul<Fr>(tt, s))), mo);
-  out.term(j, 3, fp_from_mont<Fr>(fp_mul<Fr>(uu, c)), pr);
+  out.term(j, 2, fp_neg<Fr>(fp_mul<Fr>(fp_mul<Fr>(s, t_plain), r2)), mo);
+  out.term(j, 3, fp_mul<Fr>(fp_mul<Fr>(c, u_plain), r2), pr);
   out.term(j, 4, u_plain, pr + 64);
-  const fp us = fp_mul<Fr>(uu, s); usb = fp_mul<Fr>(uu, sb);
-  return us;
+  usb = fp_mul<Fr>(fp_mul<Fr>(sb, u_plain), r3);
+  return fp_mul<Fr>(fp_mul<Fr>(s, u_plain), r3);
 }
 
 template <class S, bool ROLLED = false>
diff --git a/ark_vrf_amd/csrc/consts_gen.h b/ark_vrf_amd/csrc/consts_gen.h
--- a/ark_vrf_amd/csrc/consts_gen.h
+++ b/ark_vrf_amd/csrc/consts_gen.h
@@ -8,6 +8,7 @@
   static constexpr uint32_t P[8] = {0x00000001u, 0xffffffffu, 0xfffe5bfeu, 0x53bda402u, 0x09a1d805u, 0x3339d808u, 0x299d7d48u, 0x73eda753u};
   static constexpr uint32_t ONE[8] = {0xfffffffeu, 0x00000001u, 0x00034802u, 0x5884b7fau, 0xecbc4ff5u, 0x998c4fefu, 0xacc5056fu, 0x1824b159u};
   static constexpr uint32_t R2[8] = {0xf3f29c6du, 0xc999e990u, 0x87925c23u, 0x2b6cedcbu, 0x7254398fu, 0x05d31496u, 0x9f59ff11u, 0x0748d9d9u};
+  static constexpr uint32_t R3[8] = {0x439b73afu, 0xc62c1807u, 0x8cf06990u, 0x1b3e0d18u, 0xc7b5f418u, 0x73d13c71u, 0xc8db33e9u, 0x6e2a5bb9u};
   static constexpr uint32_t HALF[8] = {0x80000000u, 0x7fffffffu, 0x7fff2dffu, 0xa9ded201u, 0x04d0ec02u, 0x199cec04u, 0x94cebea4u, 0x39f6d3a9u};
   static constexpr uint32_t NINV = 0xffffffffu;
   static constexpr int BITS = 255;
@@ -2139,6 +2140,7 @@
   static constexpr uint32_t P[8] = {0x2876e7e1u, 0x74fd06b5u, 0x74190471u, 0xff8f8700u, 0x02687600u, 0x0cce7602u, 0xca675f52u, 0x1cfb69d4u};
   static constexpr uint32_t ONE[8] = {0xbc48c0f8u, 0x5817ca56u, 0x5f37dc74u, 0x0383c7fcu, 0xecbc4ff8u, 0x998c4fefu, 0xacc5056fu, 0x1824b159u};
   static constexpr uint32_t R2[8] = {0x58db47cbu, 0xdbb4f5d6u, 0x7fecb938u, 0x40fa7ca2u, 0xc0055ceau, 0xaa9e6daeu, 0xb14aec7du, 0x0ae793ddu};
+  static constexpr uint32_t R3[8] = {0x79377bd1u, 0x1eb6e3ebu, 0xeddd7769u, 0xb0ce06dau, 0x05341936u, 0x11265871u, 0xf5775113u, 0x053a3b49u};
   static constexpr uint32_t HALF[8] = {0x943b73f0u, 0xba7e835au, 0x3a0c8238u, 0x7fc7c380u, 0x01343b00u, 0x06673b01u, 0x6533afa9u, 0x0e7db4eau};
   static constexpr uint32_t NINV = 0x5cc063dfu;
   static constexpr int BITS = 253;
@@ -2153,6 +2155,7 @@
   static constexpr uint32_t P[8] = {0xf0000001u, 0x43e1f593u, 0x79b97091u, 0x2833e848u, 0x8181585du, 0xb85045b6u, 0xe131a029u, 0x30644e72u};
   static constexpr uint32_t ONE[8] = {0x4ffffffbu, 0xac96341cu, 0x9f60cd29u, 0x36fc7695u, 0x7879462eu, 0x666ea36fu, 0x9a07df2fu, 0x0e0a77c1u};
   static constexpr uint32_t R2[8] = {0xae216da7u, 0x1bb8e645u, 0xe35c59e3u, 0x53fe3ab1u, 0x53bb8085u, 0x8c49833du, 0x7f4e44a5u, 0x0216d0b1u};
+  static constexpr uint32_t R3[8] = {0xb4bf0040u, 0x5e94d8e1u, 0x1cfbb6b8u, 0x2a489cbeu, 0xa19fcfedu, 0x893cc664u, 0x7fcc657cu, 0x0cf8594bu};
   static constexpr uint32_t HALF[8] = {0xf8000000u, 0xa1f0fac9u, 0x3cdcb848u, 0x9419f424u, 0x40c0ac2eu, 0xdc2822dbu, 0x7098d014u, 0x18322739u};
   static constexpr uint32_t NINV = 0xefffffffu;
   static constexpr int BITS = 254;
@@ -4284,6 +4287,7 @@
   static constexpr uint32_t P[8] = {0x392126f1u, 0x677297dcu, 0x3920ee0au, 0xab3eedb8u, 0xd0302b0bu, 0x370a08b6u, 0x5c263405u, 0x060c89ceu};
   static constexpr uint32_t ONE[8] = {0xa08f9c76u, 0x073315deu, 0xa098f24bu, 0xe7acffc6u, 0xd818f015u, 0xf85a9201u, 0xe1bb7724u, 0x01f16424u};
   static constexpr uint32_t R2[8] = {0xe7ecb21eu, 0x35e44abeu, 0xf5f84ec4u, 0x74646cacu, 0x3faa158fu, 0xe472df20u, 0xf1ba50a8u, 0x0445b524u};
+  static constexpr uint32_t R3[8] = {0x42917c21u, 0x30886e7bu, 0x55d7cd2au, 0x98dae87bu, 0xcc608b7bu, 0xeefe3d08u, 0xb2bc97aau, 0x02b4dbffu};
   static constexpr uint32_t HALF[8] = {0x1c909378u, 0x33b94beeu, 0x1c907705u, 0xd59f76dcu, 0x68181585u, 0x9b85045bu, 0x2e131a02u, 0x030644e7u};
   static constexpr uint32_t NINV = 0xbc48f5efu;
   static constexpr int BITS = 251;
@@ -4298,6 +4302,7 @@
   static constexpr uint32_t P[8] = {0xd6f72cb7u, 0xd0970e5eu, 0xccc81082u, 0xa6682093u, 0x01343b00u, 0x06673b01u, 0x6533afa9u, 0x0e7db4eau};
   static constexpr uint32_t ONE[8] = {0xb99607d9u, 0x25f80bb3u, 0x66b6e750u, 0xf315d62fu, 0xeb8814f4u, 0x932514eeu, 0x479155c6u, 0x09a6fc6fu};
   static constexpr uint32_t R2[8] = {0x95e57731u, 0x67719aa4u, 0x9ce3fc26u, 0x51b0cef0u, 0xc026e9a5u, 0x69dab7fau, 0x8d127688u, 0x04f6547bu};
+  static constexpr uint32_t R3[8] = {0x3d830544u, 0xe0d6c656u, 0x598d0f85u, 0x323e3883u, 0x4c2e2ba8u, 0xf0fea300u, 0x946737ecu, 0x05874f84u};
   static constexpr uint32_t HALF[8] = {0x6b7b965bu, 0x684b872fu, 0xe6640841u, 0x53341049u, 0x809a1d80u, 0x83339d80u, 0x3299d7d4u, 0x073eda75u};
   static constexpr uint32_t NINV = 0xef788ef9u;
   static constexpr int BITS = 252;
@@ -4312,6 +4317,7 @@
   static constexpr uint32_t P[8] = {0xffffffedu, 0xffffffffu, 0xffffffffu, 0xffffffffu, 0xffffffffu, 0xffffffffu, 0xffffffffu, 0x7fffffffu};
   static constexpr uint32_t ONE[8] = {0x00000026u, 0x00000000u, 0x00000000u, 0x00000000u, 0x00000000u, 0x00000000u, 0x00000000u, 0x00000000u};
   static constexpr uint32_t R2[8] = {0x000005a4u, 0x00000000u, 0x00000000u, 0x00000000u, 0x00000000u, 0x00000000u, 0x00000000u, 0x00000000u};
+  static constexpr uint32_t R3[8] = {0x0000d658u, 0x00000000u, 0x00000000u, 0x00000000u, 0x00000000u, 0x00000000u, 0x00000000u, 0x00000000u};
   static constexpr uint32_t HALF[8] = {0xfffffff6u, 0xffffffffu, 0xffffffffu, 0xffffffffu, 0xffffffffu, 0xffffffffu, 0xffffffffu, 0x3fffffffu};
   static constexpr uint32_t NINV = 0x286bca1bu;
   static constexpr int BITS = 255;
@@ -4340,6 +4346,7 @@
   static constexpr uint32_t P[8] = {0x5cf5d3edu, 0x5812631au, 0xa2f79cd6u, 0x14def9deu, 0x00000000u, 0x00000000u, 0x00000000u, 0x10000000u};
   static constexpr uint32_t ONE[8] = {0x8d98951du, 0xd6ec3174u, 0x737dcf70u, 0xc6ef5bf4u, 0xfffffffeu, 0xffffffffu, 0xffffffffu, 0x0fffffffu};
   static constexpr uint32_t R2[8] = {0x449c0f01u, 0xa40611e3u, 0x68859347u, 0xd00e1ba7u, 0x17f5be65u, 0xceec73d2u, 0x7c309a3du, 0x0399411bu};
+  static constexpr uint32_t R3[8] = {0x7b83a2dbu, 0x2a9e4968u, 0xaef7f3ecu, 0x278324e6u, 0x04ec5b65u, 0x8065dc6cu, 0x3599cec7u, 0x0e530b77u};
   static constexpr uint32_t HALF[8] = {0x2e7ae9f6u, 0x2c09318du, 0x517bce6bu, 0x0a6f7cefu, 0x00000000u, 0x00000000u, 0x00000000u, 0x08000000u};
   static constexpr uint32_t NINV = 0x12547e1bu;
   static constexpr int BITS = 253;
@@ -4354,6 +4361,7 @@
   static constexpr uint32_t P[8] = {0xffffffffu, 0xffffffffu, 0xffffffffu, 0x00000000u, 0x00000000u, 0x00000000u, 0x00000001u, 0xffffffffu};
   static constexpr uint32_t ONE[8] = {0x00000001u, 0x00000000u, 0x00000000u, 0xffffffffu, 0xffffffffu, 0xffffffffu, 0xfffffffeu, 0x00000000u};
   static constexpr uint32_t R2[8] = {0x00000003u, 0x00000000u, 0xffffffffu, 0xfffffffbu, 0xfffffffeu, 0xffffffffu, 0xfffffffdu, 0x00000004u};
+  static constexpr uint32_t R3[8] = {0x0000000au, 0xfffffffdu, 0xfffffff7u, 0xffffffedu, 0xfffffffcu, 0x00000005u, 0x00000001u, 0x00000018u};
   static constexpr uint32_t HALF[8] = {0xffffffffu, 0xffffffffu, 0x7fffffffu, 0x00000000u, 0x00000000u, 0x80000000u, 0x80000000u, 0x7fffffffu};
   static constexpr uint32_t NINV = 0x00000001u;
   static constexpr int BITS = 256;
@@ -4378,6 +4386,7 @@
   static constexpr uint32_t P[8] = {0xfc632551u, 0xf3b9cac2u, 0xa7179e84u, 0xbce6faadu, 0xffffffffu, 0xffffffffu, 0x00000000u, 0xffffffffu};
   static constexpr uint32_t ONE[8] = {0x039cdaafu, 0x0c46353du, 0x58e8617bu, 0x43190552u, 0x00000000u, 0x00000000u, 0xffffffffu, 0x00000000u};
   static constexpr uint32_t R2[8] = {0xbe79eea2u, 0x83244c95u, 0x49bd6fa6u, 0x4699799cu, 0x2b6bec59u, 0x2845b239u, 0xf3d95620u, 0x66e12d94u};
+  static constexpr uint32_t R3[8] = {0x0b65a624u, 0xac8ebec9u, 0x0c0555c9u, 0x111f28aeu, 0x6ba5e93fu, 0x2543b924u, 0x6407be65u, 0x503a54e7u};
   static constexpr uint32_t HALF[8] = {0x7e3192a8u, 0x79dce561u, 0xd38bcf42u, 0xde737d56u, 0xffffffffu, 0x7fffffffu, 0x80000000u, 0x7fffffffu};
   static constexpr uint32_t NINV = 0xee00bc4fu;
   static constexpr int BITS = 256;
diff --git a/ark_vrf_amd/csrc/proto_dev.h b/ark_vrf_amd/csrc/proto_dev.h
--- a/ark_vrf_amd/csrc/proto_dev.h
+++ b/ark_vrf_amd/csrc/proto_dev.h
@@ -117,6 +117,29 @@
   if (schnorr) { x = fp_load_le(pk_xy); y = fp_load_le(pk_xy + 32); }
   tr_base<S>(h, scheme, schnorr, x, y, ios_xy, m, ad, adl, flags);
 }
+template <class S> struct ThinLayout1 {
+  static constexpr bool OK = !S::SW_CODEC && !S::XOF_SHAKE && !S::TR_SHA256 && S::POINT_LEN == 32;
+  static constexpr int TAG = S::SUITE_ID_LEN, COUNT = TAG + 1, G = COUNT + 8, PK = G + S::POINT_LEN, IN = PK + S::POINT_LEN,
+                       OUT = IN + S::POINT_LEN, ADL = OUT + S::POINT_LEN, END = ADL + 8;
+  static_assert(!OK || PK <= 128, "the literal prefix (suite id, tag, count, generator) lies within the first block");
+  static constexpr ShaLit prefix() {
+    ShaLit l{};
+    for (int i = 0; i < S::SUITE_ID_LEN; i++) sha512_lit_byte(l, i, S::SUITE_ID[i]);
+    sha512_lit_byte(l, TAG, DS_THIN);
+    sha512_lit_byte(l, COUNT, 2);
+    for (int i = 0; i < S::POINT_LEN; i++) sha512_lit_byte(l, G + i, S::G_ENC[i]);
+    return l;
+  }
+};
+static_assert(ThinLayout1<SuiteBandersnatch>::OK && ThinLayout1<SuiteBandersnatch>::PK == 68 && ThinLayout1<SuiteBandersnatch>::IN == 100 &&
+              ThinLayout1<SuiteBandersnatch>::OUT == 132 && ThinLayout1<SuiteBandersnatch>::ADL == 164 && ThinLayout1<SuiteBandersnatch>::END == 172,
+              "Bandersnatch: 27 + 1 + 8 + 4 x 32 + 8 = 172 bytes before the additional data");
+template <class S> AVRF_DI void point_words(const fp &x, const fp &y, uint32_t (&v)[8]) {
+  const uint32_t sign = fp_is_negative_plain<typename S::Fq>(x) ? 0x80000000u : 0u;
+#pragma unroll
+  for (int i = 0; i < 8; i++) v[i] = y.v[i] | (i == 7 ? sign : 0u);
+}
+
 template <class T> AVRF_DI auto delin_seed(const T &h) {
   T hd = h; tr_byte(hd, DS_DELINEARIZE); return tr_reader(hd);
 }
diff --git a/ark_vrf_amd/csrc/sha512_dev.h b/ark_vrf_amd/csrc/sha512_dev.h
--- a/ark_vrf_amd/csrc/sha512_dev.h
+++ b/ark_vrf_amd/csrc/sha512_dev.h
@@ -158,12 +158,88 @@
 #pragma unroll
   for (int i = 0; i < 8; i++) out[i] = s.h[i];
 }
+AVRF_DI void be128_le(uint64_t hi, uint64_t lo, uint32_t (&w)[4]) {
+  uint64_t b0 = __builtin_bswap64(hi), b1 = __builtin_bswap64(lo);
+  w[0] = (uint32_t)b0; w[1] = (uint32_t)(b0 >> 32); w[2] = (uint32_t)b1; w[3] = (uint32_t)(b1 >> 32);
+}
 AVRF_DI void digest_le128(const uint64_t (&dg)[8], int off16, uint32_t (&w)[4]) {
   uint64_t hi = 0, lo = 0;
 #pragma unroll
   for (int i = 0; i < 4; i++) { if (off16 == i) { hi = dg[2 * i]; lo = dg[2 * i + 1]; } }
-  uint64_t b0 = __builtin_bswap64(hi), b1 = __builtin_bswap64(lo);
-  w[0] = (uint32_t)b0; w[1] = (uint32_t)(b0 >> 32); w[2] = (uint32_t)b1; w[3] = (uint32_t)(b1 >> 32);
+  be128_le(hi, lo, w);
+}
+
+struct ShaLit { uint64_t w[16]; };
+constexpr void sha512_lit_byte(ShaLit &l, int pos, uint8_t b) { l.w[pos >> 3] |= (uint64_t)b << (56 - 8 * (pos & 7)); }
+template <int LEN> AVRF_DI void sha512_lit(Sha512 &s, const ShaLit &l) {
+  static_assert(LEN > 0 && LEN <= 128, "a literal prefix lies within the first block");
+#pragma unroll
+  for (int i = 0; i < (LEN + 7) / 8; i++) s.w[i] |= l.w[i];
+  if constexpr (LEN == 128) sha512_flush(s);
+}
+template <int POS> AVRF_DI void sha512_u32le_at(Sha512 &s, uint32_t v) {
+  constexpr int p = POS & 127, wi = p >> 3, k = p & 7;
+  const uint64_t be = __builtin_bswap32(v);
+  if constexpr (k <= 4) s.w[wi] |= be << (8 * (4 - k));
+  else {
+    s.w[wi] |= be >> (8 * (k - 4));
+    if constexpr (wi == 15) sha512_flush(s);
+    s.w[(wi + 1) & 15] |= be << (64 - 8 * (k - 4));
+  }
+  if constexpr (p + 4 == 128) sha512_flush(s);
+}
+template <int POS, int I = 0> AVRF_DI void sha512_words_at(Sha512 &s, const uint32_t (&v)[8]) {
+  sha512_u32le_at<POS + 4 * I>(s, v[I]);
+  if constexpr (I < 7) sha512_words_at<POS, I + 1>(s, v);
+}
+template <int END> AVRF_DI void sha512_static_end(Sha512 &s) { s.fill = END & 127; s.total = END; }
+
+struct Sha512Tail { Sha512 s; uint64_t acc; };
+AVRF_DI void sha512_deposit(Sha512 &s, uint32_t wi, uint64_t v) {
+#pragma unroll
+  for (int i = 0; i < 16; i++) s.w[i] = (wi == (uint32_t)i) ? v : s.w[i];
+}
+AVRF_DI Sha512Tail sha512_tail_begin(const Sha512 &s) {
+  Sha512Tail t; t.s = s; t.acc = 0;
+  const uint32_t wi = s.fill >> 3;
+#pragma unroll
+  for (int i = 0; i < 16; i++) { if (wi == (uint32_t)i) { t.acc = s.w[i]; t.s.w[i] = 0; } }
+  return t;
+}
+AVRF_DI void sha512_tail_absorb(Sha512Tail &t, uint64_t x, uint32_t nb) {
+  const uint32_t k = t.s.fill & 7;
+  const uint64_t full = t.acc | (x >> (8 * k));
+  if (k + nb >= 8) {
+    sha512_deposit(t.s, t.s.fill >> 3, full);
+    t.acc = k ? x << (64 - 8 * k) : 0ULL;
+    t.s.fill += nb; t.s.total += nb;
+    if (t.s.fill >= 128) { const uint32_t rest = t.s.fill - 128; sha512_flush(t.s); t.s.fill = rest; }
+  } else {
+    t.acc = full; t.s.fill += nb; t.s.total += nb;
+  }
+}
+AVRF_DI void sha512_tail_bytes(Sha512Tail &t, const uint8_t *p, uint32_t n) {
+  for (uint32_t off = 0; off < n; off += 8) {
+    const uint32_t nb = n - off < 8 ? n - off : 8;
+    uint64_t x = 0;
+#pragma unroll
+    for (uint32_t i = 0; i < 8; i++) if (i < nb) x |= (uint64_t)p[off + i] << (56 - 8 * i);
+    sha512_tail_absorb(t, x, nb);
+  }
+}
+AVRF_DI void sha512_tail_words(Sha512Tail &t, const uint32_t (&v)[8]) {
+#pragma unroll
+  for (int i = 0; i < 4; i++) sha512_tail_absorb(t, ((uint64_t)__builtin_bswap32(v[2 * i]) << 32) | __builtin_bswap32(v[2 * i + 1]), 8);
+}
+AVRF_DI void sha512_tail_final(Sha512Tail t, uint64_t (&out)[8]) {
+  const uint64_t bits = (uint64_t)t.s.total * 8;
+  const uint32_t k = t.s.fill & 7;
+  sha512_deposit(t.s, t.s.fill >> 3, t.acc | (0x8000000000000000ULL >> (8 * k)));
+  if (t.s.fill >= 112) sha512_flush(t.s);
+  t.s.w[15] = bits;
+  sha512_compress(t.s.h, t.s.w);
+#pragma unroll
+  for (int i = 0; i < 8; i++) out[i] = t.s.h[i];
 }
 
 AVRF_DI void tr_init(Sha512 &s) { sha512_init(s); }
diff --git a/ark_vrf_amd/csrc/vrf_batch.hip b/ark_vrf_amd/csrc/vrf_batch.hip
--- a/ark_vrf_amd/csrc/vrf_batch.hip
+++ b/ark_vrf_amd/csrc/vrf_batch.hip
@@ -7,6 +7,48 @@
 #error "vrf_batch.hip is built once per suite: -DAVRF_TU_SUITE=<id> (csrc/Makefile)"
 #endif
 namespace avrf {
+
+template <class S>
+AVRF_DI uint32_t thin_prepare_one(const BatchDev &b, uint32_t j, uint32_t io0, uint32_t ad0, uint32_t adl,
+                                  uint32_t *__restrict__ c_out, uint32_t *__restrict__ z_out) {
+  using Fr = typename S::Fr; using L = ThinLayout1<S>;
+  constexpr ShaLit lit = L::prefix();
+  const uint8_t *pk = b.pks_xy + 64 * (size_t)j, *p = b.ios_xy + 128 * (size_t)io0, *pr = b.proofs + 96 * (size_t)j;
+  uint32_t f = 0, v[8];
+  Sha512 h; sha512_init(h);
+  sha512_lit<L::PK>(h, lit);
+  fp x = fp_load_le(pk), y = fp_load_le(pk + 32);
+  f |= point_flags<S>(x, y); point_words<S>(x, y, v); sha512_words_at<L::PK>(h, v);
+  x = fp_load_le(p); y = fp_load_le(p + 32);
+  f |= point_flags<S>(x, y); point_words<S>(x, y, v); sha512_words_at<L::IN>(h, v);
+  x = fp_load_le(p + 64); y = fp_load_le(p + 96);
+  f |= point_flags<S>(x, y); point_words<S>(x, y, v); sha512_words_at<L::OUT>(h, v);
+  sha512_u32le_at<L::ADL>(h, adl); sha512_u32le_at<L::ADL + 4>(h, 0);
+  sha512_static_end<L::END>(h);
+  Sha512Tail t = sha512_tail_begin(h);
+  sha512_tail_bytes(t, b.ads + ad0, adl);
+  uint64_t seed[8], blk[8]; uint32_t w[4];
+  {
+    Sha512Tail td = t;
+    sha512_tail_absorb(td, (uint64_t)DS_DELINEARIZE << 56, 1);
+    sha512_tail_final(td, seed); sha512_xof_block(seed, 0, blk); be128_le(blk[0], blk[1], w);
+    *reinterpret_cast<uint4 *>(z_out + 4 * (size_t)io0) = make_uint4(w[0], w[1], w[2], w[3]);
+  }
+  x = fp_load_le(pr); y = fp_load_le(pr + 32);
+  const fp s = fp_load_le(pr + 64);
+  if (point_flags<S>(x, y) & FLAG_RANGE) f |= FLAG_RANGE;
+  if (ge_p<Fr>(s)) f |= FLAG_SCALAR;
+  sha512_tail_absorb(t, (uint64_t)DS_CHALLENGE << 56, 1);
+  point_words<S>(x, y, v); sha512_tail_words(t, v);
+  sha512_tail_final(t, seed); sha512_xof_block(seed, 0, blk); be128_le(blk[0], blk[1], w);
+  *reinterpret_cast<uint4 *>(c_out + 4 * (size_t)j) = make_uint4(w[0], w[1], w[2], w[3]);
+  if (b.records) {
+    uint4 *r = reinterpret_cast<uint4 *>(b.records + 64 * (size_t)j);
+    const uint4 *sp = reinterpret_cast<const uint4 *>(pr + 64);
+    r[0] = make_uint4(w[0], w[1], w[2], w[3]); r[1] = make_uint4(0, 0, 0, 0); r[2] = sp[0]; r[3] = sp[1];
+  }
+  return f;
+}
 
 template <class S>
 __global__ void __launch_bounds__(128)
@@ -17,6 +59,11 @@
   uint32_t io0 = b.io_off[j], io1 = b.io_off[j + 1], m = io1 - io0;
   uint32_t ad0 = b.ad_off[j], adl = b.ad_off[j + 1] - ad0;
   uint32_t f = 0;
+  if constexpr (ThinLayout1<S>::OK) if (m == 1) {
+    f = thin_prepare_one<S>(b, j, io0, ad0, adl, c_out, z_out);
+    if (f) atomicOr(flags, f);
+    return;
+  }
   suite_tr<S> h; tr_init(h);
   for (int i = 0; i < S::SUITE_ID_LEN; i++) tr_byte(h, S::SUITE_ID[i]);
   tr_byte(h, DS_THIN);
@@ -75,21 +122,29 @@
   uint32_t *__restrict__ scalars; te_pre *__restrict__ pre; const uint8_t *__restrict__ pks_xy;
   using Fr = typename S::Fr;
   AVRF_DI void r(uint32_t j, uint32_t io0, const fp &w_plain, const uint8_t *xy) const { emit_term<S>(scalars, pre, 2 * j + 2 * io0, w_plain, xy); }
-  AVRF_DI void key(uint32_t j, uint32_t io0, const fp &wc) const { emit_term<S>(scalars, pre, 2 * j + 2 * io0 + 1, fp_from_mont<Fr>(wc), pks_xy + 64 * (size_t)j); }
+  AVRF_DI void key(uint32_t j, uint32_t io0, const fp &wc_plain) const { emit_term<S>(scalars, pre, 2 * j + 2 * io0 + 1, wc_plain, pks_xy + 64 * (size_t)j); }
   AVRF_DI void output(uint32_t j, uint32_t io0, uint32_t i, const fp &sc_plain, const uint8_t *xy) const { emit_term<S>(scalars, pre, 2 * j + 2 * io0 + 2 + 2 * i, sc_plain, xy); }
-  AVRF_DI void input(uint32_t j, uint32_t io0, uint32_t i, const fp &sc_mont, const uint8_t *xy) const { emit_term<S>(scalars, pre, 2 * j + 2 * io0 + 3 + 2 * i, fp_from_mont<Fr>(sc_mont), xy); }
+  AVRF_DI void input(uint32_t j, uint32_t io0, uint32_t i, const fp &sc_plain, const uint8_t *xy) const { emit_term<S>(scalars, pre, 2 * j + 2 * io0 + 3 + 2 * i, sc_plain, xy); }
 };
 
-template <class S>
-__global__ void __launch_bounds__(128)
+enum { TERMS_NT = 256 };
+template <class S>
+__global__ void __launch_bounds__(TERMS_NT)
 k_thin_terms(BatchDev b, Seed64 seed, uint64_t j0, const uint32_t *__restrict__ c_in, const uint32_t *__restrict__ z_in,
              uint32_t *__restrict__ scalars, te_pre *__restrict__ pre, uint32_t *__restrict__ gpart) {
-  using Fr = typename S::Fr;
-  __shared__ fp red[128];
-  uint32_t j = blockIdx.x * blockDim.x + threadIdx.x;
+  using Fr = typename S::Fr; using WB = WeightBlocks<TERMS_NT, 16>;
+  __shared__ fp red[TERMS_NT];
+  __shared__ uint64_t wblk[WB::WORDS];
+  const uint32_t jb = blockIdx.x * TERMS_NT, j = jb + threadIdx.x;
+  if (!b.weights) WB::fill(seed, j0 + jb, b.n - jb < TERMS_NT ? b.n - jb : TERMS_NT, wblk);
   fp ws = fp_zero();
-  if (j < b.n) ws = thin_item<S>(b, seed, j0, c_in, z_in, j, PlainTerms<S>{scalars, pre, b.pks_xy});
-  const fp sum = block_sum<Fr, 128>(ws, red);
+  if (j < b.n) {
+    uint32_t ww[4];
+    if (b.weights) { const uint4 v = *reinterpret_cast<const uint4 *>(b.weights + 16 * (size_t)j); ww[0] = v.x; ww[1] = v.y; ww[2] = v.z; ww[3] = v.w; }
+    else WB::chunk16(wblk, j0 + jb, j0 + j, 0, ww);
+    ws = thin_item_plain<S>(b, ww, c_in, z_in, j, PlainTerms<S>{scalars, pre, b.pks_xy});
+  }
+  const fp sum = block_sum<Fr, TERMS_NT>(ws, red);
   if (threadIdx.x == 0) fp_store(gpart + 8 * (size_t)blockIdx.x, sum);
 }
 
@@ -184,18 +239,29 @@
 };
 
 template <class S>
-__global__ void __launch_bounds__(128)
+__global__ void __launch_bounds__(TERMS_NT)
 k_ped_terms(BatchDev b, Seed64 seed, uint64_t j0, const uint32_t *__restrict__ c_in, const uint8_t *__restrict__ merged_xy,
             uint32_t *__restrict__ scalars, te_pre *__restrict__ pre, uint32_t *__restrict__ gpart, uint32_t *__restrict__ bpart) {
-  using Fr = typename S::Fr;
-  __shared__ fp red[128];
-  uint32_t j = blockIdx.x * blockDim.x + threadIdx.x;
+  using Fr = typename S::Fr; using WB = WeightBlocks<TERMS_NT, 32>;
+  __shared__ fp red[TERMS_NT];
+  __shared__ uint64_t wblk[WB::WORDS];
+  const uint32_t jb = blockIdx.x * TERMS_NT, j = jb + threadIdx.x;
+  if (!b.weights) WB::fill(seed, j0 + jb, b.n - jb < TERMS_NT ? b.n - jb : TERMS_NT, wblk);
   fp us = fp_zero(), usb = fp_zero();
-  if (j < b.n) us = ped_item<S>(b, seed, j0, c_in, merged_xy, j, PlainPedTerms<S>{scalars, pre}, usb);
-  const fp gsum = block_sum<Fr, 128>(us, red);
+  if (j < b.n) {
+    fp t_plain, u_plain;
+    if (b.weights) { t_plain = fp_from_u128(reinterpret_cast<const uint32_t *>(b.weights + 32 * (size_t)j)); u_plain = fp_from_u128(reinterpret_cast<const uint32_t *>(b.weights + 32 * (size_t)j + 16)); }
+    else {
+      uint32_t w[4];
+      WB::chunk16(wblk, j0 + jb, j0 + j, 0, w); t_plain = fp_zero(); t_plain.v[0] = w[0]; t_plain.v[1] = w[1]; t_plain.v[2] = w[2]; t_plain.v[3] = w[3];
+      WB::chunk16(wblk, j0 + jb, j0 + j, 1, w); u_plain = fp_zero(); u_plain.v[0] = w[0]; u_plain.v[1] = w[1]; u_plain.v[2] = w[2]; u_plain.v[3] = w[3];
+    }
+    us = ped_item_w<S>(b, t_plain, u_plain, c_in, merged_xy, j, PlainPedTerms<S>{scalars, pre}, usb);
+  }
+  const fp gsum = block_sum<Fr, TERMS_NT>(us, red);
   if (threadIdx.x == 0) fp_store(gpart + 8 * (size_t)blockIdx.x, gsum);
   __syncthreads();
-  const fp bsum = block_sum<Fr, 128>(usb, red);
+  const fp bsum = block_sum<Fr, TERMS_NT>(usb, red);
   if (threadIdx.x == 0) fp_store(bpart + 8 * (size_t)blockIdx.x, bsum);
 }
 
@@ -208,7 +274,7 @@
 template <class S> void BatchOps<S>::ped_terms(const BatchDev &b, const Seed64 &seed, uint64_t j0, const uint32_t *d_c, const uint8_t *d_merged,
                                                uint32_t *d_scalars, te_pre_raw *d_pre, uint32_t *d_gpart, uint32_t n_terms, hipStream_t st) {
   if (!b.n) return;
-  dim3 g((b.n + 127) / 128), blk(128);
+  dim3 g((b.n + TERMS_NT - 1) / TERMS_NT), blk(TERMS_NT);
   uint32_t *bp = d_gpart + 8 * (size_t)g.x;
   hipLaunchKernelGGL(k_ped_terms<S>, g, blk, 0, st, b, seed, j0, d_c, d_merged, d_scalars, (te_pre *)d_pre, d_gpart, bp);
   hipLaunchKernelGGL(k_g_final<S>, dim3(1), dim3(256), 0, st, d_gpart, g.x, d_scalars, (te_pre *)d_pre, n_terms - 2, 0);
@@ -222,7 +288,7 @@
 template <class S> void BatchOps<S>::thin_terms(const BatchDev &b, const Seed64 &seed, uint64_t j0, const uint32_t *d_c, const uint32_t *d_z,
                                                 uint32_t *d_scalars, te_pre_raw *d_pre, uint32_t *d_gpart, uint32_t n_terms, hipStream_t st) {
   if (!b.n) return;
-  dim3 g((b.n + 127) / 128), blk(128);
+  dim3 g((b.n + TERMS_NT - 1) / TERMS_NT), blk(TERMS_NT);
   hipLaunchKernelGGL(k_thin_terms<S>, g, blk, 0, st, b, seed, j0, d_c, d_z, d_scalars, (te_pre *)d_pre, d_gpart);
   hipLaunchKernelGGL(k_g_final<S>, dim3(1), dim3(256), 0, st, d_gpart, g.x, d_scalars, (te_pre *)d_pre, n_terms - 1, 0);
 }
```

After: 138.5 million, median of 6. +4.9%, better.
